# yukiteruono/pbsim3

Measured on AMD Instinct MI355X. Metric: simulated bases/sec, higher is better.
Workload: dtype u8

## Files before the change

### include/pbsim3_amd.h

```cpp
#ifndef PBSIM3_AMD_H
#define PBSIM3_AMD_H

#include <stdint.h>

#ifdef __cplusplus
extern "C" {
#endif

#define PBSIM_SUCCEEDED 1
#define PBSIM_FAILED 0

#define PBSIM_STRATEGY_WGS 1
#define PBSIM_STRATEGY_TRANS 2
#define PBSIM_STRATEGY_TEMPL 3
#define PBSIM_METHOD_QS 1
#define PBSIM_METHOD_ERR 2
#define PBSIM_METHOD_SAMPLE 3

typedef struct pbsim_params {
  int32_t strategy;
  int32_t method;
  uint32_t seed;
  int32_t pass_num;
  double depth;
  double accuracy_mean;
  double len_mean;
  double len_sd;
  double hp_del_bias;
  int64_t len_min;
  int64_t len_max;
  int64_t sub_ratio;
  int64_t ins_ratio;
  int64_t del_ratio;
  char id_prefix[64];
} pbsim_params;

typedef struct pbsim_stats {
  int64_t res_num;
  int64_t res_pass_num;
  int64_t res_len_total;
  int64_t res_len_min, res_len_max;
  int64_t res_sub_num, res_ins_num, res_del_num;
  double res_depth;
  double res_len_mean, res_len_sd;
  double res_accuracy_mean, res_accuracy_sd;
  double res_sub_rate, res_ins_rate, res_del_rate;
} pbsim_stats;

typedef struct pbsim_batch_info {
  int64_t first_read;
  int64_t n_reads;
  int64_t n_final;
  int32_t quota_reached;
  int32_t need_truncated_read;
  int64_t len_total_after;
  int64_t bases;
  int64_t read_text_bytes;
  int64_t maf_text_bytes;
  int64_t ref_bases;
  int64_t maf_columns;
} pbsim_batch_info;

typedef struct pbsim_sink {
  void *user;
  int (*on_read_text)(void *user, const char *text, int64_t bytes);
  int (*on_maf_text)(void *user, const char *text, int64_t bytes);
} pbsim_sink;

typedef struct pbsim_ctx pbsim_ctx;

void pbsim_params_default(pbsim_params *p);
pbsim_ctx *pbsim_create(const pbsim_params *p, int device);
void pbsim_destroy(pbsim_ctx *ctx);
const char *pbsim_last_error(void);
const char *pbsim_version(void);

int pbsim_load_errhmm(pbsim_ctx *ctx, const char *path);
int pbsim_load_qshmm(pbsim_ctx *ctx, const char *path);

int pbsim_set_reference(pbsim_ctx *ctx, const uint8_t *seq, int64_t len, int64_t record_index);
int pbsim_set_reference_device(pbsim_ctx *ctx, const void *seq_device, int64_t len, int64_t record_index);
int pbsim_prefetch_reference(pbsim_ctx *ctx, const uint8_t *seq, int64_t len);
int pbsim_prefetch_reference_device(pbsim_ctx *ctx, const void *seq_device, int64_t len);
int pbsim_add_hp_census(pbsim_ctx *ctx, const uint8_t *seq, int64_t len);
int pbsim_finish_hp_census(pbsim_ctx *ctx);

int pbsim_set_transcripts(pbsim_ctx *ctx, int64_t n, const char *const *ids, const int64_t *plus_exp,
                          const int64_t *minus_exp, const uint8_t *const *seqs, const int64_t *lens);

int pbsim_set_templates(pbsim_ctx *ctx, int64_t n, const char *const *ids, const uint8_t *const *seqs,
                        const int64_t *lens);

int pbsim_simulate_wgs(pbsim_ctx *ctx, const pbsim_sink *sink);
int pbsim_simulate_trans(pbsim_ctx *ctx, const pbsim_sink *sink);
int pbsim_simulate_templ(pbsim_ctx *ctx, const pbsim_sink *sink);
int pbsim_simulate_units_range(pbsim_ctx *ctx, int64_t first_read, int64_t n_reads, const pbsim_sink *sink);
int64_t pbsim_unit_reads(pbsim_ctx *ctx);

typedef struct pbsim_read_arrays {
  uint8_t *seq, *qual;
  int32_t *ref_pos;
  int64_t *offsets;
  int64_t *read_number;
  int32_t *pass_index, *unit;
  uint8_t *strand;
  int64_t *ref_start;
  int32_t *ref_span, *n_sub, *n_ins, *n_del;
} pbsim_read_arrays;
typedef struct pbsim_array_sink {
  void *user;
  int (*alloc)(void *user, int64_t tasks, int64_t bases, pbsim_read_arrays *out);
  int (*on_batch)(void *user, const pbsim_batch_info *info);
} pbsim_array_sink;
int pbsim_simulate_arrays(pbsim_ctx *ctx, const pbsim_array_sink *sink);
int pbsim_load_transcript_file(pbsim_ctx *ctx, const char *path, int64_t stats[2]);
int pbsim_load_template_file(pbsim_ctx *ctx, const char *path, int64_t stats[2]);
int pbsim_get_stats(pbsim_ctx *ctx, pbsim_stats *out);
int pbsim_set_sample_profile(pbsim_ctx *ctx, int64_t n, const uint8_t *const *quals, const int64_t *lens);
int pbsim_simulate_sample(pbsim_ctx *ctx, const pbsim_sink *sink);
typedef struct pbsim_sample_stats {
  int64_t num, len_min, len_max, len_total;
  int64_t num_filtered, len_min_filtered, len_max_filtered, len_total_filtered;
  double len_mean_filtered, len_sd_filtered, accuracy_mean_filtered, accuracy_sd_filtered;
} pbsim_sample_stats;
int pbsim_sample_profile_from_bytes(pbsim_ctx *ctx, const void *fastq, int64_t n, double accuracy_min, double accuracy_max,
                                    pbsim_sample_stats *out);
int pbsim_sample_profile_from_device(pbsim_ctx *ctx, const void *d_fastq, int64_t n, double accuracy_min, double accuracy_max,
                                     pbsim_sample_stats *out);
int pbsim_load_sample_fastq(pbsim_ctx *ctx, const char *path, double accuracy_min, double accuracy_max, pbsim_sample_stats *out);
int pbsim_sample_profile_text(pbsim_ctx *ctx, char *dst, int64_t cap, int64_t *bytes);
int pbsim_set_sample_chunk_bytes(pbsim_ctx *ctx, int64_t bytes);
int pbsim_load_sample(pbsim_ctx *ctx, const char *path, double accuracy_min, double accuracy_max, pbsim_sample_stats *out);
int pbsim_sample_profile_from_bam_bytes(pbsim_ctx *ctx, const void *bam, int64_t n, double accuracy_min, double accuracy_max,
                                        pbsim_sample_stats *out);
int pbsim_sample_profile_from_bam_device(pbsim_ctx *ctx, const void *d_bam, int64_t n, double accuracy_min, double accuracy_max,
                                         pbsim_sample_stats *out);
int64_t pbsim_sam_header(pbsim_ctx *ctx, char *buf, int64_t cap);
int pbsim_set_bam_output(pbsim_ctx *ctx, int on);
int64_t pbsim_bam_header(pbsim_ctx *ctx, char *buf, int64_t cap);
int pbsim_set_truth_bam(pbsim_ctx *ctx, int on);
int64_t pbsim_truth_bam_header(pbsim_ctx *ctx, char *buf, int64_t cap);
int64_t pbsim_job_truth_bam_header(pbsim_ctx *ctx, int64_t record, char *buf, int64_t cap);
int pbsim_set_deflate(pbsim_ctx *ctx, int mask);
int64_t pbsim_deflate_bound(int64_t text_bytes);
int pbsim_batch_fetch_deflated(pbsim_ctx *ctx, char *read_gz, int64_t read_cap, char *maf_gz, int64_t maf_cap,
                               int64_t *read_gz_bytes, int64_t *maf_gz_bytes);
int pbsim_deflate_buffer(pbsim_ctx *ctx, const void *src, int64_t n, void *dst, int64_t cap, int64_t *out_bytes);
int64_t pbsim_inflate_bound(const void *src, int64_t n);
int pbsim_inflate_buffer(pbsim_ctx *ctx, const void *src, int64_t n, void *dst, int64_t cap, int64_t *out_bytes);
typedef struct pbsim_sorted_bam_sink {
  void *user;
  int (*on_bam)(void *user, const char *bytes, int64_t n, int64_t offset);
  int (*on_index)(void *user, const char *bytes, int64_t n);
} pbsim_sorted_bam_sink;
int pbsim_truth_bam_sort(pbsim_ctx *ctx, const void *bam, int64_t n, const pbsim_sorted_bam_sink *sink, int64_t stats[4]);
typedef struct pbsim_eval_truth {
  const void *bytes;
  int64_t n;
  const char *ref_name;
} pbsim_eval_truth;
typedef struct pbsim_eval_opts {
  int32_t overlap_permille;
  int32_t hash_bits;
} pbsim_eval_opts;
typedef struct pbsim_eval_sink {
  void *user;
  int (*on_verdicts)(void *user, const unsigned char *bytes, int64_t n);
} pbsim_eval_sink;
int pbsim_truth_bam_eval(pbsim_ctx *ctx, const pbsim_eval_truth *truth, int n_truth, const void *query, int64_t n,
                         const pbsim_eval_opts *opts, const pbsim_eval_sink *sink, int64_t counts[12], int64_t hist[512]);
int64_t pbsim_eval_report(const int64_t counts[12], const int64_t hist[512], char *buf, int64_t cap);
typedef struct pbsim_depth_opts {
  int32_t exclude_flags, min_mapq, count_deletions;
  int32_t format;
  int64_t window;
  int64_t piece_bytes;
} pbsim_depth_opts;
typedef struct pbsim_depth_sink {
  void *user;
  int (*on_text)(void *user, const char *bytes, int64_t n, int64_t offset);
  int (*on_refs)(void *user, int32_t n_ref, const char *const *names,
                 const int64_t *rows );
  int (*on_depth)(void *user, int32_t ref, const int32_t *depth, int64_t l_ref);
} pbsim_depth_sink;
int pbsim_bam_depth(pbsim_ctx *ctx, const void *bam, int64_t n, const pbsim_depth_opts *opts,
                    const pbsim_depth_sink *sink, int64_t counts[6], int64_t hist[256]);
int64_t pbsim_depth_report(const int64_t counts[6], int32_t n_ref, const char *const *names, const int64_t *rows,
                           const int64_t hist[256], char *buf, int64_t cap);
typedef struct pbsim_stats_file {
  const void *bam;
  int64_t n;
} pbsim_stats_file;
typedef struct pbsim_stats_opts {
  int32_t exclude_flags, min_mapq;
  int64_t piece_bytes;
} pbsim_stats_opts;
typedef struct pbsim_stats_sink {
  void *user;
  int (*on_text)(void *user, const char *bytes, int64_t n, int64_t offset);
} pbsim_stats_sink;
int pbsim_bam_stats(pbsim_ctx *ctx, const pbsim_stats_file *files, int n_files, const pbsim_stats_opts *opts,
                    const pbsim_stats_sink *sink, int64_t counts[10], int64_t len_row[16], int64_t totals[12],
                    int64_t hist_q[128], int64_t hist_identity[1001], int64_t hist_qacc[1001]);
int64_t pbsim_stats_report(const int64_t counts[10], const int64_t len_row[16], const int64_t totals[12],
                           const int64_t hist_q[128], const int64_t hist_identity[1001], const int64_t hist_qacc[1001],
                           char *buf, int64_t cap);
typedef struct pbsim_errors_ref {
  const char *name;
  const void *lines;
  int64_t bytes;
} pbsim_errors_ref;
typedef struct pbsim_errors_file {
  const void *bam;
  int64_t n;
  const char *ref_name;
} pbsim_errors_file;
typedef struct pbsim_errors_opts {
  int32_t exclude_flags, min_mapq;
  int64_t piece_bytes;
} pbsim_errors_opts;
typedef struct pbsim_errors_sink {
  void *user;
  int (*on_text)(void *user, const char *bytes, int64_t n, int64_t offset);
} pbsim_errors_sink;
typedef struct pbsim_errors_result {
  int64_t counts[14];
  int64_t totals[11];
  int64_t pair[25];
  int64_t hp_cols[12], hp_sub[12], hp_del[12];
  int64_t ins_len[64], del_len[64];
  int64_t ins_base[5], del_base[5];
  int64_t qcal[128][3];
  int64_t hist_identity[1001];
  int64_t fit_ok, fit_bias_milli, fit_suggest_milli;
} pbsim_errors_result;
int pbsim_bam_errors(pbsim_ctx *ctx, const pbsim_errors_ref *refs, int n_refs, const pbsim_errors_file *files, int n_files,
                     const pbsim_errors_opts *opts, const pbsim_errors_sink *sink, pbsim_errors_result *result);
int64_t pbsim_errors_report(const pbsim_errors_result *result, char *buf, int64_t cap);
typedef struct pbsim_pileup_opts {
  int32_t exclude_flags, min_mapq, min_baseq;
  int32_t format;
  int64_t min_depth;
  int64_t piece_bytes;
} pbsim_pileup_opts;
typedef struct pbsim_pileup_sink {
  void *user;
  int (*on_text)(void *user, const char *bytes, int64_t n, int64_t offset);
  int (*on_cells)(void *user, int32_t ref, const uint32_t *cells, int64_t l_ref);
} pbsim_pileup_sink;
typedef struct pbsim_pileup_result {
  int64_t counts[9];
  int64_t sites[9];
  int64_t cell_sums[8];
  int64_t ins_unanchored, max_depth;
  int64_t hp_called[12], hp_sub[12], hp_del[12], hp_ins[12];
} pbsim_pileup_result;
int pbsim_bam_pileup(pbsim_ctx *ctx, const pbsim_errors_ref *refs, int n_refs, const pbsim_errors_file *files, int n_files,
                     const pbsim_pileup_opts *opts, const pbsim_pileup_sink *sink, pbsim_pileup_result *result);
int64_t pbsim_pileup_report(const pbsim_pileup_result *result, char *buf, int64_t cap);
typedef struct pbsim_consensus_opts {
  int32_t exclude_flags, min_mapq, min_baseq;
  int32_t fill;
  int64_t min_depth;
  int32_t max_ins;
  int32_t line_width;
  int64_t piece_bytes;
} pbsim_consensus_opts;
typedef struct pbsim_consensus_sink {
  void *user;
  int (*on_text)(void *user, const char *bytes, int64_t n, int64_t offset);
  int (*on_record)(void *user, int32_t ref, int64_t l_ref, int64_t l_cons);
} pbsim_consensus_sink;
typedef struct pbsim_consensus_result {
  int64_t counts[9];
  int64_t sites[9];
  int64_t ins_unanchored, max_depth;
  int64_t bases[6];
  int64_t ins_sites, ins_longest, ins_capped;
  int64_t ins_len[64];
  int64_t text_bytes;
} pbsim_consensus_result;
int pbsim_bam_consensus(pbsim_ctx *ctx, const pbsim_errors_ref *refs, int n_refs, const pbsim_errors_file *files, int n_files,
                        const pbsim_consensus_opts *opts, const pbsim_consensus_sink *sink, pbsim_consensus_result *result);
int64_t pbsim_consensus_report(const pbsim_consensus_result *result, char *buf, int64_t cap);
typedef struct pbsim_call_opts {
  int32_t exclude_flags, min_mapq, min_baseq;
  int32_t max_ins;
  int64_t min_depth;
  int64_t piece_bytes;
} pbsim_call_opts;
typedef struct pbsim_call_sink {
  void *user;
  int (*on_text)(void *user, const char *bytes, int64_t n, int64_t offset);
  int (*on_record)(void *user, int32_t ref, int64_t l_ref, int64_t n_variants);
} pbsim_call_sink;
typedef struct pbsim_call_result {
  int64_t counts[9];
  int64_t sites[9];
  int64_t ins_unanchored, max_depth;
  int64_t variants;
// ... 174 lines not shown
```

### pbsim3_amd/__init__.py

```python
import ctypes as C
import os
from typing import NamedTuple

from . import build as _build

STRATEGY_WGS, STRATEGY_TRANS, STRATEGY_TEMPL = 1, 2, 3
METHOD_QS, METHOD_ERR, METHOD_SAMPLE = 1, 2, 3


class Params(C.Structure):
    _fields_ = [
        ("strategy", C.c_int32), ("method", C.c_int32), ("seed", C.c_uint32), ("pass_num", C.c_int32),
        ("depth", C.c_double), ("accuracy_mean", C.c_double), ("len_mean", C.c_double), ("len_sd", C.c_double),
        ("hp_del_bias", C.c_double), ("len_min", C.c_int64), ("len_max", C.c_int64),
        ("sub_ratio", C.c_int64), ("ins_ratio", C.c_int64), ("del_ratio", C.c_int64),
        ("id_prefix", C.c_char * 64),
    ]


class Stats(C.Structure):
    _fields_ = [
        ("res_num", C.c_int64), ("res_pass_num", C.c_int64), ("res_len_total", C.c_int64),
        ("res_len_min", C.c_int64), ("res_len_max", C.c_int64),
        ("res_sub_num", C.c_int64), ("res_ins_num", C.c_int64), ("res_del_num", C.c_int64),
# ... 257 lines not shown



class MutateOpts(C.Structure):
    _fields_ = [("seed", C.c_uint32), ("snv_ppm", C.c_int32), ("ins_ppm", C.c_int32), ("del_ppm", C.c_int32), ("ext_ppm", C.c_int32),
                ("max_indel", C.c_int32), ("line_width", C.c_int32), ("piece_bytes", C.c_int64)]


MUTATE_TEXT_CB = C.CFUNCTYPE(C.c_int, C.c_void_p, C.c_void_p, C.c_int64, C.c_int64)
MUTATE_RECORD_CB = C.CFUNCTYPE(C.c_int, C.c_void_p, C.c_int32, C.c_int64, C.c_int64, C.c_int64)
MUTATE_ORIGIN_CB = C.CFUNCTYPE(C.c_int, C.c_void_p, C.c_int32, C.c_void_p, C.c_int64)


class MutateSink(C.Structure):
    _fields_ = [("user", C.c_void_p), ("on_fasta", MUTATE_TEXT_CB), ("on_vcf", MUTATE_TEXT_CB), ("on_record", MUTATE_RECORD_CB),
                ("on_origin", MUTATE_ORIGIN_CB)]


MUTATE_TYPES = ["snv", "ins", "del"]


class MutateResult(C.Structure):
    _fields_ = [("records", C.c_int64), ("bases_in", C.c_int64), ("eligible", C.c_int64), ("bases_out", C.c_int64), ("drawn", C.c_int64 * 3),
                ("void_del", C.c_int64), ("dropped", C.c_int64), ("merged", C.c_int64), ("substituted", C.c_int64), ("inserted", C.c_int64),
                ("deleted", C.c_int64), ("variants", C.c_int64), ("types", C.c_int64 * 3), ("ref_bases", C.c_int64), ("alt_bases", C.c_int64),
                ("longest_ref", C.c_int64), ("longest_alt", C.c_int64), ("header_bytes", C.c_int64), ("vcf_bytes", C.c_int64),
                ("fasta_bytes", C.c_int64)]


class CompareOpts(C.Structure):
    _fields_ = [("lines", C.c_int32), ("min_ms", C.c_int32), ("piece_bytes", C.c_int64)]


COMPARE_TEXT_CB = C.CFUNCTYPE(C.c_int, C.c_void_p, C.c_void_p, C.c_int64, C.c_int64)


class CompareSink(C.Structure):
    _fields_ = [("user", C.c_void_p), ("on_text", COMPARE_TEXT_CB)]


COMPARE_LINES = {"discordant": 0, "all": 1}


class CompareResult(C.Structure):
    _fields_ = [("files", C.c_int64 * 11 * 2), ("types", C.c_int64 * 6 * 4), ("lengths", C.c_int64 * 4 * 5 * 2), ("ms", C.c_int64 * 2 * 64),
                ("text_bytes", C.c_int64)]

class ApplyOpts(C.Structure):
    _fields_ = [("haplotype", C.c_int32), ("sample", C.c_int32), ("lines", C.c_int32), ("line_width", C.c_int32), ("piece_bytes", C.c_int64)]


APPLY_TEXT_CB = C.CFUNCTYPE(C.c_int, C.c_void_p, C.c_void_p, C.c_int64, C.c_int64)
APPLY_RECORD_CB = C.CFUNCTYPE(C.c_int, C.c_void_p, C.c_int32, C.c_int64, C.c_int64, C.c_int64)
APPLY_ORIGIN_CB = C.CFUNCTYPE(C.c_int, C.c_void_p, C.c_int32, C.c_void_p, C.c_int64)


class ApplySink(C.Structure):
    _fields_ = [("user", C.c_void_p), ("on_fasta", APPLY_TEXT_CB), ("on_text", APPLY_TEXT_CB), ("on_record", APPLY_RECORD_CB),
                ("on_origin", APPLY_ORIGIN_CB)]


APPLY_LINES = {"discordant": 0, "all": 1}
APPLY_TYPES = ["snv", "ins", "del", "complex"]
APPLY_SCALARS = ["lines", "malformed", "unknown_contig", "no_call", "ref_allele", "unsupported", "ref_mismatch", "filtered", "no_change", "overlap",
                 "applied", "bases_in", "bases_out", "inserted", "deleted", "substituted", "longest_cluster", "fasta_bytes", "text_bytes"]


class ApplyResult(C.Structure):
    _fields_ = [("lines", C.c_int64), ("malformed", C.c_int64), ("unknown_contig", C.c_int64), ("no_call", C.c_int64), ("ref_allele", C.c_int64),
                ("unsupported", C.c_int64), ("ref_mismatch", C.c_int64), ("filtered", C.c_int64), ("no_change", C.c_int64), ("overlap", C.c_int64),
                ("applied", C.c_int64), ("types", C.c_int64 * 4), ("bases_in", C.c_int64), ("bases_out", C.c_int64), ("inserted", C.c_int64),
                ("deleted", C.c_int64), ("substituted", C.c_int64), ("longest_cluster", C.c_int64), ("fasta_bytes", C.c_int64),
                ("text_bytes", C.c_int64)]

API = [
    ("pbsim_job_add_record", C.c_int, [C.c_void_p, C.c_void_p, C.c_int64]),
    ("pbsim_job_add_record_device", C.c_int, [C.c_void_p, C.c_void_p, C.c_int64]),
    ("pbsim_job_add_record_lines", C.c_int, [C.c_void_p, C.c_void_p, C.c_int64, C.c_int64]),
    ("pbsim_job_add_record_comm", C.c_int, [C.c_void_p, C.c_void_p, C.c_int64, C.POINTER(Comm), C.c_int32]),
    ("pbsim_job_records", C.c_int64, [C.c_void_p]),
    ("pbsim_job_begin", C.c_int, [C.c_void_p, C.c_int64]),
    ("pbsim_job_clear", C.c_int, [C.c_void_p]),
    ("pbsim_job_run", C.c_int, [C.c_void_p, C.POINTER(Comm), C.POINTER(RecordSink)]),
    ("pbsim_job_sam_header", C.c_int64, [C.c_void_p, C.c_int64, C.c_char_p, C.c_int64]),
    ("pbsim_job_bam_header", C.c_int64, [C.c_void_p, C.c_int64, C.c_char_p, C.c_int64]),
    ("pbsim_job_counters", C.c_int, [C.c_void_p, C.POINTER(C.c_int64)]),
    ("pbsim_job_progress", C.c_int, [C.c_void_p, C.POINTER(C.c_int64)]),
    ("pbsim_job_set_interleave", C.c_int, [C.c_void_p, C.c_int]),
    ("pbsim_job_expect", C.c_int, [C.c_void_p, C.c_int64, C.POINTER(C.c_int64)]),
    ("pbsim_job_feed_abort", C.c_int, [C.c_void_p, C.c_char_p]),
    ("pbsim_scratch_state", C.c_int, [C.c_void_p, C.POINTER(C.c_double)]),
    ("pbsim_batch_fetch_lengths", C.c_int, [C.c_void_p, C.c_void_p, C.c_void_p, C.c_void_p]),
    ("pbsim_job_breakdown", C.c_int, [C.c_void_p, C.POINTER(C.c_double)]),
    ("pbsim_bind_host_to_device", C.c_int, [C.c_int, C.c_char_p, C.c_int64]),
    ("pbsim_rccl_unique_id", C.c_int64, [C.c_void_p, C.c_int64]),
    ("pbsim_rccl_comm_create", C.POINTER(Comm), [C.c_void_p, C.c_int64, C.c_int32, C.c_int32, C.c_int32]),
    ("pbsim_rccl_comm_create_file", C.POINTER(Comm), [C.c_char_p, C.c_int32, C.c_int32, C.c_int32]),
    ("pbsim_rccl_comm_info", C.c_int, [C.POINTER(Comm), C.POINTER(C.c_int64)]),
    ("pbsim_rccl_comm_destroy", None, [C.POINTER(Comm)]),
    ("pbsim_stats_keep_values", C.c_int, [C.c_void_p, C.c_int]),
    ("pbsim_stats_merge", C.c_int, [C.c_void_p, C.POINTER(Comm)]),
    ("pbsim_stats_add_tasks", C.c_int, [C.c_void_p, C.c_int64, C.c_int64, C.POINTER(C.c_int32), C.POINTER(C.c_int32),
                                        C.POINTER(C.c_int32), C.POINTER(C.c_int32), C.POINTER(C.c_double)]),
    ("pbsim_format_stats", C.c_int64, [C.POINTER(Params), C.POINTER(Stats), C.c_int64, C.c_char_p, C.c_int64]),
    ("pbsim_cli_main", C.c_int, [C.c_int, C.POINTER(C.c_char_p), C.POINTER(Comm), C.c_int]),
    ("pbsim_params_default", None, [C.POINTER(Params)]),
    ("pbsim_create", C.c_void_p, [C.POINTER(Params), C.c_int]),
    ("pbsim_destroy", None, [C.c_void_p]),
    ("pbsim_last_error", C.c_char_p, []),
    ("pbsim_version", C.c_char_p, []),
    ("pbsim_load_errhmm", C.c_int, [C.c_void_p, C.c_char_p]),
    ("pbsim_load_qshmm", C.c_int, [C.c_void_p, C.c_char_p]),
    ("pbsim_set_reference", C.c_int, [C.c_void_p, C.c_void_p, C.c_int64, C.c_int64]),
    ("pbsim_set_reference_device", C.c_int, [C.c_void_p, C.c_void_p, C.c_int64, C.c_int64]),
    ("pbsim_add_hp_census", C.c_int, [C.c_void_p, C.c_void_p, C.c_int64]),
    ("pbsim_finish_hp_census", C.c_int, [C.c_void_p]),
    ("pbsim_set_transcripts", C.c_int, [C.c_void_p, C.c_int64, C.POINTER(C.c_char_p), C.POINTER(C.c_int64),
                                        C.POINTER(C.c_int64), C.POINTER(C.c_void_p), C.POINTER(C.c_int64)]),
    ("pbsim_set_templates", C.c_int, [C.c_void_p, C.c_int64, C.POINTER(C.c_char_p), C.POINTER(C.c_void_p),
                                      C.POINTER(C.c_int64)]),
    ("pbsim_simulate_templ", C.c_int, [C.c_void_p, C.POINTER(Sink)]),
    ("pbsim_prefetch_reference", C.c_int, [C.c_void_p, C.c_char_p, C.c_int64]),
    ("pbsim_prefetch_reference_device", C.c_int, [C.c_void_p, C.c_void_p, C.c_int64]),
    ("pbsim_simulate_units_range", C.c_int, [C.c_void_p, C.c_int64, C.c_int64, C.POINTER(Sink)]),
    ("pbsim_unit_reads", C.c_int64, [C.c_void_p]),
    ("pbsim_load_transcript_file", C.c_int, [C.c_void_p, C.c_char_p, C.POINTER(C.c_int64)]),
    ("pbsim_load_template_file", C.c_int, [C.c_void_p, C.c_char_p, C.POINTER(C.c_int64)]),
    ("pbsim_simulate_wgs", C.c_int, [C.c_void_p, C.POINTER(Sink)]),
    ("pbsim_simulate_trans", C.c_int, [C.c_void_p, C.POINTER(Sink)]),
    ("pbsim_simulate_arrays", C.c_int, [C.c_void_p, C.POINTER(ArraySink)]),
    ("pbsim_get_stats", C.c_int, [C.c_void_p, C.POINTER(Stats)]),
    ("pbsim_sam_header", C.c_int64, [C.c_void_p, C.c_char_p, C.c_int64]),
    ("pbsim_set_bam_output", C.c_int, [C.c_void_p, C.c_int]),
    ("pbsim_bam_header", C.c_int64, [C.c_void_p, C.c_char_p, C.c_int64]),
    ("pbsim_set_truth_bam", C.c_int, [C.c_void_p, C.c_int]),
    ("pbsim_truth_bam_header", C.c_int64, [C.c_void_p, C.c_char_p, C.c_int64]),
    ("pbsim_job_truth_bam_header", C.c_int64, [C.c_void_p, C.c_int64, C.c_char_p, C.c_int64]),
    ("pbsim_set_sample_profile", C.c_int, [C.c_void_p, C.c_int64, C.POINTER(C.c_void_p), C.POINTER(C.c_int64)]),
    ("pbsim_simulate_sample", C.c_int, [C.c_void_p, C.POINTER(Sink)]),
    ("pbsim_sample_profile_from_bytes", C.c_int, [C.c_void_p, C.c_void_p, C.c_int64, C.c_double, C.c_double, C.POINTER(SampleStats)]),
    ("pbsim_sample_profile_from_device", C.c_int, [C.c_void_p, C.c_void_p, C.c_int64, C.c_double, C.c_double, C.POINTER(SampleStats)]),
    ("pbsim_load_sample_fastq", C.c_int, [C.c_void_p, C.c_char_p, C.c_double, C.c_double, C.POINTER(SampleStats)]),
    ("pbsim_load_sample", C.c_int, [C.c_void_p, C.c_char_p, C.c_double, C.c_double, C.POINTER(SampleStats)]),
    ("pbsim_sample_profile_from_bam_bytes", C.c_int, [C.c_void_p, C.c_void_p, C.c_int64, C.c_double, C.c_double, C.POINTER(SampleStats)]),
    ("pbsim_sample_profile_from_bam_device", C.c_int, [C.c_void_p, C.c_void_p, C.c_int64, C.c_double, C.c_double, C.POINTER(SampleStats)]),
    ("pbsim_sample_profile_text", C.c_int, [C.c_void_p, C.c_void_p, C.c_int64, C.POINTER(C.c_int64)]),
    ("pbsim_set_sample_chunk_bytes", C.c_int, [C.c_void_p, C.c_int64]),
    ("pbsim_simulate_sample_comm", C.c_int, [C.c_void_p, C.POINTER(Comm), C.POINTER(RecordSink)]),
    ("pbsim_set_deflate", C.c_int, [C.c_void_p, C.c_int]),
    ("pbsim_deflate_bound", C.c_int64, [C.c_int64]),
    ("pbsim_batch_fetch_deflated", C.c_int, [C.c_void_p, C.c_void_p, C.c_int64, C.c_void_p, C.c_int64,
                                             C.POINTER(C.c_int64), C.POINTER(C.c_int64)]),
    ("pbsim_deflate_buffer", C.c_int, [C.c_void_p, C.c_void_p, C.c_int64, C.c_void_p, C.c_int64, C.POINTER(C.c_int64)]),
    ("pbsim_inflate_bound", C.c_int64, [C.c_void_p, C.c_int64]),
    ("pbsim_inflate_buffer", C.c_int, [C.c_void_p, C.c_void_p, C.c_int64, C.c_void_p, C.c_int64, C.POINTER(C.c_int64)]),
    ("pbsim_truth_bam_sort", C.c_int, [C.c_void_p, C.c_void_p, C.c_int64, C.POINTER(SortedBamSink), C.POINTER(C.c_int64)]),
    ("pbsim_truth_bam_eval", C.c_int, [C.c_void_p, C.POINTER(EvalTruth), C.c_int, C.c_char_p, C.c_int64, C.POINTER(EvalOpts),
                                       C.POINTER(EvalSink), C.POINTER(C.c_int64), C.POINTER(C.c_int64)]),
    ("pbsim_eval_report", C.c_int64, [C.POINTER(C.c_int64), C.POINTER(C.c_int64), C.c_char_p, C.c_int64]),
    ("pbsim_bam_depth", C.c_int, [C.c_void_p, C.c_char_p, C.c_int64, C.POINTER(DepthOpts), C.POINTER(DepthSink), C.POINTER(C.c_int64),
                                  C.POINTER(C.c_int64)]),
    ("pbsim_depth_report", C.c_int64, [C.POINTER(C.c_int64), C.c_int32, C.POINTER(C.c_char_p), C.POINTER(C.c_int64), C.POINTER(C.c_int64),
                                       C.c_char_p, C.c_int64]),
    ("pbsim_bam_stats", C.c_int, [C.c_void_p, C.POINTER(StatsFile), C.c_int, C.POINTER(StatsOpts), C.POINTER(StatsSink)] + [C.POINTER(C.c_int64)] * 6),
    ("pbsim_stats_report", C.c_int64, [C.POINTER(C.c_int64)] * 6 + [C.c_char_p, C.c_int64]),
    ("pbsim_bam_errors", C.c_int, [C.c_void_p, C.POINTER(ErrorsRef), C.c_int, C.POINTER(ErrorsFile), C.c_int, C.POINTER(ErrorsOpts),
                                   C.POINTER(ErrorsSink), C.POINTER(ErrorsResult)]),
    ("pbsim_errors_report", C.c_int64, [C.POINTER(ErrorsResult), C.c_char_p, C.c_int64]),
    ("pbsim_bam_pileup", C.c_int, [C.c_void_p, C.POINTER(ErrorsRef), C.c_int, C.POINTER(ErrorsFile), C.c_int, C.POINTER(PileupOpts),
                                   C.POINTER(PileupSink), C.POINTER(PileupResult)]),
    ("pbsim_pileup_report", C.c_int64, [C.POINTER(PileupResult), C.c_char_p, C.c_int64]),
    ("pbsim_bam_consensus", C.c_int, [C.c_void_p, C.POINTER(ErrorsRef), C.c_int, C.POINTER(ErrorsFile), C.c_int, C.POINTER(ConsensusOpts),
                                      C.POINTER(ConsensusSink), C.POINTER(ConsensusResult)]),
    ("pbsim_consensus_report", C.c_int64, [C.POINTER(ConsensusResult), C.c_char_p, C.c_int64]),
    ("pbsim_bam_call", C.c_int, [C.c_void_p, C.POINTER(ErrorsRef), C.c_int, C.POINTER(ErrorsFile), C.c_int, C.POINTER(CallOpts), C.POINTER(CallSink),
                                 C.POINTER(CallResult)]),
    ("pbsim_call_report", C.c_int64, [C.POINTER(CallResult), C.c_char_p, C.c_int64]),
    ("pbsim_genome_mutate", C.c_int, [C.c_void_p, C.POINTER(ErrorsRef), C.c_int, C.POINTER(MutateOpts), C.POINTER(MutateSink),
                                      C.POINTER(MutateResult)]),
    ("pbsim_mutate_report", C.c_int64, [C.POINTER(MutateResult), C.c_char_p, C.c_int64]),
    ("pbsim_vcf_compare", C.c_int, [C.c_void_p, C.POINTER(ErrorsRef), C.c_int, C.POINTER(C.c_char_p), C.c_char_p, C.c_int64, C.c_char_p, C.c_int64,
                                    C.POINTER(CompareOpts), C.POINTER(CompareSink), C.POINTER(CompareResult)]),
    ("pbsim_compare_report", C.c_int64, [C.POINTER(CompareResult), C.c_char_p, C.c_int64]),
    ("pbsim_vcf_apply", C.c_int, [C.c_void_p, C.POINTER(ErrorsRef), C.c_int, C.POINTER(C.c_char_p), C.c_char_p, C.c_int64, C.POINTER(ApplyOpts),
                                  C.POINTER(ApplySink), C.POINTER(ApplyResult)]),
    ("pbsim_apply_report", C.c_int64, [C.POINTER(ApplyResult), C.c_char_p, C.c_int64]),
    ("pbsim_apply_sample", C.c_int32, [C.c_char_p, C.c_int64, C.c_char_p]),
    ("pbsim_batch_walk", C.c_int, [C.c_void_p, C.c_int64, C.c_int64, C.c_int64, C.POINTER(C.c_int64)]),
    ("pbsim_slot_count", C.c_int, []),
    ("pbsim_select_slot", C.c_int, [C.c_void_p, C.c_int]),
    ("pbsim_batch_walk_begin", C.c_int, [C.c_void_p, C.c_int64, C.c_int64, C.c_int64]),
    ("pbsim_batch_walk_end", C.c_int, [C.c_void_p, C.POINTER(C.c_int64)]),
    ("pbsim_batch_finalize", C.c_int, [C.c_void_p, C.c_int64, C.POINTER(BatchInfo)]),
    ("pbsim_batch_fetch", C.c_int, [C.c_void_p, C.c_void_p, C.c_void_p]),
    ("pbsim_batch_account", C.c_int, [C.c_void_p]),
    ("pbsim_reset_stats", C.c_int, [C.c_void_p]),
    ("pbsim_unit_quota", C.c_int64, [C.c_void_p]),
    ("pbsim_batch_capacity", C.c_int64, [C.c_void_p]),
    ("pbsim_set_scratch_bytes", C.c_int, [C.c_void_p, C.c_int64]),
    ("pbsim_release_pools", C.c_int, [C.c_void_p]),
    ("pbsim_prof_reset", C.c_int, [C.c_void_p]),
    ("pbsim_prof_get", C.c_int, [C.c_void_p, C.POINTER(C.c_double), C.POINTER(C.c_int64), C.POINTER(C.c_double)]),
    ("pbsim_prof_walk_busy", C.c_int, [C.c_void_p, C.POINTER(C.c_double)]),
    ("pbsim_prof_tail", C.c_int, [C.c_void_p, C.POINTER(C.c_double), C.POINTER(C.c_int64)]),
    ("pbsim_prof_secondary", C.c_int, [C.c_void_p, C.POINTER(C.c_double)]),
    ("pbsim_prof_wave_launches", C.c_int64, [C.c_void_p]),
    ("pbsim_stream", C.c_void_p, [C.c_void_p]),
    ("pbsim_device_synchronize", C.c_int, [C.c_void_p]),
    ("pbsim_philox4x32_10", None, [C.POINTER(C.c_uint32), C.POINTER(C.c_uint32), C.POINTER(C.c_uint32)]),
    ("pbsim_dump_table", C.c_int64, [C.c_void_p, C.c_int, C.c_void_p, C.c_int64]),
]

_lib = None


def lib_path():
    return _build.LIB


def _torch_runtime_first():
    import sys
    if "torch" in sys.modules or os.environ.get("PBSIM_TORCH_COMPAT", "1") == "0":
        return
    try:
        import importlib.util
        spec = importlib.util.find_spec("torch")
        if not spec or not spec.origin:
            return
        libdir = os.path.join(os.path.dirname(spec.origin), "lib")
        for name in ("libhsa-runtime64.so", "libamdhip64.so"):
            path = os.path.join(libdir, name)
            if os.path.exists(path):
                C.CDLL(path, mode=C.RTLD_GLOBAL)
    except Exception:
        pass


def load(build_if_missing=True):
    global _lib
    if _lib is not None:
        return _lib
    _torch_runtime_first()
    if not os.path.exists(_build.LIB):
        if not build_if_missing:
            raise RuntimeError("libpbsim3_amd.so is not built (python -m pbsim3_amd.build)")
        _build.build()
    lib = C.CDLL(_build.LIB)
    for name, res, args in API:
        fn = getattr(lib, name)
        fn.restype = res
        fn.argtypes = args
    _lib = lib
    return lib


def eval_report(counts, hist) -> bytes:
    vals = [counts[k] for k in EVAL_COUNTS] if isinstance(counts, dict) else list(counts)
    c = (C.c_int64 * 12)(*[int(v) for v in vals])
    h = (C.c_int64 * 512)(*[int(v) for row in hist for v in row])
    n = load().pbsim_eval_report(c, h, None, 0)
    if n < 0:
        raise PbsimError("pbsim_eval_report: bad argument")
    buf = C.create_string_buffer(max(n, 1))
    load().pbsim_eval_report(c, h, buf, n)
    return buf.raw[:n]


def depth_report(counts, refs, hist) -> bytes:
    vals = [counts[k] for k in DEPTH_COUNTS] if isinstance(counts, dict) else list(counts)
    refs = list(refs)
    c = (C.c_int64 * 6)(*[int(v) for v in vals])
    h = (C.c_int64 * 256)(*[int(v) for v in hist])
    names = (C.c_char_p * max(len(refs), 1))(*[r[0].encode() if isinstance(r[0], str) else bytes(r[0]) for r in refs])
    rows = (C.c_int64 * max(4 * len(refs), 1))(*[int(v) for r in refs for v in r[1:5]])
    n = load().pbsim_depth_report(c, len(refs), names, rows, h, None, 0)
    if n < 0:
        raise PbsimError("pbsim_depth_report: bad argument")
    buf = C.create_string_buffer(max(n, 1))
    load().pbsim_depth_report(c, len(refs), names, rows, h, buf, n)
    return buf.raw[:n]


def stats_report(counts, len_row, totals, hist_q, hist_identity, hist_qacc) -> bytes:
    def vals(x, names):
        return [int(x[k]) for k in names] if isinstance(x, dict) else [int(v) for v in x]
    parts = [vals(counts, STATS_COUNTS), vals(len_row, STATS_LEN_ROW), vals(totals, STATS_TOTALS), [int(v) for v in hist_q],
             [int(v) for v in hist_identity], [int(v) for v in hist_qacc]]
    if [len(p) for p in parts] != [10, 16, 12, 128, 1001, 1001]:
        raise ValueError("stats_report: 10 counts, 16 length values, 12 totals and histograms of 128, 1001 and 1001 bins")
    arrs = [(C.c_int64 * len(p))(*p) for p in parts]
    n = load().pbsim_stats_report(*arrs, None, 0)
    if n < 0:
        raise PbsimError("pbsim_stats_report: bad argument")
    buf = C.create_string_buffer(max(n, 1))
    load().pbsim_stats_report(*arrs, buf, n)
    return buf.raw[:n]


def _errors_dict(res) -> dict:
    out = dict(counts=dict(zip(ERRORS_COUNTS, (int(v) for v in res.counts))), totals=dict(zip(ERRORS_TOTALS, (int(v) for v in res.totals))))
    for name, _ in ERRORS_ARRAYS:
        out[name] = [int(v) for v in getattr(res, name)]
    for name in ERRORS_FIT:
        out[name] = int(getattr(res, name))
    return out

# ... 450 lines not shown
        sink = Sink(None, SINK_CB(on_read), SINK_CB(on_maf))
        _check(self.lib.pbsim_simulate_wgs(self.h, C.byref(sink) if collect else None))
        return b"".join(reads), b"".join(mafs)

    def simulate_arrays(self, on_batch=None, labels=True):
        import collections

        import torch
        dev = torch.device("cuda", self.device)
        pending, batches, error = collections.deque(), [], []

        def alloc(user, tasks, bases, out):
            try:
                torch.cuda.current_stream(dev).synchronize()
                t = {}
                for name, dtype, per in ARRAY_FIELDS:
                    if name == "ref_pos" and not labels:
                        t[name] = None
                        continue
                    n = bases if per == "base" else tasks + 1 if per == "offset" else tasks
                    t[name] = torch.empty(n, dtype=getattr(torch, dtype), device=dev)
                    setattr(out.contents, name, t[name].data_ptr() or None)
                pending.append(t)
                return 1
            except BaseException as e:
                error.append(e)
                return 0

        def done(user, info):
            try:
                b = ReadBatch(first_read=info.contents.first_read, **pending.popleft())
                if on_batch is None:
                    batches.append(b)
                    return 1
                return 0 if on_batch(b) is False else 1
            except BaseException as e:
                error.append(e)
                return 0

        sink = ArraySink(None, ARRAY_ALLOC_CB(alloc), ARRAY_BATCH_CB(done))
        ok = self.lib.pbsim_simulate_arrays(self.h, C.byref(sink))
        if error:
            raise error[0]
        _check(ok)
        if on_batch is not None:
            return None
        if not batches:
            empty = {name: torch.zeros(1 if per == "offset" else 0, dtype=getattr(torch, dtype), device=dev)
                     for name, dtype, per in ARRAY_FIELDS}
            if not labels:
                empty["ref_pos"] = None
            return ReadBatch(first_read=1, **empty)
        cat = {}
        for name, _, per in ARRAY_FIELDS:
            if name == "ref_pos" and not labels:
                cat[name] = None
            elif per == "offset":
                base, parts = 0, []
                for b in batches:
                    parts.append(b.offsets[:-1] + base)
                    base += int(b.offsets[-1])
                parts.append(torch.tensor([base], dtype=torch.int64, device=dev))
                cat[name] = torch.cat(parts)
            else:
                cat[name] = torch.cat([getattr(b, name) for b in batches])
        return ReadBatch(first_read=batches[0].first_read, **cat)

    def sam_header(self):
        n = self.lib.pbsim_sam_header(self.h, None, 0)
        buf = C.create_string_buffer(n + 1)
        self.lib.pbsim_sam_header(self.h, buf, n + 1)
        return buf.raw[:n]

    def set_sample_profile(self, quals):
        n = len(quals)
        keep = [C.create_string_buffer(q, len(q)) for q in quals]
        ptrs = (C.c_void_p * n)(*[C.cast(b, C.c_void_p).value for b in keep])
        lens = (C.c_int64 * n)(*[len(q) for q in quals])
        _check(self.lib.pbsim_set_sample_profile(self.h, n, ptrs, lens))

    def load_sample_fastq(self, path, acc_min=0.75, acc_max=1.0):
        st = SampleStats()
        _check(self.lib.pbsim_load_sample_fastq(self.h, os.fsencode(path), acc_min, acc_max, C.byref(st)))
        return st

    def sample_profile_from_fastq(self, data, acc_min=0.75, acc_max=1.0):
        st = SampleStats()
        if isinstance(data, (bytes, bytearray, memoryview)):
            data = bytes(data)
            _check(self.lib.pbsim_sample_profile_from_bytes(self.h, data, len(data), acc_min, acc_max, C.byref(st)))
            return st
        import torch
        if not (isinstance(data, torch.Tensor) and data.dtype == torch.uint8 and data.is_cuda and data.is_contiguous()):
            raise TypeError("sample_profile_from_fastq: bytes or a contiguous uint8 tensor on the context's device")
        if data.device.index != self.device:
            raise ValueError("sample_profile_from_fastq: the tensor is on another device than the context")
        torch.cuda.current_stream(data.device).synchronize()
        _check(self.lib.pbsim_sample_profile_from_device(self.h, C.c_void_p(data.data_ptr()), data.numel(), acc_min, acc_max,
                                                         C.byref(st)))
        return st

    def load_sample(self, path, acc_min=0.75, acc_max=1.0):
        st = SampleStats()
        _check(self.lib.pbsim_load_sample(self.h, os.fsencode(path), acc_min, acc_max, C.byref(st)))
        return st

    def sample_profile_from_bam(self, data, acc_min=0.75, acc_max=1.0):
        st = SampleStats()
        if isinstance(data, (bytes, bytearray, memoryview)):
            data = bytes(data)
            _check(self.lib.pbsim_sample_profile_from_bam_bytes(self.h, data, len(data), acc_min, acc_max, C.byref(st)))
            return st
        import torch
        if not (isinstance(data, torch.Tensor) and data.dtype == torch.uint8 and data.is_cuda and data.is_contiguous()):
            raise TypeError("sample_profile_from_bam: bytes or a contiguous uint8 tensor on the context's device")
        if data.device.index != self.device:
            raise ValueError("sample_profile_from_bam: the tensor is on another device than the context")
        torch.cuda.current_stream(data.device).synchronize()
        _check(self.lib.pbsim_sample_profile_from_bam_device(self.h, C.c_void_p(data.data_ptr()), data.numel(), acc_min, acc_max,
                                                             C.byref(st)))
        return st

    def sample_profile(self):
        n = C.c_int64(0)
        _check(self.lib.pbsim_sample_profile_text(self.h, None, 0, C.byref(n)))
        buf = C.create_string_buffer(max(n.value, 1))
        _check(self.lib.pbsim_sample_profile_text(self.h, buf, n.value, C.byref(n)))
        return buf.raw[:n.value].split(b"\n")[:-1]

    def set_sample_chunk_bytes(self, n):
        _check(self.lib.pbsim_set_sample_chunk_bytes(self.h, n))

    def simulate_sample(self, collect=True):
        return self._simulate(self.lib.pbsim_simulate_sample, collect)

    def _simulate(self, fn, collect):
        reads, mafs = [], []

        def on_read(user, text, n):
            reads.append(C.string_at(text, n))
            return 1

        def on_maf(user, text, n):
            mafs.append(C.string_at(text, n))
            return 1

        sink = Sink(None, SINK_CB(on_read), SINK_CB(on_maf))
        _check(fn(self.h, C.byref(sink) if collect else None))
        return b"".join(reads), b"".join(mafs)

    def set_deflate(self, mask=3):
        _check(self.lib.pbsim_set_deflate(self.h, 3 if mask is True else int(mask)))

    def deflate_buffer(self, data: bytes) -> bytes:
        cap = self.lib.pbsim_deflate_bound(len(data)) + 64
        dst = C.create_string_buffer(cap)
        n = C.c_int64(0)
        src = C.create_string_buffer(data, len(data)) if data else None
        _check(self.lib.pbsim_deflate_buffer(self.h, src, len(data), dst, cap, C.byref(n)))
        return dst.raw[:n.value]

    def inflate_buffer(self, data: bytes) -> bytes:
        cap = inflate_bound(data)
        if cap < 0:
            _check(self.lib.pbsim_inflate_buffer(self.h, data, len(data), None, 0, C.byref(C.c_int64(0))))
        dst = C.create_string_buffer(max(cap, 1))
        n = C.c_int64(0)
        _check(self.lib.pbsim_inflate_buffer(self.h, data, len(data), dst, cap, C.byref(n)))
        return dst.raw[:n.value]

    def sort_truth_bam(self, data, on_index=None):
        parts, index, at = [], [], [0]

        def on_bam(user, ptr, n, offset):
            if offset != at[0]:
                return 0
            parts.append(C.string_at(ptr, n))
            at[0] += n
            return 1

        def on_idx(user, ptr, n):
            index.append(C.string_at(ptr, n))
            if on_index:
                on_index(index[-1])
            return 1
        sink = SortedBamSink(None, SORTED_BAM_CB(on_bam), SORTED_INDEX_CB(on_idx))
        stats = (C.c_int64 * 4)()
        _check(self.lib.pbsim_truth_bam_sort(self.h, bytes(data), len(data), C.byref(sink), stats))
        return b"".join(parts), b"".join(index), tuple(stats)

    def eval_bam(self, truth, query, ref_names=None, overlap=0.1, verdicts=False, hash_bits=0):
        import numpy as np
        files = [truth] if isinstance(truth, (bytes, bytearray, memoryview)) else list(truth)
        names = list(ref_names) if ref_names is not None else [None] * len(files)
        if len(names) != len(files):
            raise ValueError("ref_names: one entry per truth file (%d given for %d files)" % (len(names), len(files)))
        if not 0 < overlap <= 1:
            raise ValueError("overlap must be in (0, 1]")
        keep = [bytes(f) for f in files]
        arr = (EvalTruth * max(len(keep), 1))()
        for k, (f, nm) in enumerate(zip(keep, names)):
            arr[k] = EvalTruth(f, len(f), None if nm is None else (nm.encode() if isinstance(nm, str) else bytes(nm)))
        opts = EvalOpts(max(1, int(round(overlap * 1000))), int(hash_bits))
        got = []

        def on_verdicts(user, ptr, n):
            got.append(np.frombuffer(C.string_at(ptr, n), dtype=np.uint8).copy() if n else np.zeros(0, np.uint8))
            return 1
        sink = EvalSink(None, EVAL_VERDICTS_CB(on_verdicts))
        counts = (C.c_int64 * 12)()
        hist = (C.c_int64 * 512)()
        query = bytes(query)
        _check(self.lib.pbsim_truth_bam_eval(self.h, arr, len(keep), query, len(query), C.byref(opts), C.byref(sink) if verdicts else None,
                                             counts, hist))
        cd = dict(zip(EVAL_COUNTS, (int(v) for v in counts)))
        hd = np.array(list(hist), dtype=np.int64).reshape(256, 2)
        out = (cd, hd, eval_report(cd, hd))
        return out + (got[0],) if verdicts else out

    def bam_depth(self, data, fmt="bedgraph", window=0, min_mapq=0, exclude_flags=0x704, deletions=True, arrays=False, piece_bytes=0):
        import numpy as np
        if fmt not in DEPTH_FORMATS:
            raise ValueError("fmt must be bedgraph or window")
        parts, at, refs, depth = [], [0], [], []

        def on_text(user, ptr, n, offset):
            if offset != at[0]:
                return 0
            parts.append(C.string_at(ptr, n))
            at[0] += n
            return 1

        def on_refs(user, n_ref, names, rows):
            refs.extend((names[r],) + tuple(int(rows[4 * r + k]) for k in range(4)) for r in range(n_ref))
            return 1

        def on_depth(user, ref, ptr, l_ref):
            depth.append(np.frombuffer(C.string_at(ptr, 4 * l_ref), dtype=np.int32).copy() if l_ref else np.zeros(0, np.int32))
            return 1
        sink = DepthSink(None, DEPTH_TEXT_CB(on_text), DEPTH_REFS_CB(on_refs), DEPTH_ARRAY_CB(on_depth) if arrays else DEPTH_ARRAY_CB())
        opts = DepthOpts(int(exclude_flags), int(min_mapq), 1 if deletions else 0, DEPTH_FORMATS[fmt], int(window), int(piece_bytes))
        counts = (C.c_int64 * 6)()
        hist = (C.c_int64 * 256)()
        data = bytes(data)
        _check(self.lib.pbsim_bam_depth(self.h, data, len(data), C.byref(opts), C.byref(sink), counts, hist))
        cd = dict(zip(DEPTH_COUNTS, (int(v) for v in counts)))
        hd = np.array(list(hist), dtype=np.int64)
        out = (b"".join(parts), cd, refs, hd, depth_report(cd, refs, hd))
        return out + (depth,) if arrays else out

    def bam_stats(self, files, min_mapq=0, exclude_flags=0x900, text=False, piece_bytes=0):
        import numpy as np
        if isinstance(files, (bytes, bytearray, memoryview)):
            files = [files]
        files = [bytes(f) for f in files]
        arr = (StatsFile * max(len(files), 1))(*[StatsFile(C.cast(C.c_char_p(f), C.c_void_p), len(f)) for f in files])
        parts, at = [], [0]

        def on_text(user, ptr, n, offset):
            if offset != at[0]:
                return 0
            parts.append(C.string_at(ptr, n))
            at[0] += n
            return 1
        sink = StatsSink(None, STATS_TEXT_CB(on_text) if text else STATS_TEXT_CB())
        opts = StatsOpts(int(exclude_flags), int(min_mapq), int(piece_bytes))
        out = [(C.c_int64 * k)() for k in (10, 16, 12, 128, 1001, 1001)]
        _check(self.lib.pbsim_bam_stats(self.h, arr, len(files), C.byref(opts), C.byref(sink), *out))
        cd = dict(zip(STATS_COUNTS, (int(v) for v in out[0])))
        ld = dict(zip(STATS_LEN_ROW, (int(v) for v in out[1])))
        td = dict(zip(STATS_TOTALS, (int(v) for v in out[2])))
        hists = tuple(np.array(list(h), dtype=np.int64) for h in out[3:])
        res = (cd, ld, td) + hists + (stats_report(cd, ld, td, *hists),)
        return res + (b"".join(parts),) if text else res

    def bam_errors(self, files, genome, ref_names=None, text=False, min_mapq=0, exclude_flags=0x900, piece_bytes=0):
        if isinstance(files, (bytes, bytearray, memoryview)):
            files = [files]
        files = [bytes(f) for f in files]
        names = list(ref_names) if ref_names is not None else [None] * len(files)
        if len(names) != len(files):
            raise ValueError("ref_names: one entry per file (%d given for %d files)" % (len(names), len(files)))
        names = [None if nm is None else (nm.encode() if isinstance(nm, str) else bytes(nm)) for nm in names]
        genome = [((nm.encode() if isinstance(nm, str) else bytes(nm)), bytes(lines)) for nm, lines in genome]
        refs = (ErrorsRef * max(len(genome), 1))(*[ErrorsRef(nm, C.cast(C.c_char_p(lines), C.c_void_p), len(lines)) for nm, lines in genome])
        arr = (ErrorsFile * max(len(files), 1))(*[ErrorsFile(C.cast(C.c_char_p(f), C.c_void_p), len(f), nm) for f, nm in zip(files, names)])
        parts, at = [], [0]

        def on_text(user, ptr, n, offset):
            if offset != at[0]:
                return 0
            parts.append(C.string_at(ptr, n))
            at[0] += n
            return 1
        sink = ErrorsSink(None, ERRORS_TEXT_CB(on_text) if text else ERRORS_TEXT_CB())
        opts = ErrorsOpts(int(exclude_flags), int(min_mapq), int(piece_bytes))
        res = ErrorsResult()
        _check(self.lib.pbsim_bam_errors(self.h, refs, len(genome), arr, len(files), C.byref(opts), C.byref(sink), C.byref(res)))
        out = _errors_dict(res)
        got = (out, errors_report(out))
        return got + (b"".join(parts),) if text else got

    def bam_pileup(self, files, genome, ref_names=None, text=False, fmt="sites", min_mapq=0, exclude_flags=0x900, min_baseq=0, min_depth=1,
                   arrays=False, piece_bytes=0):
        import numpy as np
        if arrays:
            import torch
        if fmt not in PILEUP_FORMATS:
            raise ValueError("fmt must be sites or all")
        if isinstance(files, (bytes, bytearray, memoryview)):
            files = [files]
        files = [bytes(f) for f in files]
# ... 503 lines not shown
```

### pbsim3_amd/csrc/ctx.h

```cpp
#pragma once
#include <hip/hip_runtime.h>
#include <limits.h>
#include <stdio.h>
#include <stdlib.h>
#include <stdint.h>

#include <algorithm>
#include <condition_variable>
#include <functional>
#include <memory>
#include <mutex>
#include <string>
#include <vector>

#include "../../include/pbsim3_amd.h"
#include "host_tables.h"
#include "kernels.h"

namespace pbsim {
extern thread_local std::string g_err;
int fail(const std::string &m);
}


#define NEED_DEVICE(c)                                                                      \
  do {                                                                                      \
    if ((c)->device < 0 || !(c)->stream)                                                    \
      return fail("this context has no HIP device: the gfx950 product path has no CPU fallback"); \
  } while (0)

#define HIP_OK(expr)                                                                        \
  do {                                                                                      \
    hipError_t e_ = (expr);                                                                 \
    if (e_ != hipSuccess)                                                                   \
      return fail(std::string("HIP error: ") + hipGetErrorString(e_) + " at " #expr);       \
  } while (0)

struct DevBuf {
  void *p = nullptr;
  size_t bytes = 0;
  ~DevBuf() { release(); }
  void release() {
    if (p) (void)hipFree(p);
    p = nullptr;
    bytes = 0;
  }
  hipError_t ensure(size_t n, bool exact = false) {
    if (n <= bytes) return hipSuccess;
    release();
    size_t want = exact ? n : std::max<size_t>(n + n / 8 + 256, 64u << 10);
    hipError_t e = hipMalloc(&p, want);
    if (e != hipSuccess) {
      p = nullptr;
      return e;
    }
    bytes = want;
    return hipSuccess;
  }
  template <class T>
  T *as() const {
    return reinterpret_cast<T *>(p);
  }
};

struct HostBuf {
  void *p = nullptr;
  size_t bytes = 0;
  ~HostBuf() {
    if (p) (void)hipHostFree(p);
  }
  hipError_t ensure(size_t n) {
    if (n <= bytes) return hipSuccess;
    if (p) (void)hipHostFree(p);
    p = nullptr;
    bytes = 0;
    size_t want = std::max<size_t>(n + n / 8 + 4096, 1u << 20);
    hipError_t e = hipHostMalloc(&p, want, hipHostMallocDefault);
    if (e != hipSuccess) {
      p = nullptr;
      return e;
    }
    bytes = want;
    return hipSuccess;
  }
};

using namespace pbsim;

constexpr int kMaxSlots = 6;
constexpr int kPipelineDepth = 2;
static_assert(kPipelineDepth >= 1 && kPipelineDepth <= kMaxSlots, "the pipeline's slots are the first of kMaxSlots");

constexpr size_t kScratchSlack = 64u << 10;
constexpr double kSinkBatchBases = 5.0e9;

constexpr int kDfBuffers = 5;
struct DfLane {
  DevBuf d_df_status, d_df_ctl;
  uint32_t epoch = 0;
  DevBuf d_df_dense[kDfBuffers];
  DevBuf d_df_code;
  HostBuf h_df_total, h_df_out[kDfBuffers];
  hipStream_t stream = nullptr;
  hipStream_t copy_stream = nullptr;
  bool own_streams = false;
  hipStream_t own[2] = {nullptr, nullptr};
  bool pre_valid = false, pre_own_staging = false, pre_elsewhere = false;
  const uint8_t *pre_text = nullptr;
  int64_t pre_n = 0;
  int pre_count = 0;
  hipStream_t lane_stream = nullptr;
  hipEvent_t ev_pre = nullptr;
  hipEvent_t ev_hand = nullptr;
  bool hand_open = false;
  hipEvent_t ev_df[kDfBuffers] = {}, ev_cp[kDfBuffers] = {};
  hipEvent_t ev_k0[kDfBuffers] = {}, ev_k1[kDfBuffers] = {};
  std::vector<std::unique_ptr<HostBuf>> arena_blocks;
  std::vector<size_t> arena_fill;
  std::vector<char> arena_touched;
  std::vector<int> arena_idle;
  std::vector<std::pair<const char *, int64_t>> arena_segs;
  size_t arena_bytes() const {
    size_t n = 0;
    for (const auto &b : arena_blocks) n += b->bytes;
    return n;
  }
  void arena_reset() {
    std::fill(arena_fill.begin(), arena_fill.end(), 0);
    arena_segs.clear();
  }
  char *arena_reserve(int64_t n, size_t max_bytes) {
    static const size_t kBlock = getenv("PBSIM_PINNED_BLOCK_KB") && atoll(getenv("PBSIM_PINNED_BLOCK_KB")) > 0
                                     ? (size_t)atoll(getenv("PBSIM_PINNED_BLOCK_KB")) << 10 : (size_t)256u << 20;
    const size_t need = ((size_t)n + 63) & ~(size_t)63;
    for (size_t i = 0; i < arena_blocks.size(); i++) {
      HostBuf &b = *arena_blocks[i];
      if (arena_fill[i] + need <= b.bytes) {
        char *p = (char *)b.p + arena_fill[i];
        arena_fill[i] += need;
        arena_touched[i] = 1;
        arena_segs.emplace_back(p, n);
        return p;
      }
    }
    const size_t want = std::max(kBlock, need);
    if (max_bytes && arena_bytes() + want > max_bytes) return nullptr;
    if (getenv("PBSIM_TRACE")) fprintf(stderr, "[pbsim arena] new block of %zu MB (lane holds %zu MB in %zu blocks)\n", want >> 20, arena_bytes() >> 20, arena_blocks.size());
    arena_blocks.emplace_back(new HostBuf);
    arena_fill.push_back(0);
    arena_touched.push_back(1);
    arena_idle.push_back(0);
    if (arena_blocks.back()->ensure(want) != hipSuccess) {
      arena_blocks.pop_back();
      arena_fill.pop_back();
      arena_touched.pop_back();
      arena_idle.pop_back();
      return nullptr;
    }
    arena_fill.back() = need;
    arena_segs.emplace_back((char *)arena_blocks.back()->p, n);
    return (char *)arena_blocks.back()->p;
  }
  static constexpr int kArenaIdleJobs = 16;
  void arena_release() {
    arena_blocks.clear();
    arena_fill.clear();
    arena_touched.clear();
    arena_idle.clear();
    arena_segs.clear();
  }
  void arena_trim() {
    size_t k = 0;
    for (size_t i = 0; i < arena_blocks.size(); i++) arena_idle[i] = arena_touched[i] ? 0 : arena_idle[i] + 1;
    if (getenv("PBSIM_TRACE")) {
      size_t drop = 0;
      for (size_t i = 0; i < arena_blocks.size(); i++) drop += arena_idle[i] >= kArenaIdleJobs ? 1 : 0;
      if (drop) fprintf(stderr, "[pbsim arena] trim: %zu of %zu blocks go back\n", drop, arena_blocks.size());
    }
    for (size_t i = 0; i < arena_blocks.size(); i++)
      if (arena_idle[i] < kArenaIdleJobs) {
        if (k != i) {
          arena_blocks[k] = std::move(arena_blocks[i]);
          arena_idle[k] = arena_idle[i];
        }
        k++;
      }
    arena_blocks.resize(k);
    arena_idle.resize(k);
    arena_fill.assign(k, 0);
    arena_touched.assign(k, 0);
    arena_segs.clear();
  }
};

struct RefDesc {
  const uint8_t *seq = nullptr;
  const uint8_t *hp = nullptr;
  int64_t len = 0;
  int64_t unit = 0;
  bool hp_flag = false;
  bool hp11 = false;
};

struct StatsAcc {
  int64_t res_num = 0, res_len_total = 0, res_len_min = LONG_MAX, res_len_max = 0;
  int64_t res_sub = 0, res_ins = 0, res_del = 0;
  double accuracy_total = 0.0;
  std::vector<int64_t> freq_len, freq_acc;
  bool keep_values = false;
  struct Block {
    int64_t first_task;
    std::vector<double> values;
  };
  std::vector<Block> blocks;
  void reset() {
    res_num = res_len_total = res_len_max = 0;
    res_len_min = LONG_MAX;
    res_sub = res_ins = res_del = 0;
    accuracy_total = 0.0;
    std::fill(freq_len.begin(), freq_len.end(), 0);
    std::fill(freq_acc.begin(), freq_acc.end(), 0);
    blocks.clear();
  }
};

struct Slot {
  RefDesc ref;
  hipStream_t stream = nullptr;
  hipEvent_t ev0 = nullptr, ev1 = nullptr, ev2 = nullptr, ev3 = nullptr;
  DevBuf d_flags;
  DevBuf d_rawlen, d_len, d_off, d_acc;
  DevBuf d_hist, d_bin_start, d_bin_cursor, d_class_start;
  DevBuf d_task_of_slot, d_slot_of_task, d_wave_cap, d_wave_off, d_wg_tmp, d_wg_order;
  DevBuf d_out_len, d_maf_len, d_nsub, d_nins, d_ndel, d_qsum;
  DevBuf d_cum, d_scan_tmp, d_rt_len, d_mt_len, d_row_dst;
  DevBuf d_n_runs;
  hipEvent_t ev_c0 = nullptr, ev_c1 = nullptr;
  DevBuf d_chain, d_chain_mask;
  DevBuf d_scratch, d_read_text, d_maf_text;
  HostBuf h_read_text, h_maf_text, h_stats, h_flags;
  DfLane df[2];
  hipStream_t walk_stream = nullptr;
  hipEvent_t ev_sq_walk = nullptr, ev_sq_done = nullptr;
  bool sq_pending = false;
  hipEvent_t ev_prep = nullptr;
  hipStream_t coop_stream = nullptr;
  hipEvent_t ev_coop = nullptr;
  bool stats_fetched = false;
  hipEvent_t ev_t0 = nullptr, ev_t1 = nullptr;
  bool text_timed = false;
  int64_t text_in = 0, text_out = 0;
  hipEvent_t ev_text = nullptr;
  int64_t b_first = 0, b_n = 0, b_slots_max = 0;
  bool b_truncated = false, b_enqueued = false, b_walked = false, b_finalized = false;
  bool b_chain = false;
  bool b_exported = false;
  int64_t b_trunc = -1;
  double b_factor = 2.0;
  int64_t b_pass0 = 0;
  int64_t b_max_raw = 0;
  pbsim_batch_info b_info;
};

struct JobRecord {
  DevBuf seq, hp, tiles, flags;
  int64_t len = 0;
  RefDesc ref;
  hipEvent_t ready = nullptr;
  DeviceFlags *h_flags = nullptr;
  ~JobRecord() {
    if (ready) (void)hipEventDestroy(ready);
    if (h_flags) (void)hipHostFree(h_flags);
  }
};

struct pbsim_ctx {
  pbsim_params p;
  int device = 0;
  hipStream_t stream = nullptr;
  Slot slots[kMaxSlots];
  int cur = 0;
  Slot &s() { return slots[cur]; }

  std::unique_ptr<ErrModel> err;
  std::unique_ptr<QsModel> qs;
  HeaderTables hdr;
  HpBias bias;
  ErrClassTables ect;
  QsClassTables qct;
  bool class_tables_dirty = true;
  int coop_wg_errhmm[2] = {0, 0};
  bool header_uploaded = false;

  DevBuf d_prob2len, d_prob2acc, d_cls;
  DevBuf d_qs_tabs_v[2];
  bool qs_tabs_ready[2] = {false, false};
  DevBuf d_seq_own, d_hp, d_tiles, d_ref_flags;
  DevBuf d_seq_next, d_hp_next, d_tiles_next, d_ref_flags_next;
  hipStream_t prefetch_stream = nullptr;
  DevBuf d_lines, d_lines_tmp;
  hipStream_t sq_stream = nullptr;
  const void *pf_src = nullptr;
  int64_t pf_len = 0;
  bool seq_hp_flag = false;
  const uint8_t *d_seq = nullptr;
  int64_t ref_len = 0;
  int64_t unit = 0;
  int64_t census[kHpSlots] = {0};
  int64_t unit_census[kHpSlots] = {0};
  bool census_done = false;
  bool census_from_job = false;
  bool hp11_explicit = false;
  bool hp11_before_job = false;
  int64_t n_units = 0, trans_reads = 0;
  DevBuf d_read_unit, d_read_minus, d_read_base, d_unit_len, d_unit_rank, d_unit_names, d_off_table, d_ssp, d_ssp_rv;
  DevBuf d_sq, d_sq_line_len, d_sq_line_qoff, d_sq_vbase;
  std::vector<int32_t> sq_len;
  std::vector<int64_t> sq_off;
  int64_t sq_total = 0;
  int64_t sp_chunk_bytes = 0;
  int64_t scratch_budget = 0;
  double scratch_factor = 2.0, need_seen = 0.0;
  bool scratch_factor_fixed = false;
  int64_t rewalked_batches = 0;
  bool scratch_auto = true;
  hipStream_t df_streams[2][2] = {{nullptr, nullptr}, {nullptr, nullptr}};
  bool defer_text_sync = false;
  bool defer_account = false;
  int walk_lds_kb = 27;
  bool bam_output = false;
  bool truth_bam = false;
  std::vector<std::string> unit_sn;
  std::vector<int64_t> unit_ln;
  int deflate = 0;
  bool deflate_parallel = false;
  DevBuf d_df_tables;
  DevBuf d_df_prof;

  StatsAcc st;
  std::vector<std::unique_ptr<JobRecord>> job_records;
  std::mutex job_mu;
  std::condition_variable job_cv;
  std::vector<int64_t> job_expect_len;
  std::vector<std::unique_ptr<JobRecord>> job_spare;
  bool job_feed_failed = false;
  std::string job_feed_err;
  int64_t job_counters[8] = {0};
  int64_t job_progress[8] = {0};
  double job_breakdown[16] = {0};
  int job_interleave = 1;
  int64_t job_first_unit = 1;

  double prof_walk_ms = 0, prof_total_ms = 0, prof_tail_ms = 0;
  int64_t prof_walk_launches = 0, prof_tail_launches = 0;
  int64_t prof_wave_launches = 0;
  hipEvent_t ev_prof_base = nullptr;
  std::vector<std::pair<float, float>> prof_intervals;
  double prof_text_ms = 0, prof_deflate_ms = 0;
  int64_t prof_text_launches = 0, prof_text_in = 0, prof_text_out = 0;
  int64_t prof_deflate_launches = 0, prof_deflate_in = 0, prof_deflate_out = 0;
  std::mutex prof_mu;
};

namespace pbsim {
RefDesc current_ref(const pbsim_ctx *c);
int64_t quota_of(const pbsim_ctx *c, int64_t ref_len);
int walk_begin(pbsim_ctx *c, const RefDesc &ref, int64_t first_read, int64_t n_reads, int64_t truncate_remaining, bool chain = false,
               double factor = 0.0 );
double scratch_factor_of(const pbsim_ctx *c);
int chain_end_finalize(pbsim_ctx *c, int64_t len_total_before, pbsim_batch_info *out);
int chain_reads_for(const pbsim_ctx *c, int64_t ref_len, int64_t remaining);
constexpr int kChainReads = 6;
int64_t batch_capacity_for(const pbsim_ctx *c, int64_t ref_len);
int finalize_cut(pbsim_ctx *c, int64_t len_total_before, pbsim_batch_info *out);
int finalize_text(pbsim_ctx *c, pbsim_batch_info *info);
int finalize_uncut(pbsim_ctx *c, pbsim_batch_info *out);
std::string sam_header_text(const pbsim_ctx *c, int64_t unit);
std::string truth_bam_header_bytes(const pbsim_ctx *c, int64_t ref_len);
int truth_bam_check_names(const pbsim_ctx *c);
int account_slot(pbsim_ctx *c, StatsAcc *st);
int account_of(pbsim_ctx *c, Slot &sl, StatsAcc *st);
void stats_add_task(StatsAcc *st, int64_t len_max, bool quality, long len, long nsub, long nins, long ndel, double qsum,
                    std::vector<double> *values);
void stats_finish(const StatsAcc &st, const pbsim_params &p, int64_t ref_len, pbsim_stats *o);
int stats_merge(StatsAcc *st, const pbsim_params &p, const pbsim_comm *comm, int64_t *extra, int n_extra);
int deflate_prelaunch(pbsim_ctx *c, Slot &sl, bool want_read, bool want_maf);
int deflate_pieces(pbsim_ctx *c, DfLane &lane, const uint8_t *d_text, int64_t n,
                   const std::function<int(const char *, int64_t)> &consume,
                   const std::function<char *(int64_t)> *place = nullptr, const std::function<bool()> *tail_hook = nullptr);
int deflate_handoff(pbsim_ctx *c, DfLane &next, int lane_index, const uint8_t *d_text, int64_t n, bool own_staging,
                    hipEvent_t text_ready);
int deflate_settle(DfLane &lane);
int ensure_deflate_ready(pbsim_ctx *c);
int ensure_crc_tables(pbsim_ctx *c);
// ... 5 lines not shown
```

### pbsim3_amd/csrc/deflate.hip

```cpp
#include <hip/hip_runtime.h>
#include <stdint.h>
#include <stdlib.h>

#include "kernels.h"

namespace pbsim {

namespace {

constexpr int kChunk = DF_CHUNK;
constexpr int kThreads = 256;
constexpr int kSeg = kChunk / kThreads;
constexpr int kSegDw = kSeg / 4;
constexpr int kInDw = kChunk / 4 + kChunk / 128;
constexpr int kOutBytes = 33024;
constexpr int kOutDw = kOutBytes / 4;
constexpr int kSyms = 288;
constexpr uint32_t kPoly = 0xEDB88320u;
constexpr int kHeadBits = 18 * 8;
constexpr int kPrefixBits = 3 + 5 + 5 + 4 + 19 * 3;

constexpr int kClLenTab[19] = {3, 5, 4, 4, 4, 5, 5, 5, 5, 5, 5, 5, 4, 5, 5, 5, 5, 3, 3};
constexpr int kClOrderTab[19] = {16, 17, 18, 0, 8, 7, 9, 6, 10, 5, 11, 4, 12, 3, 13, 2, 14, 1, 15};
constexpr uint64_t pack_cl_len() {
  uint64_t v = 0;
  for (int s = 0; s < 19; ++s) v |= (uint64_t)kClLenTab[s] << (3 * s);
  return v;
}
constexpr uint64_t kClLenPacked = pack_cl_len();
__device__ __forceinline__ uint32_t cl_len(uint32_t s) { return (uint32_t)(kClLenPacked >> (3 * s)) & 7u; }
constexpr unsigned __int128 pack_prefix() {
  unsigned __int128 v = 1u | (2u << 1) | ((unsigned __int128)15 << 13);
  for (int i = 0; i < 19; ++i) v |= (unsigned __int128)kClLenTab[kClOrderTab[i]] << (17 + 3 * i);
  return v;
}
constexpr uint64_t kPrefixLo = (uint64_t)pack_prefix();
constexpr uint32_t kPrefixHi = (uint32_t)(pack_prefix() >> 64);

__device__ __forceinline__ uint32_t rev_bits(uint32_t code, uint32_t len) { return __brev(code) >> (32 - len); }

__device__ __forceinline__ uint32_t cl_code(uint32_t s) {
  uint32_t c, l = cl_len(s);
  if (l == 3) c = s == 0 ? 0 : s - 16;
  else if (l == 4) c = s == 12 ? 9 : 4 + s;
  else c = s == 1 ? 20 : s <= 11 ? 16 + s : 15 + s;
  return rev_bits(c, l);
}

__device__ __forceinline__ uint32_t gf2_mul(uint32_t a, uint32_t b) {
  uint32_t p = 0;
#pragma unroll
  for (int i = 0; i < 32; ++i) {
    p ^= b & (0u - ((a >> (31 - i)) & 1u));
    b = (b >> 1) ^ (kPoly & (0u - (b & 1u)));
  }
  return p;
}

struct BitWriter {
  uint32_t *out;
  uint32_t word, nb;
  uint64_t acc;
  __device__ __forceinline__ void init(uint32_t *o, uint32_t bitpos) {
    out = o;
    word = bitpos >> 5;
    nb = bitpos & 31;
    acc = 0;
  }
  __device__ __forceinline__ void put(uint32_t v, uint32_t k) {
    acc |= (uint64_t)v << nb;
    nb += k;
    if (nb >= 32) {
      atomicOr(&out[word++], (uint32_t)acc);
      acc >>= 32;
      nb -= 32;
    }
  }
  __device__ __forceinline__ void put64(uint64_t v, uint32_t k) {
    if (k > 32) {
      put((uint32_t)v, 32);
      put((uint32_t)(v >> 32), k - 32);
    } else {
      put((uint32_t)v, k);
    }
  }
  __device__ __forceinline__ void flush() {
    if (nb) atomicOr(&out[word], (uint32_t)acc);
  }
};

__device__ __forceinline__ void length_symbol(uint32_t L, uint32_t *sym, uint32_t *eb, uint32_t *ev) {
  const uint32_t v = L - 3;
  if (v < 8) {
    *sym = 257 + v;
    *eb = 0;
    *ev = 0;
  } else if (L == 258) {
    *sym = 285;
    *eb = 0;
    *ev = 0;
  } else {
    const uint32_t e = (31 - __clz(v)) - 2;
    *sym = 261 + 4 * e + ((v >> e) & 3);
    *eb = e;
    *ev = v & ((1u << e) - 1);
  }
}

__device__ __forceinline__ uint32_t block_scan_excl(uint32_t v, uint32_t *s_wave, uint32_t *total) {
  const int lane = threadIdx.x & 63, wave = threadIdx.x >> 6;
  uint32_t inc = v;
#pragma unroll
  for (int d = 1; d < 64; d <<= 1) {
    const uint32_t o = __shfl_up(inc, d, 64);
    if (lane >= d) inc += o;
  }
  __syncthreads();
  if (lane == 63) s_wave[wave] = inc;
  __syncthreads();
  uint32_t base = 0, tot = 0;
#pragma unroll
  for (int w = 0; w < kThreads / 64; ++w) {
    const uint32_t x = s_wave[w];
    if (w < wave) base += x;
    tot += x;
  }
  *total = tot;
  return base + inc - v;
}

struct Mask128 {
  uint64_t lo, hi;
};
__device__ __forceinline__ Mask128 m_and(Mask128 a, Mask128 b) { return {a.lo & b.lo, a.hi & b.hi}; }
__device__ __forceinline__ Mask128 m_or(Mask128 a, Mask128 b) { return {a.lo | b.lo, a.hi | b.hi}; }
__device__ __forceinline__ Mask128 m_not(Mask128 a) { return {~a.lo, ~a.hi}; }
template <int K>
__device__ __forceinline__ Mask128 m_shl(Mask128 a) { return {a.lo << K, (a.hi << K) | (a.lo >> (64 - K))}; }
template <int K>
__device__ __forceinline__ Mask128 m_shr(Mask128 a) { return {(a.lo >> K) | (a.hi << (64 - K)), a.hi >> K}; }
__device__ __forceinline__ uint32_t m_nibble(Mask128 a, int j) {
  return (uint32_t)((j < 16 ? a.lo >> (4 * j) : a.hi >> (4 * j - 64)) & 15u);
}
__device__ __forceinline__ int m_first(Mask128 a) { return a.lo ? __builtin_ctzll(a.lo) : 64 + __builtin_ctzll(a.hi); }
__device__ __forceinline__ Mask128 m_clear(Mask128 a, int pos) {
  if (pos < 64) a.lo &= ~(1ull << pos);
  else a.hi &= ~(1ull << (pos - 64));
  return a;
}
__device__ __forceinline__ int m_run(Mask128 m, int pos) {
  uint64_t lo, hi;
  if (pos == 0) {
    lo = m.lo;
    hi = m.hi;
  } else if (pos < 64) {
    lo = (m.lo >> pos) | (m.hi << (64 - pos));
    hi = m.hi >> pos;
  } else {
    lo = m.hi >> (pos - 64);
    hi = 0;
  }
  if (~lo) return __builtin_ctzll(~lo);
  return ~hi ? 64 + __builtin_ctzll(~hi) : 128;
}

struct SegTokens {
  Mask128 lit;
  Mask128 start;
  Mask128 cover;
};

__device__ __forceinline__ SegTokens seg_tokens(const uint32_t (&seg)[kSegDw], int seg_n, uint32_t prev_dword,
                                                bool chunk_start) {
  uint64_t e[2] = {0, 0};
  uint32_t pw = prev_dword;
#pragma unroll
  for (int j = 0; j < kSegDw; ++j) {
    const uint32_t w = seg[j];
    const uint32_t d = w ^ ((w << 8) | (pw >> 24));
    const uint32_t z = ~(((d & 0x7F7F7F7Fu) + 0x7F7F7F7Fu) | d | 0x7F7F7F7Fu);
    const uint32_t nib = (((z >> 7) * 0x00204081u) >> 21) & 15u;
    e[j >> 4] |= (uint64_t)nib << (4 * (j & 15));
    pw = w;
  }
  Mask128 valid;
  valid.lo = seg_n >= 64 ? ~0ull : (1ull << seg_n) - 1;
  valid.hi = seg_n >= 128 ? ~0ull : seg_n > 64 ? (1ull << (seg_n - 64)) - 1 : 0ull;
  Mask128 eq = {e[0] & valid.lo, e[1] & valid.hi};
  if (chunk_start) eq.lo &= ~1ull;
  const Mask128 r3 = m_and(eq, m_and(m_shr<1>(eq), m_shr<2>(eq)));
  SegTokens t;
  t.cover = m_or(r3, m_or(m_shl<1>(r3), m_shl<2>(r3)));
  t.start = m_and(t.cover, m_not(m_shl<1>(t.cover)));
  t.lit = m_and(valid, m_not(t.cover));
  return t;
}

constexpr int kSampleChunks = DF_SAMPLE_CHUNKS;
constexpr int kHdrDw = DF_TABLE_HDR_DW;

struct DfTable {
  uint32_t code[kSyms];
  uint32_t hdr_end_bits;
  uint32_t pad[3];
  uint32_t hdr[kHdrDw];
};
static_assert(sizeof(DfTable) <= DF_TABLE_BYTES, "DF_TABLE_BYTES too small");

__device__ __forceinline__ void load_chunk(const uint8_t *__restrict__ text, int64_t n_bytes, int64_t chunk, uint32_t *s_in,
                                           uint32_t (&seg)[kSegDw], int *n_out, int *seg_n_out, uint32_t *prev_dw) {
  const int tid = threadIdx.x;
  const int64_t base = chunk * (int64_t)kChunk;
  const int n = (int)((n_bytes - base) < (int64_t)kChunk ? (n_bytes - base) : (int64_t)kChunk);
  const uint4 *src4 = reinterpret_cast<const uint4 *>(text + base);
  for (int q = tid; q < kChunk / 16; q += kThreads) {
    uint4 v = make_uint4(0, 0, 0, 0);
    if (q * 16 < n) v = src4[q];
    const int d = q * 4;
    uint32_t *dst = &s_in[d + (d >> 5)];
    dst[0] = v.x;
    dst[1] = v.y;
    dst[2] = v.z;
    dst[3] = v.w;
  }
  __syncthreads();
  const int beg = tid * kSeg;
  *n_out = n;
  *seg_n_out = n - beg < 0 ? 0 : (n - beg < kSeg ? n - beg : kSeg);
#pragma unroll
  for (int j = 0; j < kSegDw; ++j) seg[j] = s_in[tid * (kSegDw + 1) + j];
  *prev_dw = tid ? s_in[tid * (kSegDw + 1) - 2] : 0u;
  __syncthreads();
}

__global__ __launch_bounds__(kThreads) void k_deflate_hist(const uint8_t *__restrict__ text, int64_t n_bytes,
                                                            uint32_t *__restrict__ hist) {
  __shared__ uint32_t s_in[kInDw];
  __shared__ uint32_t s_hist[3 * kSyms + 64];
  const int tid = threadIdx.x, lane = tid & 63;
  for (int i = tid; i < 3 * kSyms + 64; i += kThreads) s_hist[i] = 0;
  uint32_t seg[kSegDw], prev_dw;
  int n, seg_n;
  load_chunk(text, n_bytes, blockIdx.x, s_in, seg, &n, &seg_n, &prev_dw);
  const SegTokens tk = seg_tokens(seg, seg_n, prev_dw, tid == 0);
  const uint32_t copy = (uint32_t)(lane % 3) * kSyms, dummy = 3 * kSyms + lane;
#pragma unroll
  for (int j = 0; j < kSegDw; ++j) {
    const uint32_t nl = m_nibble(tk.lit, j);
    if (nl == 0) continue;
    const uint32_t w = seg[j];
#pragma unroll
    for (int k = 0; k < 4; ++k) atomicAdd(&s_hist[((nl >> k) & 1u) ? copy + ((w >> (8 * k)) & 255u) : dummy], 1u);
  }
  Mask128 st = tk.start;
  while (st.lo | st.hi) {
    const int pos = m_first(st);
    st = m_clear(st, pos);
    uint32_t sy, eb, ev;
    length_symbol((uint32_t)m_run(tk.cover, pos), &sy, &eb, &ev);
    atomicAdd(&s_hist[copy + sy], 1u);
  }
  __syncthreads();
  for (int i = tid; i < 286; i += kThreads) {
    const uint32_t f = s_hist[i] + s_hist[kSyms + i] + s_hist[2 * kSyms + i] + (i == 256 ? 1u : 0u);
    if (f) atomicAdd(&hist[i], f);
  }
}

__global__ __launch_bounds__(kThreads) void k_deflate_build(const uint32_t *__restrict__ hist, DfTable *__restrict__ tbl) {
  __shared__ uint32_t s_freq[kSyms], s_sfreq[kSyms], s_w[kSyms], s_code[kSyms];
  __shared__ uint16_t s_sorted[kSyms], s_par[kSyms], s_leafpar[kSyms], s_dep[kSyms];
  __shared__ uint8_t s_len[kSyms];
  __shared__ uint32_t s_cnt[16], s_first[16];
  __shared__ uint32_t s_img[4 + kHdrDw];
  const int tid = threadIdx.x;
  constexpr int m = 286;
  for (int i = tid; i < kSyms; i += kThreads) {
    s_freq[i] = i < m ? hist[i] + 1u : 0u;
    s_code[i] = 0;
    s_len[i] = 0;
  }
  for (int i = tid; i < 4 + kHdrDw; i += kThreads) s_img[i] = 0;
  if (tid < 16) s_cnt[tid] = 0;
  __syncthreads();
  for (int i = tid; i < m; i += kThreads) {
    const uint32_t fi = s_freq[i];
    uint32_t rank = 0;
    for (int u = 0; u < m; ++u) {
      const uint32_t g = s_freq[u];
      rank += (g < fi) | ((g == fi) & (u < i));
    }
    s_sorted[rank] = (uint16_t)i;
    s_sfreq[rank] = fi;
  }
  __syncthreads();
  if (tid == 0) {
    int leaf = 0, root = 0;
    for (int nxt = 0; nxt < m - 1; ++nxt) {
      uint32_t tot = 0;
      for (int k = 0; k < 2; ++k) {
        const bool take_leaf = leaf < m && (root >= nxt || s_sfreq[leaf] <= s_w[root]);
        if (take_leaf) {
          tot += s_sfreq[leaf];
          s_leafpar[leaf] = (uint16_t)nxt;
          ++leaf;
        } else {
          tot += s_w[root];
          s_par[root] = (uint16_t)nxt;
          ++root;
        }
      }
      s_w[nxt] = tot;
    }
    s_dep[m - 2] = 0;
    for (int i = m - 3; i >= 0; --i) s_dep[i] = s_dep[s_par[i]] + 1;
    for (int i = 0; i < m; ++i) {
      int d = s_dep[s_leafpar[i]] + 1;
      if (d > 15) d = 15;
      s_cnt[d] += 1;
    }
    uint32_t total = 0;
    for (int l = 1; l <= 15; ++l) total += s_cnt[l] << (15 - l);
    while (total > (1u << 15)) {
      s_cnt[15] -= 1;
      for (int l = 14; l >= 1; --l)
        if (s_cnt[l]) {
          s_cnt[l] -= 1;
          s_cnt[l + 1] += 2;
          break;
        }
      total -= 1;
    }
    int i = 0;
    for (int l = 15; l >= 1; --l)
      for (uint32_t k = 0; k < s_cnt[l]; ++k) s_len[s_sorted[i++]] = (uint8_t)l;
    uint32_t code = 0;
    s_cnt[0] = 0;
    for (int l = 1; l <= 15; ++l) {
      code = (code + s_cnt[l - 1]) << 1;
      s_first[l] = code;
    }
  }
  __syncthreads();
  for (int i = tid; i < m; i += kThreads) {
    const uint32_t l = s_len[i];
    uint32_t idx = 0;
    for (int u = 0; u < i; ++u) idx += s_len[u] == l;
    s_code[i] = rev_bits(s_first[l] + idx, l) | (l << 16);
  }
  __syncthreads();
  if (tid == 0) {
    BitWriter bw;
    bw.init(s_img, kHeadBits);
    bw.put64(kPrefixLo | ((uint64_t)(m - 257) << 3), 64);
    bw.put(kPrefixHi, kPrefixBits - 64);
    uint32_t bits = kHeadBits + kPrefixBits;
    int p = 0;
    const int npos = m + 1;
    while (p < npos) {
      const uint32_t v = p < m ? s_len[p] : 1u;
      bw.put(cl_code(v), cl_len(v));
      bits += cl_len(v);
      ++p;
      int r = 0;
      while (p + r < npos && (p + r < m ? s_len[p + r] : 1u) == v) ++r;
      while (r >= 3) {
        const int t = r < 6 ? r : 6;
        bw.put(cl_code(16) | ((uint32_t)(t - 3) << cl_len(16)), cl_len(16) + 2);
        bits += cl_len(16) + 2;
        r -= t;
        p += t;
      }
    }
    bw.flush();
    tbl->hdr_end_bits = bits;
  }
  __syncthreads();
  for (int i = tid; i < kSyms; i += kThreads) tbl->code[i] = s_code[i];
  for (int i = tid; i < kHdrDw; i += kThreads) tbl->hdr[i] = s_img[4 + i];
}

struct DfCtl {
  uint32_t ticket;
  uint32_t error;
  int64_t total;
};
static_assert(sizeof(DfCtl) == DF_CTL_BYTES, "DF_CTL_BYTES");

constexpr uint64_t kStSize = 1ull << 32, kStPrefix = 2ull << 32;
__device__ __forceinline__ uint64_t st_word(uint32_t epoch, uint64_t flag, uint32_t v) { return ((uint64_t)epoch << 34) | flag | v; }

__device__ __forceinline__ uint32_t look_back(const uint64_t *status, int64_t c, uint32_t epoch, int lane, uint32_t *error) {
  uint32_t sum = 0;
  int64_t hi = c - 1;
  for (uint32_t spins = 0;; spins++) {
    if (spins > (1u << 24)) {
      if (lane == 0) atomicOr(error, 1u);
      return sum;
    }
    const int64_t i = hi - lane;
    uint64_t w = 0;
    if (i >= 0) w = __hip_atomic_load(&status[i], __ATOMIC_RELAXED, __HIP_MEMORY_SCOPE_AGENT);
    const bool mine = i >= 0 && (uint32_t)(w >> 34) == epoch && ((w >> 32) & 3u) != 0;
    const uint64_t ready = __ballot(mine || i < 0);
    const uint64_t pref = __ballot(mine && ((w >> 32) & 3u) == 2u);
    const int k = ~ready ? __builtin_ctzll(~ready) : 64;
    const uint64_t usable = k >= 64 ? ~0ull : ((1ull << k) - 1);
    const uint64_t stop = pref & usable;
    if (stop) {
      const int e = __builtin_ctzll(stop);
      uint32_t v = (lane <= e && i >= 0) ? (uint32_t)w : 0u;
#pragma unroll
      for (int d = 32; d >= 1; d >>= 1) v += __shfl_xor(v, d, 64);
      return sum + v;
    }
    if (k == 0) {
      __builtin_amdgcn_s_sleep(2);
      continue;
    }
    uint32_t v = (lane < k && i >= 0) ? (uint32_t)w : 0u;
#pragma unroll
    for (int d = 32; d >= 1; d >>= 1) v += __shfl_xor(v, d, 64);
    sum += v;
    hi -= k;
    if (hi < 0) return sum;
  }
}

typedef uint32_t u32x4 __attribute__((ext_vector_type(4)));
__device__ __forceinline__ void store_member(uint8_t *dst, const uint32_t *s_img, uint32_t bytes, int tid) {
  const uint32_t head = min((uint32_t)((16u - ((uintptr_t)dst & 15u)) & 15u), bytes);
  const uint8_t *s8 = reinterpret_cast<const uint8_t *>(s_img);
  if ((uint32_t)tid < head) dst[tid] = s8[tid];
  const uint32_t nvec = (bytes - head) >> 4;
  const uint32_t sh = head & 3u, dw0 = head >> 2;
  u32x4 *d4 = reinterpret_cast<u32x4 *>(dst + head);
  for (uint32_t v = tid; v < nvec; v += kThreads) {
    const uint32_t *p = s_img + dw0 + 4u * v;
    const uint32_t a = p[0], b = p[1], c = p[2], d = p[3], e = p[4];
    u32x4 o;
    o.x = __builtin_amdgcn_alignbyte(b, a, sh);
    o.y = __builtin_amdgcn_alignbyte(c, b, sh);
    o.z = __builtin_amdgcn_alignbyte(d, c, sh);
    o.w = __builtin_amdgcn_alignbyte(e, d, sh);
    __builtin_nontemporal_store(o, &d4[v]);
  }
  const uint32_t done = head + 16u * nvec;
  if ((uint32_t)tid < bytes - done) dst[done + tid] = s8[done + tid];
}

__global__ __launch_bounds__(kThreads) void k_deflate_chunks(const uint8_t *__restrict__ text, int64_t n_bytes,
                                                              uint8_t *__restrict__ dense, uint64_t *__restrict__ status,
                                                              DfCtl *__restrict__ ctl, uint32_t epoch,
                                                              const uint32_t *__restrict__ crc_table,
                                                              const uint32_t *__restrict__ pow128, uint32_t x8rem,
                                                              const DfTable *__restrict__ tbl,
                                                              unsigned long long *__restrict__ prof) {
  __shared__ uint32_t s_in[kInDw];
  static_assert(kOutDw <= kInDw, "the output image must fit the input image");
  uint32_t *const s_out = s_in;
  __shared__ uint32_t s_code[kSyms];
  uint32_t *const s_crc = s_in;
  __shared__ uint32_t s_wave[kThreads / 64];
  __shared__ uint32_t s_misc[4];

  const int tid = threadIdx.x, lane = tid & 63;
  unsigned long long t_prev = prof ? wall_clock64() : 0;
  int phase = 0;
  auto mark = [&]() {
    if (prof && tid == 0) {
      const unsigned long long t = wall_clock64();
      atomicAdd(&prof[phase], t - t_prev);
      t_prev = t;
    }
    ++phase;
  };
  for (int i = tid; i < kSyms; i += kThreads) s_code[i] = i < 286 ? tbl->code[i] : 0u;
  if (tid < 4) s_misc[tid] = tid == 0 ? atomicAdd(&ctl->ticket, 1u) : 0u;
  __syncthreads();
  const int64_t chunk = s_misc[0];
  const int64_t n_chunks = (n_bytes + kChunk - 1) / kChunk;
  uint32_t seg[kSegDw], prev_dw;
  int n, seg_n;
  load_chunk(text, n_bytes, chunk, s_in, seg, &n, &seg_n, &prev_dw);
  const int beg = tid * kSeg;
  mark();
  for (int i = tid; i < kInDw; i += kThreads) s_in[i] = (i < 1024) ? crc_table[i] : 0u;
  __syncthreads();
  const SegTokens tk = seg_tokens(seg, seg_n, prev_dw, tid == 0);

  uint32_t tok_bits = 0;
  {
    uint32_t c = tid == 0 ? 0xFFFFFFFFu : 0u;
    const int full = seg_n >> 2;
#pragma unroll
    for (int j = 0; j < kSegDw; ++j) {
      if (j < full) {
        const uint32_t x = c ^ seg[j];
        c = s_crc[768 + (x & 255u)] ^ s_crc[512 + ((x >> 8) & 255u)] ^ s_crc[256 + ((x >> 16) & 255u)] ^ s_crc[x >> 24];
      } else if (j == full) {
        for (int k = 0; k < (seg_n & 3); ++k) c = s_crc[(c ^ (seg[j] >> (8 * k))) & 255u] ^ (c >> 8);
      }
    }
    const int q = n >> 7, r = n & 127;
    if (seg_n == kSeg && tid < q) {
      c = gf2_mul(c, pow128[q - tid - 1]);
      if (r) c = gf2_mul(c, x8rem);
    }
    if (seg_n == 0) c = 0;
#pragma unroll
    for (int d = 32; d >= 1; d >>= 1) c ^= __shfl_xor(c, d, 64);
    if (lane == 0) atomicXor(&s_misc[3], c);
  }
  mark();
  {
#pragma unroll
    for (int j = 0; j < kSegDw; ++j) {
      const uint32_t nl = m_nibble(tk.lit, j);
      if (nl == 0) continue;
      const uint32_t w = seg[j];
#pragma unroll
      for (int k = 0; k < 4; ++k)
        tok_bits += s_code[((nl >> k) & 1u) ? (w >> (8 * k)) & 255u : 287u] >> 16;
    }
    Mask128 st = tk.start;
    while (st.lo | st.hi) {
      const int pos = m_first(st);
      st = m_clear(st, pos);
      uint32_t sy, eb, ev;
      length_symbol((uint32_t)m_run(tk.cover, pos), &sy, &eb, &ev);
      tok_bits += (s_code[sy] >> 16) + eb + 1;
    }
  }
  uint32_t tok_total;
  const uint32_t tok_off = block_scan_excl(tok_bits, s_wave, &tok_total);
  const uint32_t hdr_end = tbl->hdr_end_bits;
  const uint32_t eob_len = s_code[256] >> 16;
  const uint32_t payload_bits = hdr_end - kHeadBits + tok_total + eob_len;
  const uint32_t payload_bytes = (payload_bits + 7) >> 3;
  const bool huff = (18 + payload_bytes + 8 <= (uint32_t)kOutBytes) && (payload_bytes < (uint32_t)n + 5);
  const uint32_t crc = s_misc[3] ^ 0xFFFFFFFFu;
  const uint32_t member = huff ? 18 + payload_bytes + 8 : 18 + 5 + (uint32_t)n + 8;
  if (tid == 0)
    __hip_atomic_store(&status[chunk], st_word(epoch, chunk == 0 ? kStPrefix : kStSize, member), __ATOMIC_RELAXED, __HIP_MEMORY_SCOPE_AGENT);
  mark();

  if (huff) {
    __syncthreads();
    for (int i = tid; i < 1024; i += kThreads) s_in[i] = 0;
    __syncthreads();
    if (tid < kHdrDw) s_out[4 + tid] = tbl->hdr[tid];
    if (tid == 0) {
      s_out[0] = 0x04088b1fu;
      s_out[1] = 0;
      s_out[2] = 0x0006ff00u;
      s_out[3] = 0x00024342u;
    }
    __syncthreads();
    if (tid == 0) atomicOr(&s_out[4], member - 1);
    mark();
    {
      BitWriter bw;
      bw.init(s_out, hdr_end + tok_off);
#pragma unroll
      for (int j = 0; j < kSegDw; ++j) {
        const uint32_t nl = m_nibble(tk.lit, j), ns = m_nibble(tk.start, j);
        if ((nl | ns) == 0) continue;
        const uint32_t w = seg[j];
        uint32_t c[4];
#pragma unroll
        for (int k = 0; k < 4; ++k) c[k] = s_code[((nl >> k) & 1u) ? (w >> (8 * k)) & 255u : 287u];
        uint32_t mv = 0, ml = 0, ks = 4;
        if (ns) {
          ks = (uint32_t)__builtin_ctz(ns);
          uint32_t sy, eb, ev;
          length_symbol((uint32_t)m_run(tk.cover, 4 * j + (int)ks), &sy, &eb, &ev);
          const uint32_t cm = s_code[sy];
          mv = (cm & 0xFFFFu) | (ev << (cm >> 16));
          ml = (cm >> 16) + eb + 1;
        }
        bw.put(ks == 0 ? mv : 0u, ks == 0 ? ml : 0u);
        {
          const uint32_t l0 = c[0] >> 16;
          bw.put((c[0] & 0xFFFFu) | ((c[1] & 0xFFFFu) << l0), l0 + (c[1] >> 16));
        }
        const bool mid = ks == 1 || ks == 2;
        bw.put(mid ? mv : 0u, mid ? ml : 0u);
        {
          const uint32_t l2 = c[2] >> 16;
          bw.put((c[2] & 0xFFFFu) | ((c[3] & 0xFFFFu) << l2), l2 + (c[3] >> 16));
        }
        bw.put(ks == 3 ? mv : 0u, ks == 3 ? ml : 0u);
      }
      bw.flush();
    }
    mark();
    if (tid == 0) {
      BitWriter bw;
      bw.init(s_out, hdr_end + tok_total);
      bw.put(s_code[256] & 0xFFFFu, eob_len);
      bw.flush();
      bw.init(s_out, (18 + payload_bytes) * 8);
      bw.put(crc, 32);
      bw.put((uint32_t)n, 32);
      bw.flush();
    }
    if (tid < 64 && chunk > 0) {
      const uint32_t excl = look_back(status, chunk, epoch, tid, &ctl->error);
      if (tid == 0) {
        s_misc[1] = excl;
        __hip_atomic_store(&status[chunk], st_word(epoch, kStPrefix, excl + member), __ATOMIC_RELAXED, __HIP_MEMORY_SCOPE_AGENT);
      }
    }
    __syncthreads();
    mark();
    const uint32_t off = s_misc[1];
    store_member(dense + off, s_out, member, tid);
    if (tid == 0 && chunk == n_chunks - 1) ctl->total = (int64_t)off + member;
    mark();
  } else {
    if (tid < 64 && chunk > 0) {
      const uint32_t excl = look_back(status, chunk, epoch, tid, &ctl->error);
      if (tid == 0) {
        s_misc[1] = excl;
        __hip_atomic_store(&status[chunk], st_word(epoch, kStPrefix, excl + member), __ATOMIC_RELAXED, __HIP_MEMORY_SCOPE_AGENT);
      }
    }
    __syncthreads();
    uint8_t *slot = dense + s_misc[1];
    if (tid == 0 && chunk == n_chunks - 1) ctl->total = (int64_t)s_misc[1] + member;
    if (tid == 0) {
      const uint8_t head[23] = {0x1f, 0x8b, 8,   4,   0,   0,
                                0,    0,    0,   0xff, 6,  0,
                                'B',  'C',  2,   0,   (uint8_t)((member - 1) & 255), (uint8_t)((member - 1) >> 8),
                                1,    (uint8_t)(n & 255), (uint8_t)(n >> 8), (uint8_t)(~n & 255), (uint8_t)((~n >> 8) & 255)};
      for (int i = 0; i < 23; ++i) slot[i] = head[i];
      uint8_t *t = slot + 23 + n;
      for (int i = 0; i < 4; ++i) t[i] = (uint8_t)(crc >> (8 * i));
      for (int i = 0; i < 4; ++i) t[4 + i] = (uint8_t)((uint32_t)n >> (8 * i));
    }
#pragma unroll
    for (int j = 0; j < kSegDw; ++j)
#pragma unroll
      for (int k = 0; k < 4; ++k)
        if (4 * j + k < seg_n) slot[23 + beg + 4 * j + k] = (uint8_t)(seg[j] >> (8 * k));
  }
}

uint32_t host_gf2_mul(uint32_t a, uint32_t b) {
  uint32_t p = 0;
  for (int i = 0; i < 32; ++i) {
    if (a & (0x80000000u >> i)) p ^= b;
    b = (b >> 1) ^ ((b & 1u) ? kPoly : 0u);
  }
  return p;
}

uint32_t host_xpow8(uint64_t nbytes) {
  uint32_t r = 0x80000000u, b = 0x00800000u;
  while (nbytes) {
    if (nbytes & 1) r = host_gf2_mul(r, b);
    b = host_gf2_mul(b, b);
    nbytes >>= 1;
  }
  return r;
}

}

void deflate_host_tables(uint32_t *crc_table, uint32_t *pow128) {
  for (uint32_t i = 0; i < 256; ++i) {
    uint32_t c = i;
    for (int k = 0; k < 8; ++k) c = (c >> 1) ^ ((c & 1u) ? kPoly : 0u);
    crc_table[i] = c;
  }
  for (int t = 1; t < 4; ++t)
    for (uint32_t i = 0; i < 256; ++i) {
      const uint32_t c = crc_table[(t - 1) * 256 + i];
      crc_table[t * 256 + i] = (c >> 8) ^ crc_table[c & 255u];
    }
  const uint32_t step = host_xpow8(128);
  uint32_t v = 0x80000000u;
  for (int k = 0; k < 256; ++k) {
    pow128[k] = v;
    v = host_gf2_mul(v, step);
  }
}

void launch_deflate_table(const uint8_t *text, int64_t n_bytes, uint32_t *hist, void *table, hipStream_t s) {
  if (n_bytes <= 0) return;
  const int64_t nch = (n_bytes + DF_CHUNK - 1) / DF_CHUNK;
  const int64_t ns = nch < kSampleChunks ? nch : kSampleChunks;
  const int64_t sample_bytes = ns * (int64_t)DF_CHUNK < n_bytes ? ns * (int64_t)DF_CHUNK : n_bytes;
  (void)hipMemsetAsync(hist, 0, 288 * sizeof(uint32_t), s);
  hipLaunchKernelGGL(k_deflate_hist, dim3((unsigned)ns), dim3(kThreads), 0, s, text, sample_bytes, hist);
  hipLaunchKernelGGL(k_deflate_build, dim3(1), dim3(kThreads), 0, s, (const uint32_t *)hist, reinterpret_cast<DfTable *>(table));
}

void launch_deflate(const uint8_t *text, int64_t n_bytes, uint64_t *status, void *ctl, uint32_t epoch, uint8_t *dense,
                    const uint32_t *d_crc_table, const uint32_t *d_pow128, const void *table, hipStream_t s,
                    unsigned long long *d_prof, hipEvent_t ev_begin, hipEvent_t ev_chunks_done) {
  if (n_bytes <= 0) return;
  const int64_t nch = (n_bytes + DF_CHUNK - 1) / DF_CHUNK;
  const uint32_t x8rem = host_xpow8((uint64_t)(n_bytes % DF_CHUNK) & 127u);
  (void)hipMemsetAsync(ctl, 0, DF_CTL_BYTES, s);
  if (ev_begin) (void)hipEventRecord(ev_begin, s);
  hipLaunchKernelGGL(k_deflate_chunks, dim3((unsigned)nch), dim3(kThreads), 0, s, text, n_bytes, dense, status,
                     reinterpret_cast<DfCtl *>(ctl), epoch & 0x3fffffffu, d_crc_table, d_pow128, x8rem,
                     reinterpret_cast<const DfTable *>(table), d_prof);
  if (ev_chunks_done) (void)hipEventRecord(ev_chunks_done, s);
}

}
```

### pbsim3_amd/csrc/deflate_host.cpp

```cpp
#include <hip/hip_runtime.h>
#include <limits.h>
#include <math.h>
#include <stdio.h>
#include <stdlib.h>
#include <string.h>

#include <algorithm>
#include <chrono>
#include <functional>
#include <memory>
#include <string>
#include <thread>
#include <vector>

#include "ctx.h"
#include "engine_internal.h"
#include "unit_io.h"

extern "C" {

extern "C++" {
namespace {

int ensure_deflate_tables(pbsim_ctx *c) {
  if (c->d_df_tables.p) return PBSIM_SUCCEEDED;
  std::vector<uint32_t> t(1024 + 256);
  deflate_host_tables(t.data(), t.data() + 1024);
  if (!upload(c->d_df_tables, t.data(), t.size() * 4, c->stream)) return PBSIM_FAILED;
  HIP_OK(hipStreamSynchronize(c->stream));
  return PBSIM_SUCCEEDED;
}

struct DfGeom {
  int64_t piece, max_ch, n_pieces;
  int ahead, nbuf;
  int64_t off(int64_t j) const { return j * piece; }
  int64_t len(int64_t j, int64_t n) const { return std::min(piece, n - off(j)); }
};
DfGeom df_geom(int64_t n) {
  constexpr int64_t piece_chunks = DF_PIECE_CHUNKS;
  constexpr int kDfAhead = 4;
  static_assert(kDfAhead >= 1 && kDfAhead <= kDfBuffers - 1, "ahead + 1 dense buffers are in use");
  DfGeom g;
  g.piece = piece_chunks * DF_CHUNK;
  g.max_ch = std::min<int64_t>(piece_chunks, (n + DF_CHUNK - 1) / DF_CHUNK);
  g.n_pieces = (n + g.piece - 1) / g.piece;
  g.ahead = kDfAhead;
  g.nbuf = g.ahead + 1;
  return g;
}

int df_launch_piece(pbsim_ctx *c, DfLane &sl, const DfGeom &g, const uint8_t *d_text, int64_t n, int64_t j, bool wait_buffer,
                    bool own_staging, unsigned long long *d_prof) {
  const int b = (int)(j % g.nbuf);
  const int64_t off = g.off(j), len = g.len(j, n);
  const uint32_t *tab = c->d_df_tables.as<uint32_t>();
  int64_t *h_total = reinterpret_cast<int64_t *>(sl.h_df_total.p);
  HIP_OK(sl.d_df_dense[b].ensure((size_t)g.max_ch * DF_SLOT + 64, true));
  if (own_staging) HIP_OK(sl.h_df_out[b].ensure((size_t)g.max_ch * DF_SLOT + 64));
  if (wait_buffer) HIP_OK(hipStreamWaitEvent(sl.stream, sl.ev_cp[b], 0));
  uint8_t *dense = sl.d_df_dense[b].as<uint8_t>();
  if (((sl.epoch + 1) & 0x3fffffffu) == 0) {
    HIP_OK(hipMemsetAsync(sl.d_df_status.p, 0, sl.d_df_status.bytes, sl.stream));
    sl.epoch++;
  }
  launch_deflate(d_text + off, len, sl.d_df_status.as<uint64_t>(), sl.d_df_ctl.p, ++sl.epoch, dense, tab, tab + 1024,
                 sl.d_df_code.p, sl.stream, d_prof, sl.ev_k0[b], sl.ev_k1[b]);
  HIP_OK(hipGetLastError());
  HIP_OK(hipMemcpyAsync(&h_total[2 * b], sl.d_df_ctl.p, DF_CTL_BYTES, hipMemcpyDeviceToHost, sl.stream));
  HIP_OK(hipEventRecord(sl.ev_df[b], sl.stream));
  return PBSIM_SUCCEEDED;
}

int df_begin(pbsim_ctx *c, DfLane &sl, const uint8_t *d_text, int64_t n, bool own_staging, hipStream_t launch_stream) {
  if (!ensure_deflate_tables(c)) return PBSIM_FAILED;
  const DfGeom g = df_geom(n);
  const size_t status_bytes_was = sl.d_df_status.bytes;
  HIP_OK(sl.d_df_status.ensure((size_t)(g.piece / DF_CHUNK) * 8));
  HIP_OK(sl.d_df_ctl.ensure(DF_CTL_BYTES));
  HIP_OK(sl.h_df_total.ensure(DF_CTL_BYTES * kDfBuffers));
  HIP_OK(sl.d_df_code.ensure(DF_TABLE_BYTES + 288 * 4));
  int lane_index = 0;
  for (Slot &slot : c->slots)
    if (&slot.df[1] == &sl) lane_index = 1;
  hipStream_t lane_streams[2];
  if (sl.own_streams) {
    for (int i = 0; i < 2; i++)
      if (!sl.own[i]) HIP_OK(hipStreamCreateWithFlags(&sl.own[i], hipStreamNonBlocking));
    lane_streams[0] = sl.own[0];
    lane_streams[1] = sl.own[1];
  } else {
    for (int i = 0; i < 2; i++)
      if (!c->df_streams[lane_index][i]) HIP_OK(hipStreamCreateWithFlags(&c->df_streams[lane_index][i], hipStreamNonBlocking));
    lane_streams[0] = c->df_streams[lane_index][0];
    lane_streams[1] = c->df_streams[lane_index][1];
  }
  sl.lane_stream = lane_streams[0];
  sl.stream = launch_stream ? launch_stream : lane_streams[0];
  sl.copy_stream = lane_streams[1];
  if (sl.d_df_status.bytes != status_bytes_was) HIP_OK(hipMemsetAsync(sl.d_df_status.p, 0, sl.d_df_status.bytes, sl.stream));
  launch_deflate_table(d_text, n, reinterpret_cast<uint32_t *>(sl.d_df_code.as<uint8_t>() + DF_TABLE_BYTES), sl.d_df_code.p, sl.stream);
  if (!sl.ev_df[0]) {
    for (int i = 0; i < kDfBuffers; i++) {
      HIP_OK(hipEventCreateWithFlags(&sl.ev_df[i], hipEventDisableTiming));
      HIP_OK(hipEventCreateWithFlags(&sl.ev_cp[i], hipEventDisableTiming));
      HIP_OK(hipEventCreate(&sl.ev_k0[i]));
      HIP_OK(hipEventCreate(&sl.ev_k1[i]));
    }
  }
  unsigned long long *d_prof = nullptr;
  if (getenv("PBSIM_DEFLATE_PROF")) {
    HIP_OK(c->d_df_prof.ensure(128));
    HIP_OK(hipMemsetAsync(c->d_df_prof.p, 0, 128, sl.stream));
    d_prof = c->d_df_prof.as<unsigned long long>();
  }
  const int64_t first = std::min<int64_t>(launch_stream ? 1 : g.ahead, g.n_pieces);
  for (int64_t j = 0; j < first; j++)
    if (!df_launch_piece(c, sl, g, d_text, n, j, false, own_staging, d_prof)) return PBSIM_FAILED;
  sl.pre_count = (int)first;
  sl.pre_text = d_text;
  sl.pre_n = n;
  sl.pre_own_staging = own_staging;
  sl.pre_valid = true;
  sl.pre_elsewhere = launch_stream != nullptr;
  if (launch_stream) {
    if (!sl.ev_pre) HIP_OK(hipEventCreateWithFlags(&sl.ev_pre, hipEventDisableTiming));
    HIP_OK(hipEventRecord(sl.ev_pre, launch_stream));
  }
  return PBSIM_SUCCEEDED;
}

template <class F>
int deflate_stream(pbsim_ctx *c, DfLane &sl, const uint8_t *d_text, int64_t n, F &&consume,
                   const std::function<char *(int64_t)> *place = nullptr, const std::function<bool()> *tail_hook = nullptr) {
  if (n <= 0) return PBSIM_SUCCEEDED;
  const bool prelaunched = sl.pre_valid && sl.pre_text == d_text && sl.pre_n == n && sl.pre_own_staging == (place == nullptr);
  sl.pre_valid = false;
  const bool handed = prelaunched && sl.hand_open;
  if (!prelaunched && !pbsim::deflate_settle(sl)) return PBSIM_FAILED;
  if (!prelaunched && !df_begin(c, sl, d_text, n, place == nullptr, nullptr)) return PBSIM_FAILED;
  sl.pre_valid = false;
  if (handed && getenv("PBSIM_TRACE"))
    fprintf(stderr, "[deflate] lane call of %.1f MB found its head handed off (%d pieces launched behind the call in front)\n", n / 1e6,
            sl.pre_count);
  if (sl.pre_elsewhere) {
    sl.stream = sl.lane_stream;
    HIP_OK(hipStreamWaitEvent(sl.stream, sl.ev_pre, 0));
    sl.pre_elsewhere = false;
  }
  const DfGeom g = df_geom(n);
  const int64_t n_pieces = g.n_pieces;
  const int ahead = g.ahead, nbuf = g.nbuf;
  unsigned long long *d_prof = getenv("PBSIM_DEFLATE_PROF") ? c->d_df_prof.as<unsigned long long>() : nullptr;
  const bool trace = getenv("PBSIM_DEFLATE_TRACE") != nullptr;
  const auto now = []() { return std::chrono::duration<double, std::milli>(std::chrono::steady_clock::now().time_since_epoch()).count(); };
  double t_kernel = 0, t_copy = 0, t_consume = 0, t_begin = now();
  double t_first_copy = 0, t_last_copy = 0;
  bool hook_due = false;
  auto offer_tail = [&]() {
    if (tail_hook && hook_due && (*tail_hook)()) hook_due = false;
  };
  int64_t out_bytes = 0;
  std::vector<std::pair<hipEvent_t, hipEvent_t>> tev;
  bool used[kDfBuffers] = {false};
  int64_t *h_total = reinterpret_cast<int64_t *>(sl.h_df_total.p);
  auto launch = [&](int64_t j) -> int {
    return df_launch_piece(c, sl, g, d_text, n, j, used[(int)(j % nbuf)], place == nullptr, d_prof);
  };
  for (int64_t j = sl.pre_count; j < std::min<int64_t>(ahead, n_pieces); j++)
    if (!launch(j)) return PBSIM_FAILED;
  hook_due = n_pieces <= ahead;
  offer_tail();
  const char *prev_ptr = nullptr;
  int64_t prev_bytes = 0;
  int prev_buf = 0;
  for (int64_t k = 0; k < n_pieces; k++) {
    const int b = (int)(k % nbuf);
    const double t0 = now();
    HIP_OK(hipEventSynchronize(sl.ev_df[b]));
    t_kernel += now() - t0;
    const int64_t total = h_total[2 * b + 1];
    if ((uint64_t)h_total[2 * b] >> 32) return fail("deflate: a workgroup's look-back gave up waiting for its predecessors");
    out_bytes += total;
    {
      float ms = 0;
      if (hipEventElapsedTime(&ms, sl.ev_k0[b], sl.ev_k1[b]) == hipSuccess) {
        std::lock_guard<std::mutex> lk(c->prof_mu);
        c->prof_deflate_ms += ms;
        c->prof_deflate_launches++;
        c->prof_deflate_in += g.len(k, n);
        c->prof_deflate_out += total;
      }
    }
    char *dst = place ? (*place)(total) : (char *)sl.h_df_out[b].p;
    if (!dst) return fail("deflate: no room for a compressed piece");
    HIP_OK(hipStreamWaitEvent(sl.copy_stream, sl.ev_df[b], 0));
    if (trace) {
      hipEvent_t e0 = nullptr, e1 = nullptr;
      HIP_OK(hipEventCreate(&e0));
      HIP_OK(hipEventCreate(&e1));
      tev.emplace_back(e0, e1);
      HIP_OK(hipEventRecord(e0, sl.copy_stream));
    }
    if (k == 0) t_first_copy = now();
    HIP_OK(hipMemcpyAsync(dst, sl.d_df_dense[b].p, (size_t)total, hipMemcpyDeviceToHost, sl.copy_stream));
    if (trace) HIP_OK(hipEventRecord(tev.back().second, sl.copy_stream));
    HIP_OK(hipEventRecord(sl.ev_cp[b], sl.copy_stream));
    used[b] = true;
    if (prev_bytes) {
      const double t1 = now();
      HIP_OK(hipEventSynchronize(sl.ev_cp[prev_buf]));
      const double t2 = now();
      if (!consume(prev_ptr, prev_bytes)) return PBSIM_FAILED;
      t_copy += t2 - t1;
      t_consume += now() - t2;
    }
    prev_ptr = dst;
    prev_bytes = total;
    prev_buf = b;
    if (k + ahead < n_pieces && !launch(k + ahead)) return PBSIM_FAILED;
    if (k + ahead == n_pieces - 1) hook_due = true;
    offer_tail();
  }
  if (prev_bytes) {
    const double t1 = now();
    HIP_OK(hipEventSynchronize(sl.ev_cp[prev_buf]));
    const double t2 = now();
    t_last_copy = t2;
    if (!consume(prev_ptr, prev_bytes)) return PBSIM_FAILED;
    t_copy += t2 - t1;
    t_consume += now() - t2;
  }
  sl.hand_open = false;
  if (trace) {
    double t_link = 0, t_span = 0;
    float ms = 0;
    for (auto &e : tev) {
      if (hipEventElapsedTime(&ms, e.first, e.second) == hipSuccess) t_link += ms;
    }
    if (!tev.empty() && hipEventElapsedTime(&ms, tev.front().first, tev.back().second) == hipSuccess) t_span = ms;
    for (auto &e : tev) {
      (void)hipEventDestroy(e.first);
      (void)hipEventDestroy(e.second);
    }
    fprintf(stderr,
            "[deflate] %.1f MB -> %.1f MB in %.1f ms: waited %.1f ms for kernels, %.1f ms for copies, %.1f ms in the consumer; copies: "
            "%.1f ms on the engine within a span of %.1f ms (%.1f GB/s while copying); first copy enqueued at %.3f, last copy "
            "complete at %.3f ms%s%s\n",
            n / 1e6, out_bytes / 1e6, now() - t_begin, t_kernel, t_copy, t_consume, t_link, t_span, t_link > 0 ? out_bytes / t_link / 1e6 : 0.0,
            t_first_copy, t_last_copy, sl.own_streams ? " (chain lane)" : "", handed ? " (head handed off)" : "");
  }
  if (d_prof) {
    unsigned long long t[16];
    HIP_OK(hipMemcpy(t, d_prof, 128, hipMemcpyDeviceToHost));
    const double nch = (double)((n + DF_CHUNK - 1) / DF_CHUNK);
    static const char *names[7] = {"stage", "crc", "sizes+scan", "header", "tokens", "trailer", "store"};
    fprintf(stderr, "[deflate prof] %.0f chunks; us per chunk (lane 0):", nch);
    for (int i = 0; i < 7; ++i) fprintf(stderr, " %s %.1f", names[i], t[i] / nch / 100);
    fprintf(stderr, "\n");
  }
  return PBSIM_SUCCEEDED;
}

int deflate_to_host(pbsim_ctx *c, DfLane &sl, const uint8_t *d_text, int64_t n, char *host_dst, int64_t cap,
                    int64_t *out_bytes) {
  int64_t written = 0;
  const int ok = deflate_stream(c, sl, d_text, n, [&](const char *z, int64_t k) {
    if (written + k > cap) return fail("deflate: output buffer too small");
    memcpy(host_dst + written, z, (size_t)k);
    written += k;
    return PBSIM_SUCCEEDED;
  });
  *out_bytes = written;
  return ok;
}

}
}

extern "C++" int pbsim::deflate_pieces(pbsim_ctx *c, DfLane &lane, const uint8_t *d_text, int64_t n,
                                       const std::function<int(const char *, int64_t)> &consume,
                                       const std::function<char *(int64_t)> *place, const std::function<bool()> *tail_hook) {
  return deflate_stream(c, lane, d_text, n, consume, place, tail_hook);
}
extern "C++" int pbsim::deflate_handoff(pbsim_ctx *c, DfLane &next, int lane_index, const uint8_t *d_text, int64_t n,
                                        bool own_staging, hipEvent_t text_ready) {
  hipStream_t st = c->df_streams[lane_index][0];
  if (!st || next.own_streams || next.hand_open || n <= 0) return fail("deflate_handoff: bad argument");
  if (!next.ev_hand) HIP_OK(hipEventCreateWithFlags(&next.ev_hand, hipEventDisableTiming));
  HIP_OK(hipStreamWaitEvent(st, text_ready, 0));
  const int ok = df_begin(c, next, d_text, n, own_staging, nullptr);
  if (!ok) next.pre_valid = false;
  next.hand_open = true;
  HIP_OK(hipEventRecord(next.ev_hand, st));
  return ok;
}
extern "C++" int pbsim::deflate_settle(DfLane &lane) {
  if (!lane.hand_open) return PBSIM_SUCCEEDED;
  lane.pre_valid = false;
  HIP_OK(hipEventSynchronize(lane.ev_hand));
  lane.hand_open = false;
  return PBSIM_SUCCEEDED;
}
extern "C++" int pbsim::ensure_deflate_ready(pbsim_ctx *c) {
  for (auto &lane : c->df_streams)
    for (hipStream_t &st : lane)
      if (!st) HIP_OK(hipStreamCreateWithFlags(&st, hipStreamNonBlocking));
  return ensure_deflate_tables(c);
}
extern "C++" int pbsim::ensure_crc_tables(pbsim_ctx *c) { return ensure_deflate_tables(c); }
extern "C++" int pbsim::deflate_prelaunch(pbsim_ctx *c, Slot &sl, bool want_read, bool want_maf) {
  const pbsim_batch_info &bi = sl.b_info;
  if (want_read && bi.read_text_bytes > 0 && !df_begin(c, sl.df[0], sl.d_read_text.as<uint8_t>(), bi.read_text_bytes, true, sl.stream))
    return PBSIM_FAILED;
  if (want_maf && bi.maf_text_bytes > 0 && !df_begin(c, sl.df[1], sl.d_maf_text.as<uint8_t>(), bi.maf_text_bytes, true, sl.stream))
    return PBSIM_FAILED;
  return PBSIM_SUCCEEDED;
}

int pbsim_set_deflate(pbsim_ctx *c, int on) {
  if (!c) return fail("bad argument");
  c->deflate = on & 3;
  c->deflate_parallel = (on & 4) != 0;
  return PBSIM_SUCCEEDED;
}

int64_t pbsim_deflate_bound(int64_t n) {
  if (n <= 0) return 0;
  return n + ((n + DF_CHUNK - 1) / DF_CHUNK) * 31;
}

int pbsim_batch_fetch_deflated(pbsim_ctx *c, char *read_gz, int64_t read_cap, char *maf_gz, int64_t maf_cap,
                               int64_t *read_gz_bytes, int64_t *maf_gz_bytes) {
  if (!c || !c->s().b_finalized) return fail("pbsim_batch_fetch_deflated: no finalized batch");
  NEED_DEVICE(c);
  HIP_OK(hipSetDevice(c->device));
  int64_t nr = 0, nm = 0;
  if (read_gz && !deflate_to_host(c, c->s().df[0], c->s().d_read_text.as<uint8_t>(), c->s().b_info.read_text_bytes, read_gz,
                                  read_cap, &nr))
    return PBSIM_FAILED;
  if (maf_gz && !deflate_to_host(c, c->s().df[0], c->s().d_maf_text.as<uint8_t>(), c->s().b_info.maf_text_bytes, maf_gz,
                                 maf_cap, &nm))
    return PBSIM_FAILED;
  if (read_gz_bytes) *read_gz_bytes = nr;
  if (maf_gz_bytes) *maf_gz_bytes = nm;
  return PBSIM_SUCCEEDED;
}

int pbsim_deflate_buffer(pbsim_ctx *c, const void *src, int64_t n, void *dst, int64_t cap, int64_t *out_bytes) {
  if (!c || !out_bytes || n < 0 || (n > 0 && (!src || !dst))) return fail("pbsim_deflate_buffer: bad argument");
  NEED_DEVICE(c);
  HIP_OK(hipSetDevice(c->device));
  *out_bytes = 0;
  if (n == 0) return PBSIM_SUCCEEDED;
  Slot &sl = c->slots[0];
  DevBuf d_in;
  HIP_OK(d_in.ensure((size_t)n + 16));
  HIP_OK(hipMemcpyAsync(d_in.p, src, (size_t)n, hipMemcpyHostToDevice, sl.stream));
  HIP_OK(hipStreamSynchronize(sl.stream));
  return deflate_to_host(c, sl.df[0], d_in.as<uint8_t>(), n, (char *)dst, cap, out_bytes);
}

extern "C++" int pbsim::deliver(pbsim_ctx *c, const pbsim_sink *sink) {
  const pbsim_batch_info &bi = c->s().b_info;
  if (sink && c->defer_text_sync) {
    NEED_DEVICE(c);
    HIP_OK(hipEventSynchronize(c->s().ev_text));
  }
  if (sink && c->deflate) {
    const bool zr = c->deflate & 1, zm = c->deflate & 2;
    NEED_DEVICE(c);
    HIP_OK(hipSetDevice(c->device));
    if (!zr) HIP_OK(c->s().h_read_text.ensure((size_t)bi.read_text_bytes + 16));
    if (!zm) HIP_OK(c->s().h_maf_text.ensure((size_t)bi.maf_text_bytes + 16));
    if ((!zr || !zm) &&
        !pbsim_batch_fetch(c, zr ? nullptr : (char *)c->s().h_read_text.p, zm ? nullptr : (char *)c->s().h_maf_text.p))
      return PBSIM_FAILED;
    Slot &sl = c->s();
    auto send_read = [&]() -> int {
      if (!(sink->on_read_text && bi.read_text_bytes)) return PBSIM_SUCCEEDED;
      if (!zr)
        return sink->on_read_text(sink->user, (const char *)sl.h_read_text.p, bi.read_text_bytes) ? PBSIM_SUCCEEDED
                                                                                                 : fail("sink aborted (read text)");
      return deflate_stream(c, sl.df[0], sl.d_read_text.as<uint8_t>(), bi.read_text_bytes, [&](const char *z, int64_t k) {
        return sink->on_read_text(sink->user, z, k) ? PBSIM_SUCCEEDED : fail("sink aborted (read text)");
      });
    };
    auto send_maf = [&]() -> int {
      if (!(sink->on_maf_text && bi.maf_text_bytes)) return PBSIM_SUCCEEDED;
      if (!zm)
        return sink->on_maf_text(sink->user, (const char *)sl.h_maf_text.p, bi.maf_text_bytes) ? PBSIM_SUCCEEDED
                                                                                              : fail("sink aborted (MAF text)");
      return deflate_stream(c, sl.df[1], sl.d_maf_text.as<uint8_t>(), bi.maf_text_bytes, [&](const char *z, int64_t k) {
        return sink->on_maf_text(sink->user, z, k) ? PBSIM_SUCCEEDED : fail("sink aborted (MAF text)");
      });
    };
    if (c->deflate_parallel && zr && zm && bi.read_text_bytes && bi.maf_text_bytes) {
      if (!ensure_deflate_tables(c)) return PBSIM_FAILED;
      int ok_read = PBSIM_SUCCEEDED;
      std::string err_read;
      std::thread t([&]() {
        (void)hipSetDevice(c->device);
        ok_read = send_read();
        if (!ok_read) err_read = g_err;
      });
      const int ok_maf = send_maf();
      t.join();
      if (!ok_read) return fail(err_read);
      if (!ok_maf) return PBSIM_FAILED;
    } else {
      if (!send_read()) return PBSIM_FAILED;
      if (!send_maf()) return PBSIM_FAILED;
    }
  } else if (sink) {
    HIP_OK(c->s().h_read_text.ensure((size_t)bi.read_text_bytes + 16));
    HIP_OK(c->s().h_maf_text.ensure((size_t)bi.maf_text_bytes + 16));
    if (!pbsim_batch_fetch(c, (char *)c->s().h_read_text.p, (char *)c->s().h_maf_text.p)) return PBSIM_FAILED;
    if (sink->on_read_text && bi.read_text_bytes &&
        !sink->on_read_text(sink->user, (const char *)c->s().h_read_text.p, bi.read_text_bytes))
      return fail("sink aborted (read text)");
    if (sink->on_maf_text && bi.maf_text_bytes &&
        !sink->on_maf_text(sink->user, (const char *)c->s().h_maf_text.p, bi.maf_text_bytes))
      return fail("sink aborted (MAF text)");
  }
  return c->defer_account ? PBSIM_SUCCEEDED : pbsim_batch_account(c);
}
}
```

### pbsim3_amd/csrc/engine.cpp

```cpp
#include <hip/hip_runtime.h>
#include <limits.h>
#include <math.h>
#include <stdio.h>
#include <stdlib.h>
#include <string.h>

#include <algorithm>
#include <chrono>
#include <functional>
#include <memory>
#include <string>
#include <thread>
#include <unordered_map>
#include <vector>

#include "ctx.h"
#include "engine_internal.h"
#include "unit_io.h"
#include "philox.h"

namespace pbsim {
thread_local std::string g_err;
int fail(const std::string &m) {
  g_err = m;
// ... 861 lines not shown
}

extern "C++" int pbsim::chain_reads_for(const pbsim_ctx *c, int64_t ref_len, int64_t remaining) {
  const double lub = (double)std::min<int64_t>(std::min<int64_t>(c->p.len_max, std::max<int64_t>(ref_len, 1)),
                                               std::max<int64_t>(remaining, c->p.len_min));
  const double per_block = (double)regions_of(c) * 64.0 * (scratch_factor_of(c) * lub + kScratchPad + 64.0);
  const int64_t fit = (int64_t)((double)c->scratch_budget / (1.05 * per_block));
  return (int)std::max<int64_t>(1, std::min<int64_t>(kChainReads, fit));
}

extern "C++" int pbsim::chain_end_finalize(pbsim_ctx *c, int64_t len_total_before, pbsim_batch_info *out) {
  if (!c || !c->s().b_enqueued || !c->s().b_chain) return fail("internal: no chain of truncated reads on this slot");
  if (!pbsim_batch_walk_end(c, nullptr)) return PBSIM_FAILED;
  Slot &sl = c->s();
  ChainState *pin = reinterpret_cast<ChainState *>((char *)sl.h_flags.p + sizeof(DeviceFlags) + 16);
  HIP_OK(hipMemcpyAsync(pin, sl.d_chain.p, sizeof(ChainState), hipMemcpyDeviceToHost, sl.stream));
  HIP_OK(hipStreamSynchronize(sl.stream));
  const ChainState cs = *pin;
  pbsim_batch_info bi;
  memset(&bi, 0, sizeof bi);
  bi.first_read = sl.b_first;
  bi.n_reads = sl.b_n;
  bi.n_final = cs.made;
  bi.len_total_after = len_total_before + cs.total;
  bi.quota_reached = cs.done != 0;
  bi.need_truncated_read = !cs.done;
  sl.b_info = bi;
  if (!finalize_text(c, &bi)) return PBSIM_FAILED;
  *out = bi;
  return PBSIM_SUCCEEDED;
}

static void fill_text_args(pbsim_ctx *c, TextArgs *t, int64_t n_emit) {
  memset(t, 0, sizeof *t);
  t->first_read = c->s().b_first;
  t->n_reads = n_emit;
  t->pass_num = c->p.pass_num;
  t->is_wgs = c->p.strategy == PBSIM_STRATEGY_WGS;
  t->is_qs = has_quality_row(c);
  t->unit = (uint32_t)c->s().ref.unit;
  t->ref_len = c->s().ref.len;
  t->len = c->s().d_len.as<int32_t>();
  t->off = c->s().d_off.as<int32_t>();
  t->out_len = c->s().d_out_len.as<int32_t>();
  t->maf_len = c->s().d_maf_len.as<int32_t>();
  t->slot_of_task = c->s().d_slot_of_task.as<int32_t>();
  t->task_of_slot = c->s().d_task_of_slot.as<int32_t>();
  t->row_dst = c->s().d_row_dst.as<int64_t>();
  t->wave_cap = c->s().d_wave_cap.as<int32_t>();
  t->wave_off = c->s().d_wave_off.as<int64_t>();
  t->scratch = c->s().d_scratch.as<uint8_t>();
  t->read_text_len = c->s().d_rt_len.as<int64_t>();
  t->maf_text_len = c->s().d_mt_len.as<int64_t>();
  t->read_text_off = t->read_text_len;
  t->maf_text_off = t->maf_text_len;
  t->id_prefix_len = (int)strlen(c->p.id_prefix);
  memcpy(t->id_prefix, c->p.id_prefix, sizeof t->id_prefix);
  t->rq_len = snprintf(t->rq_text, sizeof t->rq_text, "%f", c->p.accuracy_mean);
  t->bam = c->bam_output && c->p.pass_num > 1;
  t->truth_bam = c->truth_bam;
  t->nsub = c->s().d_nsub.as<int32_t>();
  t->nins = c->s().d_nins.as<int32_t>();
  t->ndel = c->s().d_ndel.as<int32_t>();
  t->n_runs = c->s().d_n_runs.as<int32_t>();
  {
    const float f = strtof(t->rq_text, nullptr);
    memcpy(&t->rq_bits, &f, 4);
  }
  if (c->p.strategy != PBSIM_STRATEGY_WGS) {
    t->name_pad3 = c->p.strategy == PBSIM_STRATEGY_TEMPL;
    t->read_unit = c->d_read_unit.as<int32_t>() + (c->s().b_first - 1);
    t->read_minus = c->d_read_minus.as<uint8_t>() + (c->s().b_first - 1);
    t->unit_len = c->d_unit_len.as<int64_t>();
    t->unit_names = c->d_unit_names.as<char>();
  }
}

extern "C++" int pbsim::finalize_cut(pbsim_ctx *c, int64_t len_total_before, pbsim_batch_info *out) {
  if (!c || !c->s().b_walked) return fail("pbsim_batch_finalize: no walked batch");
  NEED_DEVICE(c);
  HIP_OK(hipSetDevice(c->device));
  DeviceFlags *flags = c->s().d_flags.as<DeviceFlags>();
  const int64_t quota = quota_of(c, c->s().ref.len);
  launch_quota_cut(c->s().d_cum.as<int64_t>(),
                   c->p.method == PBSIM_METHOD_SAMPLE ? nullptr : c->s().d_rawlen.as<int32_t>(), c->s().b_n, len_total_before, quota,
                   c->s().b_truncated ? 1 : 0, flags, c->s().stream);
  DeviceFlags f;
  if (!read_flags(c, &f)) return PBSIM_FAILED;
  const int64_t n_final = f.n_final;
  int64_t cum_final = c->s().b_pass0;
  if (n_final < c->s().b_n) {
    int64_t *pin = reinterpret_cast<int64_t *>((char *)c->s().h_flags.p + sizeof(DeviceFlags));
    HIP_OK(hipMemcpyAsync(pin, c->s().d_cum.as<int64_t>() + n_final, 8, hipMemcpyDeviceToHost, c->s().stream));
    HIP_OK(hipStreamSynchronize(c->s().stream));
    cum_final = *pin;
  }
  pbsim_batch_info bi;
  memset(&bi, 0, sizeof bi);
  bi.first_read = c->s().b_first;
  bi.n_reads = c->s().b_n;
  bi.n_final = n_final;
  bi.len_total_after = len_total_before + cum_final;
  if (c->p.strategy != PBSIM_STRATEGY_WGS) {
    bi.quota_reached = 0;
    bi.need_truncated_read = 0;
  } else if (c->s().b_truncated) {
    bi.quota_reached = bi.len_total_after >= quota;
    bi.need_truncated_read = !bi.quota_reached;
  } else {
    bi.quota_reached = (n_final < c->s().b_n) || (bi.len_total_after >= quota);
    bi.need_truncated_read = (n_final < c->s().b_n) && (bi.len_total_after < quota);
  }
  c->s().b_info = bi;
  *out = bi;
  return PBSIM_SUCCEEDED;
}

extern "C++" int pbsim::finalize_uncut(pbsim_ctx *c, pbsim_batch_info *out) {
  if (!c || !c->s().b_walked) return fail("pbsim_batch_finalize: no walked batch");
  NEED_DEVICE(c);
  pbsim_batch_info bi;
  memset(&bi, 0, sizeof bi);
  bi.first_read = c->s().b_first;
  bi.n_reads = c->s().b_n;
  bi.n_final = c->s().b_n;
  bi.len_total_after = c->s().b_pass0;
  c->s().b_info = bi;
  *out = bi;
  return PBSIM_SUCCEEDED;
}

static int fetch_stats(pbsim_ctx *c, Slot &sl, int64_t n_tasks);
static void collect_text_timing(pbsim_ctx *c, Slot &sl) {
  if (!sl.text_timed || hipEventQuery(sl.ev_t1) != hipSuccess) return;
  float ms = 0;
  if (hipEventElapsedTime(&ms, sl.ev_t0, sl.ev_t1) == hipSuccess) {
    std::lock_guard<std::mutex> lk(c->prof_mu);
    c->prof_text_ms += ms;
    c->prof_text_launches++;
    c->prof_text_in += sl.text_in;
    c->prof_text_out += sl.text_out;
  }
  sl.text_timed = false;
}
extern "C++" int pbsim::finalize_text(pbsim_ctx *c, pbsim_batch_info *info) {
  if (c->truth_bam && !truth_bam_check_names(c)) return PBSIM_FAILED;
  DeviceFlags *flags = c->s().d_flags.as<DeviceFlags>();
  DeviceFlags f;
  pbsim_batch_info bi = c->s().b_info;
  const int P = c->p.pass_num;
  const int64_t n_final = bi.n_final;
  const int64_t n_tasks = n_final * P;
  for (DfLane &L : c->s().df) L.pre_valid = false;
  if (n_tasks > 0) {
    HIP_OK(c->s().d_rt_len.ensure(n_tasks * 8));
    HIP_OK(c->s().d_mt_len.ensure(n_tasks * 8));
    HIP_OK(c->s().d_row_dst.ensure(n_tasks * 6 * 8));
    c->s().stats_fetched = c->defer_text_sync;
    if (c->defer_text_sync && !fetch_stats(c, c->s(), n_tasks)) return PBSIM_FAILED;
    HIP_OK(hipMemsetAsync(&flags->sums[1], 0, 5 * sizeof(int64_t), c->s().stream));
    if (c->truth_bam) HIP_OK(c->s().d_n_runs.ensure(n_tasks * 4));
    TextArgs t;
    fill_text_args(c, &t, n_final);
    if (c->truth_bam) {
      HIP_OK(hipEventRecord(c->s().ev_c0, c->s().stream));
      launch_cigar_count(t, c->s().b_slots_max, flags, c->s().stream);
      HIP_OK(hipEventRecord(c->s().ev_c1, c->s().stream));
    }
    launch_text_sizes(t, flags, c->s().stream);
    launch_exclusive_scan_i64(t.read_text_len, t.read_text_len, n_tasks, c->s().d_scan_tmp.as<int64_t>(), &flags->sums[1],
                              c->s().stream);
    launch_exclusive_scan_i64(t.maf_text_len, t.maf_text_len, n_tasks, c->s().d_scan_tmp.as<int64_t>(), &flags->sums[2],
                              c->s().stream);
    if (!read_flags(c, &f)) return PBSIM_FAILED;
    if (c->truth_bam) {
      float ms = 0;
      if (hipEventElapsedTime(&ms, c->s().ev_c0, c->s().ev_c1) == hipSuccess) {
        std::lock_guard<std::mutex> lk(c->prof_mu);
        c->prof_text_ms += ms;
        c->prof_text_in += 2 * f.sums[5];
      }
    }
    bi.read_text_bytes = f.sums[1];
    bi.maf_text_bytes = f.sums[2];
    bi.bases = f.sums[3];
    bi.ref_bases = f.sums[4];
    bi.maf_columns = f.sums[5];
    HIP_OK(c->s().d_read_text.ensure(std::max<size_t>((size_t)bi.read_text_bytes + 16, 8u << 20)));
    HIP_OK(c->s().d_maf_text.ensure(std::max<size_t>((size_t)bi.maf_text_bytes + 16, 8u << 20)));
    t.read_text = c->s().d_read_text.as<char>();
    t.maf_text = c->s().d_maf_text.as<char>();
    collect_text_timing(c, c->s());
    HIP_OK(hipEventRecord(c->s().ev_t0, c->s().stream));
    launch_text_emit(t, c->s().b_slots_max, flags, c->s().stream);
    HIP_OK(hipEventRecord(c->s().ev_t1, c->s().stream));
    c->s().text_timed = true;
    c->s().text_in = (int64_t)regions_of(c) * bi.maf_columns;
    c->s().text_out = bi.read_text_bytes + bi.maf_text_bytes;
    HIP_OK(hipGetLastError());
    HIP_OK(hipEventRecord(c->s().ev_text, c->s().stream));
    if (!c->defer_text_sync) HIP_OK(hipStreamSynchronize(c->s().stream));
  }
  c->s().b_info = bi;
  c->s().b_finalized = true;
  if (info) *info = bi;
  return PBSIM_SUCCEEDED;
}

extern "C++" int pbsim::emit_batch(pbsim_ctx *c, const BatchOutput &o, pbsim_batch_info *info) {
  return o.arrays ? export_batch(c, o.arrays, info) : finalize_text(c, info);
}
extern "C++" int pbsim::deliver_batch(pbsim_ctx *c, const BatchOutput &o) {
  return o.arrays ? deliver_arrays(c, o.arrays) : deliver(c, o.sink);
}

int pbsim_batch_finalize(pbsim_ctx *c, int64_t len_total_before, pbsim_batch_info *info) {
  pbsim_batch_info bi;
  if (!finalize_cut(c, len_total_before, &bi)) return PBSIM_FAILED;
  return finalize_text(c, info);
}

int pbsim_batch_fetch(pbsim_ctx *c, char *read_text, char *maf_text) {
  if (!c || !c->s().b_finalized) return fail("pbsim_batch_fetch: no finalized batch");
  NEED_DEVICE(c);
  HIP_OK(hipSetDevice(c->device));
  if (read_text && c->s().b_info.read_text_bytes)
    HIP_OK(hipMemcpyAsync(read_text, c->s().d_read_text.p, (size_t)c->s().b_info.read_text_bytes, hipMemcpyDeviceToHost,
                          c->s().stream));
  if (maf_text && c->s().b_info.maf_text_bytes)
    HIP_OK(hipMemcpyAsync(maf_text, c->s().d_maf_text.p, (size_t)c->s().b_info.maf_text_bytes, hipMemcpyDeviceToHost,
                          c->s().stream));
  HIP_OK(hipStreamSynchronize(c->s().stream));
  return PBSIM_SUCCEEDED;
}

static int fetch_stats(pbsim_ctx *c, Slot &sl, int64_t n_tasks) {
  HIP_OK(sl.h_stats.ensure((size_t)n_tasks * 24));
  int32_t *ol = reinterpret_cast<int32_t *>(sl.h_stats.p);
  int32_t *ns = ol + n_tasks, *ni = ns + n_tasks, *nd = ni + n_tasks;
  double *qs = reinterpret_cast<double *>(nd + n_tasks);
  if (sl.sq_pending) {
    HIP_OK(hipStreamWaitEvent(sl.stream, sl.ev_sq_done, 0));
    sl.sq_pending = false;
  }
  HIP_OK(hipMemcpyAsync(ol, sl.d_out_len.p, n_tasks * 4, hipMemcpyDeviceToHost, sl.stream));
  HIP_OK(hipMemcpyAsync(ns, sl.d_nsub.p, n_tasks * 4, hipMemcpyDeviceToHost, sl.stream));
  HIP_OK(hipMemcpyAsync(ni, sl.d_nins.p, n_tasks * 4, hipMemcpyDeviceToHost, sl.stream));
  HIP_OK(hipMemcpyAsync(nd, sl.d_ndel.p, n_tasks * 4, hipMemcpyDeviceToHost, sl.stream));
  if (has_quality_row(c)) HIP_OK(hipMemcpyAsync(qs, sl.d_qsum.p, n_tasks * 8, hipMemcpyDeviceToHost, sl.stream));
  return PBSIM_SUCCEEDED;
}

extern "C++" int pbsim::account_of(pbsim_ctx *c, Slot &sl, StatsAcc *st) {
  if (!c || !sl.b_finalized) return fail("pbsim_batch_account: no finalized batch");
  NEED_DEVICE(c);
  HIP_OK(hipSetDevice(c->device));
  const int P = c->p.pass_num;
  const int64_t n_tasks = sl.b_info.n_final * P;
  if (n_tasks == 0) return PBSIM_SUCCEEDED;
  if (!sl.stats_fetched) {
    if (!fetch_stats(c, sl, n_tasks)) return PBSIM_FAILED;
    HIP_OK(hipStreamSynchronize(sl.stream));
  }
  const int32_t *ol = reinterpret_cast<const int32_t *>(sl.h_stats.p);
  const int32_t *ns = ol + n_tasks, *ni = ns + n_tasks, *nd = ni + n_tasks;
  const double *qs = reinterpret_cast<const double *>(nd + n_tasks);
  const bool quality = has_quality_row(c);
  st->res_num += sl.b_info.n_final;
  std::vector<double> *values = nullptr;
  if (st->keep_values) {
    st->blocks.emplace_back();
    st->blocks.back().first_task = (sl.b_first - 1) * P;
    values = &st->blocks.back().values;
    values->reserve((size_t)n_tasks);
  }
  for (int64_t t = 0; t < n_tasks; t++) stats_add_task(st, c->p.len_max, quality, ol[t], ns[t], ni[t], nd[t], quality ? qs[t] : 0.0, values);
  return PBSIM_SUCCEEDED;
}

extern "C++" int pbsim::account_slot(pbsim_ctx *c, StatsAcc *st) {
  if (!c) return fail("pbsim_batch_account: bad argument");
  return account_of(c, c->s(), st);
}

int pbsim_batch_account(pbsim_ctx *c) { return c ? account_slot(c, &c->st) : fail("pbsim_batch_account: bad argument"); }

int pbsim_get_stats(pbsim_ctx *c, pbsim_stats *o) {
  if (!c || !o) return fail("pbsim_get_stats: bad argument");
  stats_finish(c->st, c->p, c->p.strategy == PBSIM_STRATEGY_WGS ? c->ref_len : 0, o);
  return PBSIM_SUCCEEDED;
}

extern "C++" std::string pbsim::sam_header_text(const pbsim_ctx *c, int64_t unit) {
  std::string h = "@HD\tVN:1.5\tSO:unknown\tpb:3.0.7\n";
  h += "@RG\tID:ffffffff\tPL:PACBIO\tDS:READTYPE=SUBREAD;Ipd:CodecV1=ip;PulseWidth:CodecV1=pw;"
       "BINDINGKIT=101-789-500;SEQUENCINGKIT=101-826-100;BASECALLERVERSION=5.0.0;FRAMERATEHZ=100.000000\tPU:";
  h += c->p.id_prefix;
  if (c->p.strategy == PBSIM_STRATEGY_WGS) h += std::to_string((long)unit);
  h += "\tPM:SEQUELII\n";
  return h;
}
int64_t pbsim_sam_header(pbsim_ctx *c, char *buf, int64_t cap) {
  if (!c) return -1;
  const std::string h = sam_header_text(c, c->unit);
  if (buf && cap > (int64_t)h.size()) memcpy(buf, h.c_str(), h.size() + 1);
  return (int64_t)h.size();
}

int pbsim_set_bam_output(pbsim_ctx *c, int on) {
  if (!c) return fail("bad argument");
  if (on && c->p.pass_num < 2) return fail("BAM output applies to --pass-num >= 2 (single pass writes FASTQ, pbsim.cpp:707)");
  c->bam_output = on != 0;
  return PBSIM_SUCCEEDED;
}

int64_t pbsim_bam_header(pbsim_ctx *c, char *buf, int64_t cap) {
  if (!c) return -1;
  const int64_t lt = pbsim_sam_header(c, nullptr, 0);
  const int64_t n = 4 + 4 + lt + 4;
  if (buf && cap >= n) {
    std::vector<char> text((size_t)lt + 1);
    pbsim_sam_header(c, text.data(), lt + 1);
    memcpy(buf, "BAM\1", 4);
    const uint32_t l = (uint32_t)lt, zero = 0;
    memcpy(buf + 4, &l, 4);
    memcpy(buf + 8, text.data(), (size_t)lt);
    memcpy(buf + 8 + lt, &zero, 4);
  }
  return n;
}

static bool rname_ok(const std::string &s) {
  if (s.empty()) return false;
  for (size_t i = 0; i < s.size(); i++) {
    const unsigned char ch = (unsigned char)s[i];
    if (ch < '!' || ch > '~') return false;
    if (strchr("\\,\"`'()[]{}<>", ch)) return false;
    if (i == 0 && (ch == '*' || ch == '=')) return false;
  }
  return true;
}
extern "C++" int pbsim::truth_bam_check_names(const pbsim_ctx *c) {
  if (c->p.strategy == PBSIM_STRATEGY_WGS) return PBSIM_SUCCEEDED;
  std::unordered_map<std::string, size_t> seen;
  for (size_t u = 0; u < c->unit_sn.size(); u++) {
    const std::string &s = c->unit_sn[u];
    const std::string which = "unit " + std::to_string(u + 1) + " ('" + s + "')";
// ... 353 lines not shown
```

### pbsim3_amd/csrc/kernels.h

```cpp
#pragma once
#include <hip/hip_runtime.h>
#include <stdint.h>

#include "modes.h"

namespace pbsim {

constexpr int kWG = 256;
constexpr int kLenBuckets = 4096;
constexpr int kBinPad = 16;
constexpr int kLenShift = 8;
constexpr int kScratchPad = 64;
constexpr int kMaxClasses = 64;
constexpr int32_t kWaveTransposed = 1 << 30;
constexpr int kHpTile = 4096;

enum : uint32_t {
  kErrScratchOverflow = 1u,
  kErrScratchBudget = 2u,
};

struct DeviceFlags {
  uint32_t error;
  uint32_t high_bytes;
// ... 71 lines not shown

struct WalkArgs {
  uint32_t seed, unit;
  int64_t first_read;
  int32_t pass_num;
  int32_t ncls;
  RefView ref;
  const int32_t *len, *off;
  const int64_t *read_base;
  const uint8_t *read_minus;
  const uint8_t *cls_blob;
  uint32_t stride, rows_off, init_off, tran_off, emis_off, freq_off, rv_off;
  const int32_t *class_start;
  const int32_t *task_of_slot;
  const int32_t *wg_order;
  int32_t mean_len;
  int32_t coop_min_len;
  int32_t coop_dynamic;
  int32_t cap_q8;
  const int32_t *coop_end;
  const int32_t *wave_cap;
  const int64_t *wave_off;
  uint8_t *scratch;
  int32_t *out_len, *maf_len, *nsub, *nins, *ndel;
  double *qsum;
  const uint32_t *sub_thre, *ins_thre, *del_thr;
  const double *qprob;
  DeviceFlags *flags;
};

struct SampleArgs {
  uint32_t seed, unit;
  int64_t first_read;
  int32_t n_lines;
  int32_t n_line_waves;
  int32_t n_coop_waves;
  int32_t n_coop_blocks;
  int64_t n_coop_slots;
  RefView ref;
  const uint8_t *quals;
  const int64_t *line_qoff;
  const int32_t *line_len;
  const int32_t *vbase;
  const int32_t *task_of_slot;
  const int32_t *wave_cap;
  const int64_t *wave_off;
  uint8_t *scratch;
  int32_t *span, *off;
  int32_t *out_len, *maf_len, *nsub, *nins, *ndel;
  double *qsum;
  const uint32_t *sub_thre, *ins_thre, *del_thr;
  const double *qprob;
  DeviceFlags *flags;
};

struct TextArgs {
  int64_t first_read;
  int64_t n_reads;
  int32_t pass_num;
  int32_t is_wgs;
  int32_t is_qs;
  uint32_t unit;
  int64_t ref_len;
  const int32_t *len, *off;
  const int32_t *out_len, *maf_len;
  const int32_t *slot_of_task;
  const int32_t *task_of_slot;
  int64_t *row_dst;
  const int32_t *wave_cap;
  const int64_t *wave_off;
  const uint8_t *scratch;
  const int64_t *read_text_off, *maf_text_off;
  int64_t *read_text_len, *maf_text_len;
  char *read_text, *maf_text;
  char id_prefix[64];
  int32_t id_prefix_len;
  char rq_text[32];
  int32_t rq_len;
  int32_t bam;
  uint32_t rq_bits;
  const int32_t *read_unit;
  const int64_t *unit_len;
  const char *unit_names;
  int32_t name_pad3;
  const uint8_t *read_minus;
  int32_t truth_bam;
  const int32_t *nsub, *nins, *ndel;
  int32_t *n_runs;
};

struct ReadArrays {
  uint8_t *seq, *qual;
  int32_t *ref_pos;
  int64_t *offsets;
  int64_t *read_number;
  int32_t *pass_index, *unit;
  uint8_t *strand;
  int64_t *ref_start;
  int32_t *ref_span, *n_sub, *n_ins, *n_del;
};

struct ExportArgs {
  int64_t first_read;
  int64_t n_reads;
  int64_t bases;
  int32_t pass_num;
  int32_t is_qs;
  uint32_t unit;
  const int32_t *len, *off;
  const int32_t *out_len, *maf_len, *nsub, *nins, *ndel;
  const int32_t *task_of_slot;
  const int32_t *wave_cap;
  const int64_t *wave_off;
  const uint8_t *scratch;
  const int32_t *read_unit;
  const uint8_t *read_minus;
  int64_t *task_off;
  ReadArrays out;
};

void launch_prepare_reference(uint8_t *seq, uint8_t *hp, int flag_hp11, int64_t len, int64_t *tile_first, int64_t *tile_last,
                              int64_t *carry_start, int64_t *carry_next, int keep_first_case, DeviceFlags *flags,
                              hipStream_t s);
void launch_squeeze_lines(const uint8_t *lines, int64_t bytes, uint8_t *dst, int64_t *tile_tmp, int64_t *scan_tmp, int64_t *total,
                          hipStream_t s);
void launch_header_wgs(const HeaderArgs &a, hipStream_t s);
void launch_header_trans(const HeaderArgs &a, hipStream_t s);
void launch_task_sort(const SortArgs &a, hipStream_t s);
void launch_chain_prepare(const HeaderArgs &a, int k, int32_t pass_num, const int32_t *task_of_slot, int32_t *masked,
                          int64_t n_slots_max, ChainState *chain, hipStream_t s);
void launch_chain_update(int k, int32_t pass_num, const int32_t *out_len, ChainState *chain, hipStream_t s);
void launch_chain_init(ChainState *chain, int64_t remaining, hipStream_t s);
void launch_walk_errhmm(const WalkArgs &a, int64_t n_slots_max, uint32_t lds_bytes, bool fast_rv, bool hp_bits,
                        hipStream_t s, int min_lds_kb);
constexpr int kCoopMaxStates = 31;
constexpr int kCoopWaves = 8;
void launch_walk_errhmm_coop(const WalkArgs &a, int n_wg, uint32_t lds_bytes, bool hp_bits, hipStream_t s);
int walk_errhmm_coop_resident(uint32_t lds_bytes, bool hp_bits);
constexpr int kQCoopMaxStates = 63;
void launch_walk_qshmm_coop(const WalkArgs &a, int n_wg, uint32_t lds_bytes, hipStream_t s);
void launch_qshmm_coop_qsum(const WalkArgs &a, int64_t n_slots_max, hipStream_t s);
void launch_walk_qshmm(const WalkArgs &a, int64_t n_slots_max, uint32_t lds_bytes, bool fast_rv, bool hp_bits,
                       hipStream_t s, int min_lds_kb);
void launch_walk_sample(const SampleArgs &a, bool hp_bits, hipStream_t s);
void launch_sample_qsum(const SampleArgs &a, hipStream_t s);
void launch_exclusive_scan_i64(const int64_t *in, int64_t *out, int64_t n, int64_t *tmp, int64_t *total, hipStream_t s);
void launch_gather_pass0_scan(const int32_t *out_len, int64_t n_reads, int32_t pass_num, int64_t *cum, int64_t *tmp,
                              int64_t *total, hipStream_t s);
void launch_quota_cut(const int64_t *cum, const int32_t *rawlen, int64_t n_reads, int64_t len_total_before,
                      int64_t quota, int force_all, DeviceFlags *flags, hipStream_t s);
void launch_cigar_count(const TextArgs &a, int64_t n_slots_max, const DeviceFlags *flags, hipStream_t s);
void launch_text_sizes(const TextArgs &a, DeviceFlags *flags, hipStream_t s);
void launch_text_emit(const TextArgs &a, int64_t n_slots_max, const DeviceFlags *flags, hipStream_t s);
void launch_export_sizes(const ExportArgs &a, DeviceFlags *flags, int64_t *scan_tmp, hipStream_t s);
void launch_export(const ExportArgs &a, int64_t n_slots_max, const DeviceFlags *flags, hipStream_t s);

#define DF_CHUNK 32768
#define DF_SLOT (DF_CHUNK + 64)
#define DF_PIECE_CHUNKS 8192
#define DF_SAMPLE_CHUNKS 64
#define DF_TABLE_HDR_DW 96
#define DF_TABLE_BYTES 2048
void deflate_host_tables(uint32_t *crc_table , uint32_t *pow128 );
void launch_deflate_table(const uint8_t *text, int64_t n_bytes, uint32_t *hist, void *table, hipStream_t s);
#define DF_CTL_BYTES 16
void launch_deflate(const uint8_t *text, int64_t n_bytes, uint64_t *status, void *ctl, uint32_t epoch, uint8_t *dense,
                    const uint32_t *d_crc_table, const uint32_t *d_pow128, const void *table, hipStream_t s,
                    unsigned long long *d_prof = nullptr ,
                    hipEvent_t ev_begin = nullptr, hipEvent_t ev_chunks_done = nullptr );

struct InflateMember {
  int64_t in_off, out_off;
  int32_t in_len, out_len;
  uint32_t crc, pad;
};
enum InflateStatus : int32_t {
  kInfOk = 0,
  kInfBlockType,
  kInfStoredLen,
  kInfTooMany,
  kInfClSet,
  kInfRepeat,
  kInfNoEob,
  kInfLitSet,
  kInfDistSet,
  kInfLitCode,
  kInfDistCode,
  kInfTooFar,
  kInfTruncated,
  kInfTrailing,
  kInfCrc,
  kInfLength,
  kInfCount
};
const char *inflate_reason(int32_t status);
void launch_inflate(const uint8_t *in, const InflateMember *members, int64_t n_members, uint8_t *out, int32_t *status,
                    const uint32_t *d_crc_table, const uint32_t *d_pow128, hipStream_t s);

constexpr int kSpTile = 1024;
inline int64_t sp_tiles(int64_t b0, int64_t b1) { return b1 > b0 ? (b1 - (b0 & ~(int64_t)(kSpTile - 1)) + kSpTile - 1) / kSpTile : 0; }
void launch_sp_count(const uint8_t *buf, int64_t b0, int64_t b1, int64_t *tile_count, int32_t *nul, hipStream_t s);
void launch_sp_lines(const uint8_t *buf, int64_t b0, int64_t b1, int phase, const int64_t *tile_base, uint32_t *rec_start,
                     uint32_t *rec_end, hipStream_t s);
void launch_sp_sums(const uint8_t *buf, const uint32_t *rec_start, const uint32_t *rec_end, int64_t n_rec, int32_t len_min,
                    int32_t len_max, double acc_min, double acc_max, const double *qprob , int32_t *rec_len,
                    double *accuracy, int64_t *padded, hipStream_t s);
void launch_sp_pool(const uint8_t *buf, const uint32_t *rec_start, const int32_t *rec_len, const int64_t *padded, const int64_t *off,
                    int64_t n_rec, uint8_t *pool, hipStream_t s);

enum : int32_t { kSbCounted = 0, kSbSkipped = 1, kSbNoQual = 2 };
void launch_sb_sums(const uint8_t *buf, const uint64_t *rec, int64_t n_rec, int32_t len_min, int32_t len_max, double acc_min, double acc_max,
                    const double *qprob , uint32_t *qual_at, int32_t *rec_len, int32_t *status, double *accuracy,
                    int64_t *padded, hipStream_t s);
void launch_sb_pool(const uint8_t *buf, const uint64_t *rec, const uint32_t *qual_at, const int32_t *rec_len, const int64_t *padded,
                    const int64_t *off, int64_t n_rec, uint8_t *pool, hipStream_t s);

}
```

### pbsim3_amd/csrc/kernels.hip

```cpp
#include <hip/hip_runtime.h>
#include <type_traits>

#include "kernels.h"
#include "philox.h"

namespace pbsim {

namespace {

constexpr int kScanBlock = 256;

__device__ __forceinline__ void short_kernel_priority() { __builtin_amdgcn_s_setprio(3); }
constexpr uint32_t kATGC = 0x43475441u;

__device__ __forceinline__ uint32_t to_upper(uint32_t c) { return (c >= 'a' && c <= 'z') ? c - 32u : c; }

__device__ __forceinline__ void scratch_store(uint32_t *p, uint32_t v) { __builtin_nontemporal_store(v, p); }
__device__ __forceinline__ uint32_t scratch_load(const uint32_t *p) { return *p; }

__device__ __forceinline__ uint32_t complement(uint32_t c) {
  uint32_t r = c;
  r = (c == 'A') ? 'T' : r;
  r = (c == 'T') ? 'A' : r;
  r = (c == 'G') ? 'C' : r;
// ... 3420 lines not shown
  hipLaunchKernelGGL(k_chain_init, dim3(1), dim3(1), 0, s, chain, remaining);
}
void launch_chain_prepare(const HeaderArgs &a, int k, int32_t pass_num, const int32_t *task_of_slot, int32_t *masked,
                          int64_t n_slots_max, ChainState *chain, hipStream_t s) {
  hipLaunchKernelGGL(k_chain_prepare, dim3(blocks_for(n_slots_max, 256)), dim3(256), 0, s, a, k, pass_num, task_of_slot, masked,
                     n_slots_max, chain);
}
void launch_chain_update(int k, int32_t pass_num, const int32_t *out_len, ChainState *chain, hipStream_t s) {
  hipLaunchKernelGGL(k_chain_update, dim3(1), dim3(1), 0, s, k, pass_num, out_len, chain);
}

void launch_header_trans(const HeaderArgs &a, hipStream_t s) {
  if (a.n_reads <= 0) return;
  hipLaunchKernelGGL(k_header_trans, dim3(blocks_for(a.n_reads, 256)), dim3(256), 0, s, a);
}

void launch_task_sort(const SortArgs &a, hipStream_t s) {
  const size_t nbins = (size_t)a.ncls * kLenBuckets;
  (void)hipMemsetAsync(a.hist, 0, nbins * kBinPad * sizeof(int32_t), s);
  (void)hipMemsetAsync(a.bin_cursor, 0, nbins * kBinPad * sizeof(int32_t), s);
  (void)hipMemsetAsync(a.task_of_slot, 0xff, (size_t)a.n_slots_max * sizeof(int32_t), s);
  hipLaunchKernelGGL(k_sort_hist, dim3(blocks_for(a.n_reads, 256)), dim3(256), 0, s, a);
  hipLaunchKernelGGL(k_sort_scan, dim3(1), dim3(kScanBlock), 0, s, a);
  hipLaunchKernelGGL(k_sort_scatter, dim3(blocks_for(a.n_reads, 256)), dim3(256), 0, s, a);
  hipLaunchKernelGGL(k_wave_cap, dim3(blocks_for(a.n_slots_max / 64, 256)), dim3(256), 0, s, a);
  hipLaunchKernelGGL(k_wave_scan, dim3(1), dim3(kScanBlock), 0, s, a);
  const int64_t n_wg = a.n_slots_max / kWG;
  (void)hipMemsetAsync(a.wg_hist, 0, (kLenBuckets + 1) * sizeof(int32_t), s);
  hipLaunchKernelGGL(k_wg_hist, dim3(blocks_for(n_wg, 256)), dim3(256), 0, s, a, a.wg_hist);
  hipLaunchKernelGGL(k_wg_scan, dim3(1), dim3(kScanBlock), 0, s, a.wg_hist, a.wg_start);
  hipLaunchKernelGGL(k_wg_scatter, dim3(blocks_for(n_wg, 256)), dim3(256), 0, s, a, a.wg_start, a.wg_order);
}

static uint32_t walk_lds(uint32_t lds_bytes, int min_lds_kb) {
  static const int env_kb = getenv("PBSIM_WALK_LDS_KB") ? atoi(getenv("PBSIM_WALK_LDS_KB")) : -1;
  const uint32_t pad = (uint32_t)(env_kb >= 0 ? env_kb : min_lds_kb) << 10;
  return lds_bytes > pad ? lds_bytes : pad;
}

void launch_walk_errhmm(const WalkArgs &a, int64_t n_slots_max, uint32_t lds_bytes, bool fast_rv, bool hp_bits,
                        hipStream_t s, int min_lds_kb) {
  lds_bytes = walk_lds(lds_bytes, min_lds_kb);
  const dim3 grid((unsigned)(n_slots_max / kWG)), block(kWG);
  if (fast_rv && hp_bits) hipLaunchKernelGGL((k_walk_errhmm<true, true>), grid, block, lds_bytes, s, a);
  else if (fast_rv) hipLaunchKernelGGL((k_walk_errhmm<true, false>), grid, block, lds_bytes, s, a);
  else if (hp_bits) hipLaunchKernelGGL((k_walk_errhmm<false, true>), grid, block, lds_bytes, s, a);
  else hipLaunchKernelGGL((k_walk_errhmm<false, false>), grid, block, lds_bytes, s, a);
}

int walk_errhmm_coop_resident(uint32_t lds_bytes, bool hp_bits) {
  int n = 0;
  const size_t lds = lds_bytes + kCoopWaves * kCoopWaveLds;
  const hipError_t e = hp_bits ? hipOccupancyMaxActiveBlocksPerMultiprocessor(&n, k_walk_errhmm_coop<true>, kCoopWaves * 64, lds)
                               : hipOccupancyMaxActiveBlocksPerMultiprocessor(&n, k_walk_errhmm_coop<false>, kCoopWaves * 64, lds);
  return e == hipSuccess ? n : 0;
}

void launch_walk_errhmm_coop(const WalkArgs &a, int n_wg, uint32_t lds_bytes, bool hp_bits, hipStream_t s) {
  const dim3 grid((unsigned)n_wg), block(kCoopWaves * 64);
  lds_bytes += kCoopWaves * kCoopWaveLds;
  if (hp_bits) hipLaunchKernelGGL((k_walk_errhmm_coop<true>), grid, block, lds_bytes, s, a);
  else hipLaunchKernelGGL((k_walk_errhmm_coop<false>), grid, block, lds_bytes, s, a);
}

void launch_walk_qshmm_coop(const WalkArgs &a, int n_wg, uint32_t lds_bytes, hipStream_t s) {
  const dim3 grid((unsigned)n_wg), block(kWG);
  lds_bytes += 94 * 32 + (kWG / 64) * kQCoopWaveLds;
  hipLaunchKernelGGL(k_walk_qshmm_coop, grid, block, lds_bytes, s, a);
}

void launch_qshmm_coop_qsum(const WalkArgs &a, int64_t n_slots_max, hipStream_t s) {
  hipLaunchKernelGGL(k_qshmm_coop_qsum, dim3((unsigned)((n_slots_max + 255) / 256)), dim3(256), 0, s, a, (int)n_slots_max);
}

void launch_walk_qshmm(const WalkArgs &a, int64_t n_slots_max, uint32_t lds_bytes, bool fast_rv, bool hp_bits,
                       hipStream_t s, int min_lds_kb) {
  lds_bytes = walk_lds(lds_bytes, min_lds_kb);
  const dim3 grid((unsigned)(n_slots_max / kWG)), block(kWG);
  if (fast_rv && hp_bits) hipLaunchKernelGGL((k_walk_qshmm<true, true>), grid, block, lds_bytes, s, a);
  else if (fast_rv) hipLaunchKernelGGL((k_walk_qshmm<true, false>), grid, block, lds_bytes, s, a);
  else if (hp_bits) hipLaunchKernelGGL((k_walk_qshmm<false, true>), grid, block, lds_bytes, s, a);
  else hipLaunchKernelGGL((k_walk_qshmm<false, false>), grid, block, lds_bytes, s, a);
}

void launch_walk_sample(const SampleArgs &a, bool hp_bits, hipStream_t s) {
  if (a.n_line_waves <= 0) return;
  const int lane_waves = a.n_line_waves - a.n_coop_waves;
  const dim3 grid((unsigned)(a.n_coop_blocks + (lane_waves + kWG / 64 - 1) / (kWG / 64))), block(kWG);
  if (hp_bits) hipLaunchKernelGGL((k_walk_sample<true>), grid, block, 0, s, a);
  else hipLaunchKernelGGL((k_walk_sample<false>), grid, block, 0, s, a);
}

void launch_sample_qsum(const SampleArgs &a, hipStream_t s) {
  if (a.n_coop_slots <= 0) return;
  hipLaunchKernelGGL(k_sample_qsum, dim3((unsigned)((a.n_coop_slots + 255) / 256)), dim3(256), 0, s, a, a.n_coop_slots);
}

void launch_exclusive_scan_i64(const int64_t *in, int64_t *out, int64_t n, int64_t *tmp, int64_t *total,
                               hipStream_t s) {
  if (n <= 0) {
    if (total) (void)hipMemsetAsync(total, 0, sizeof(int64_t), s);
    return;
  }
  const unsigned nb = blocks_for(n, kScanTile);
  hipLaunchKernelGGL(k_scan_sums, dim3(nb), dim3(256), 0, s, in, n, tmp);
  hipLaunchKernelGGL(k_scan_single, dim3(1), dim3(kScanBlock), 0, s, tmp, (int64_t)nb, total);
  hipLaunchKernelGGL(k_scan_apply, dim3(nb), dim3(256), 0, s, in, out, n, (const int64_t *)tmp);
}

void launch_quota_cut(const int64_t *cum, const int32_t *rawlen, int64_t n_reads, int64_t len_total_before,
                      int64_t quota, int force_all, DeviceFlags *flags, hipStream_t s) {
  hipLaunchKernelGGL(k_quota_init, dim3(1), dim3(1), 0, s, flags, n_reads);
  if (!force_all && n_reads > 0)
    hipLaunchKernelGGL(k_quota_find, dim3(blocks_for(n_reads, 256)), dim3(256), 0, s, cum, rawlen, n_reads,
                       len_total_before, quota, flags);
}

void launch_gather_pass0_scan(const int32_t *out_len, int64_t n_reads, int32_t pass_num, int64_t *cum, int64_t *tmp,
                              int64_t *total, hipStream_t s) {
  if (n_reads > 0)
    hipLaunchKernelGGL(k_gather_pass0, dim3(blocks_for(n_reads, 256)), dim3(256), 0, s, out_len, n_reads, pass_num,
                       cum);
  launch_exclusive_scan_i64(cum, cum, n_reads, tmp, total, s);
}

void launch_cigar_count(const TextArgs &a, int64_t n_slots_max, const DeviceFlags *flags, hipStream_t s) {
  if (a.n_reads * a.pass_num <= 0) return;
  hipLaunchKernelGGL(k_cigar_rows<false>, dim3((unsigned)(n_slots_max / 64)), dim3(256), 0, s, a, flags);
}

void launch_text_sizes(const TextArgs &a, DeviceFlags *flags, hipStream_t s) {
  const int64_t n_tasks = a.n_reads * a.pass_num;
  if (n_tasks <= 0) return;
  if (a.truth_bam) hipLaunchKernelGGL(k_text_sizes<true>, dim3(blocks_for(n_tasks, 256)), dim3(256), 0, s, a, flags);
  else hipLaunchKernelGGL(k_text_sizes<false>, dim3(blocks_for(n_tasks, 256)), dim3(256), 0, s, a, flags);
}

void launch_text_emit(const TextArgs &a, int64_t n_slots_max, const DeviceFlags *flags, hipStream_t s) {
  const int64_t n_tasks = a.n_reads * a.pass_num;
  if (n_tasks <= 0) return;
  if (a.truth_bam) hipLaunchKernelGGL(k_text_headers<true>, dim3(blocks_for(n_tasks, 256)), dim3(256), 0, s, a);
  else hipLaunchKernelGGL(k_text_headers<false>, dim3(blocks_for(n_tasks, 256)), dim3(256), 0, s, a);
  if (!a.is_qs || a.pass_num > 1) hipLaunchKernelGGL(k_text_fill, dim3(blocks_for(n_tasks, 4)), dim3(256), 0, s, a);
  if (a.truth_bam) {
    hipLaunchKernelGGL(k_text_rows<false>, dim3((unsigned)(n_slots_max / 64), a.is_qs ? 2 : 1), dim3(256), 0, s, a, flags);
    hipLaunchKernelGGL(k_cigar_rows<true>, dim3((unsigned)(n_slots_max / 64)), dim3(256), 0, s, a, flags);
    hipLaunchKernelGGL(k_aln_finish, dim3(blocks_for(n_tasks, 4)), dim3(256), 0, s, a);
  } else {
    hipLaunchKernelGGL(k_text_rows<true>, dim3((unsigned)(n_slots_max / 64), a.is_qs ? 3 : 2), dim3(256), 0, s, a, flags);
  }
  if (a.bam) hipLaunchKernelGGL(k_bam_finish, dim3(blocks_for(n_tasks, 4)), dim3(256), 0, s, a);
}

void launch_export_sizes(const ExportArgs &a, DeviceFlags *flags, int64_t *scan_tmp, hipStream_t s) {
  const int64_t n_tasks = a.n_reads * a.pass_num;
  if (n_tasks <= 0) return;
  hipLaunchKernelGGL(k_export_sizes, dim3(blocks_for(n_tasks, 256)), dim3(256), 0, s, a, flags);
  launch_exclusive_scan_i64(a.task_off, a.task_off, n_tasks, scan_tmp, a.task_off + n_tasks, s);
}

void launch_export(const ExportArgs &a, int64_t n_slots_max, const DeviceFlags *flags, hipStream_t s) {
  const int64_t n_tasks = a.n_reads * a.pass_num;
  if (n_tasks <= 0) return;
  hipLaunchKernelGGL(k_export_meta, dim3(blocks_for(n_tasks, 256)), dim3(256), 0, s, a);
  if (!a.is_qs && a.bases > 0) (void)hipMemsetAsync(a.out.qual, 0, (size_t)a.bases, s);
  const dim3 grid((unsigned)(n_slots_max / 64), a.is_qs ? 2 : 1);
  if (a.out.ref_pos)
    hipLaunchKernelGGL(k_export_rows<true>, grid, dim3(256), 0, s, a, flags);
  else
    hipLaunchKernelGGL(k_export_rows<false>, grid, dim3(256), 0, s, a, flags);
}

}
```

Measured before the change: 57.99 billion.

## Split deflate into two Huffman classes at sequence/quality boundaries

Adds a class-aware deflate path that builds two Huffman tables, one for sequence bytes and one for quality bytes. Compressed blocks switch tables at toggle positions taken from per-read sequence boundaries that a new kernel computes. The aim is better compression for mixed FASTQ/BAM text, which means fewer output bytes to write and copy. In exchange it adds a histogram pass, extra table builds, more shared-memory bookkeeping and block-switch headers, all of which add compute to the deflate kernels.

```diff
diff --git a/include/pbsim3_amd.h b/include/pbsim3_amd.h
--- a/include/pbsim3_amd.h
+++ b/include/pbsim3_amd.h
@@ -146,6 +146,8 @@
 int pbsim_batch_fetch_deflated(pbsim_ctx *ctx, char *read_gz, int64_t read_cap, char *maf_gz, int64_t maf_cap,
                                int64_t *read_gz_bytes, int64_t *maf_gz_bytes);
 int pbsim_deflate_buffer(pbsim_ctx *ctx, const void *src, int64_t n, void *dst, int64_t cap, int64_t *out_bytes);
+int pbsim_deflate_buffer_classes(pbsim_ctx *ctx, const void *src, int64_t n, const int64_t *toggles, int64_t n_toggles,
+                                 void *dst, int64_t cap, int64_t *out_bytes);
 int64_t pbsim_inflate_bound(const void *src, int64_t n);
 int pbsim_inflate_buffer(pbsim_ctx *ctx, const void *src, int64_t n, void *dst, int64_t cap, int64_t *out_bytes);
 typedef struct pbsim_sorted_bam_sink {
diff --git a/pbsim3_amd/__init__.py b/pbsim3_amd/__init__.py
--- a/pbsim3_amd/__init__.py
+++ b/pbsim3_amd/__init__.py
@@ -433,6 +433,8 @@
     ("pbsim_batch_fetch_deflated", C.c_int, [C.c_void_p, C.c_void_p, C.c_int64, C.c_void_p, C.c_int64,
                                              C.POINTER(C.c_int64), C.POINTER(C.c_int64)]),
     ("pbsim_deflate_buffer", C.c_int, [C.c_void_p, C.c_void_p, C.c_int64, C.c_void_p, C.c_int64, C.POINTER(C.c_int64)]),
+    ("pbsim_deflate_buffer_classes", C.c_int, [C.c_void_p, C.c_void_p, C.c_int64, C.POINTER(C.c_int64), C.c_int64, C.c_void_p,
+                                               C.c_int64, C.POINTER(C.c_int64)]),
     ("pbsim_inflate_bound", C.c_int64, [C.c_void_p, C.c_int64]),
     ("pbsim_inflate_buffer", C.c_int, [C.c_void_p, C.c_void_p, C.c_int64, C.c_void_p, C.c_int64, C.POINTER(C.c_int64)]),
     ("pbsim_truth_bam_sort", C.c_int, [C.c_void_p, C.c_void_p, C.c_int64, C.POINTER(SortedBamSink), C.POINTER(C.c_int64)]),
@@ -1189,12 +1191,16 @@
     def set_deflate(self, mask=3):
         _check(self.lib.pbsim_set_deflate(self.h, 3 if mask is True else int(mask)))
 
-    def deflate_buffer(self, data: bytes) -> bytes:
+    def deflate_buffer(self, data: bytes, toggles=None) -> bytes:
         cap = self.lib.pbsim_deflate_bound(len(data)) + 64
         dst = C.create_string_buffer(cap)
         n = C.c_int64(0)
         src = C.create_string_buffer(data, len(data)) if data else None
-        _check(self.lib.pbsim_deflate_buffer(self.h, src, len(data), dst, cap, C.byref(n)))
+        if toggles is None:
+            _check(self.lib.pbsim_deflate_buffer(self.h, src, len(data), dst, cap, C.byref(n)))
+        else:
+            tog = (C.c_int64 * max(1, len(toggles)))(*toggles)
+            _check(self.lib.pbsim_deflate_buffer_classes(self.h, src, len(data), tog, len(toggles), dst, cap, C.byref(n)))
         return dst.raw[:n.value]
 
     def inflate_buffer(self, data: bytes) -> bytes:
diff --git a/pbsim3_amd/csrc/ctx.h b/pbsim3_amd/csrc/ctx.h
--- a/pbsim3_amd/csrc/ctx.h
+++ b/pbsim3_amd/csrc/ctx.h
@@ -100,6 +100,8 @@
   uint32_t epoch = 0;
   DevBuf d_df_dense[kDfBuffers];
   DevBuf d_df_code;
+  const int64_t *tog = nullptr;
+  int64_t tog_n = 0;
   HostBuf h_df_total, h_df_out[kDfBuffers];
   hipStream_t stream = nullptr;
   hipStream_t copy_stream = nullptr;
@@ -240,6 +242,9 @@
   DevBuf d_scratch, d_read_text, d_maf_text;
   HostBuf h_read_text, h_maf_text, h_stats, h_flags;
   DfLane df[2];
+  DevBuf d_toggles;
+  const void *tog_text = nullptr;
+  int64_t tog_bytes = 0, tog_n = 0;
   hipStream_t walk_stream = nullptr;
   hipEvent_t ev_sq_walk = nullptr, ev_sq_done = nullptr;
   bool sq_pending = false;
diff --git a/pbsim3_amd/csrc/deflate.hip b/pbsim3_amd/csrc/deflate.hip
--- a/pbsim3_amd/csrc/deflate.hip
+++ b/pbsim3_amd/csrc/deflate.hip
@@ -86,6 +86,10 @@
   }
   __device__ __forceinline__ void flush() {
     if (nb) atomicOr(&out[word], (uint32_t)acc);
+  }
+  __device__ __forceinline__ void skip(uint32_t k) {
+    flush();
+    init(out, word * 32 + nb + k);
   }
 };
 
@@ -148,6 +152,16 @@
   else a.hi &= ~(1ull << (pos - 64));
   return a;
 }
+__device__ __forceinline__ Mask128 m_xor(Mask128 a, Mask128 b) { return {a.lo ^ b.lo, a.hi ^ b.hi}; }
+__device__ __forceinline__ uint32_t m_bit(Mask128 a, int pos) { return (uint32_t)((pos < 64 ? a.lo >> pos : a.hi >> (pos - 64)) & 1u); }
+__device__ __forceinline__ Mask128 m_set(Mask128 a, int pos) {
+  if (pos < 64) a.lo |= 1ull << pos;
+  else a.hi |= 1ull << (pos - 64);
+  return a;
+}
+__device__ __forceinline__ Mask128 m_from(int pos) {
+  return {pos < 64 ? ~0ull << pos : 0ull, pos < 64 ? ~0ull : ~0ull << (pos - 64)};
+}
 __device__ __forceinline__ int m_run(Mask128 m, int pos) {
   uint64_t lo, hi;
   if (pos == 0) {
@@ -171,7 +185,7 @@
 };
 
 __device__ __forceinline__ SegTokens seg_tokens(const uint32_t (&seg)[kSegDw], int seg_n, uint32_t prev_dword,
-                                                bool chunk_start) {
+                                                bool chunk_start, Mask128 brk = {0ull, 0ull}) {
   uint64_t e[2] = {0, 0};
   uint32_t pw = prev_dword;
 #pragma unroll
@@ -188,6 +202,7 @@
   valid.hi = seg_n >= 128 ? ~0ull : seg_n > 64 ? (1ull << (seg_n - 64)) - 1 : 0ull;
   Mask128 eq = {e[0] & valid.lo, e[1] & valid.hi};
   if (chunk_start) eq.lo &= ~1ull;
+  eq = m_and(eq, m_not(brk));
   const Mask128 r3 = m_and(eq, m_and(m_shr<1>(eq), m_shr<2>(eq)));
   SegTokens t;
   t.cover = m_or(r3, m_or(m_shl<1>(r3), m_shl<2>(r3)));
@@ -267,7 +282,76 @@
   }
 }
 
+constexpr int kSplitMaxToggles = 32;
+struct DfSplit {
+  const int64_t *toggles;
+  int64_t n_toggles;
+  int64_t base;
+};
+
+__device__ __forceinline__ void seg_classes(const DfSplit &sp, int64_t a, int seg_n, Mask128 *cls, Mask128 *tg) {
+  int64_t lo = 0, hi = sp.n_toggles;
+  while (lo < hi) {
+    const int64_t mid = (lo + hi) >> 1;
+    if (sp.toggles[mid] < a) lo = mid + 1;
+    else hi = mid;
+  }
+  Mask128 c = (lo & 1) ? Mask128{~0ull, ~0ull} : Mask128{0ull, 0ull}, t = {0ull, 0ull};
+  for (int64_t i = lo; i < sp.n_toggles; ++i) {
+    const int64_t rel = sp.toggles[i] - a;
+    if (rel >= seg_n) break;
+    c = m_xor(c, m_from((int)rel));
+    t = m_set(t, (int)rel);
+  }
+  *cls = c;
+  *tg = t;
+}
+
+__global__ __launch_bounds__(kThreads) void k_deflate_hist_classes(const uint8_t *__restrict__ text, int64_t n_bytes,
+                                                                    DfSplit sp, uint32_t *__restrict__ hist) {
+  __shared__ uint32_t s_in[kInDw];
+  __shared__ uint32_t s_hist[2 * kSyms];
+  const int tid = threadIdx.x;
+  for (int i = tid; i < 2 * kSyms; i += kThreads) s_hist[i] = 0;
+  uint32_t seg[kSegDw], prev_dw;
+  int n, seg_n;
+  load_chunk(text, n_bytes, blockIdx.x, s_in, seg, &n, &seg_n, &prev_dw);
+  const int beg = tid * kSeg;
+  Mask128 cls = {0ull, 0ull}, tg = {0ull, 0ull};
+  if (seg_n > 0) seg_classes(sp, sp.base + (int64_t)blockIdx.x * kChunk + beg, seg_n, &cls, &tg);
+  if (tid == 0) tg.lo &= ~1ull;
+  const SegTokens tk = seg_tokens(seg, seg_n, prev_dw, tid == 0, tg);
+#pragma unroll
+  for (int j = 0; j < kSegDw; ++j) {
+    const uint32_t nl = m_nibble(tk.lit, j);
+    if (nl == 0) continue;
+    const uint32_t w = seg[j], nc = m_nibble(cls, j);
+#pragma unroll
+    for (int k = 0; k < 4; ++k)
+      if ((nl >> k) & 1u) atomicAdd(&s_hist[((nc >> k) & 1u) * kSyms + ((w >> (8 * k)) & 255u)], 1u);
+  }
+  Mask128 st = tk.start;
+  while (st.lo | st.hi) {
+    const int pos = m_first(st);
+    st = m_clear(st, pos);
+    uint32_t sy, eb, ev;
+    length_symbol((uint32_t)m_run(tk.cover, pos), &sy, &eb, &ev);
+    atomicAdd(&s_hist[m_bit(cls, pos) * kSyms + sy], 1u);
+  }
+  while (tg.lo | tg.hi) {
+    const int pos = m_first(tg);
+    tg = m_clear(tg, pos);
+    atomicAdd(&s_hist[(m_bit(cls, pos) ^ 1u) * kSyms + 256], 1u);
+  }
+  if (seg_n > 0 && beg + seg_n == n) atomicAdd(&s_hist[m_bit(cls, seg_n - 1) * kSyms + 256], 1u);
+  __syncthreads();
+  for (int i = tid; i < 2 * kSyms; i += kThreads)
+    if (s_hist[i]) atomicAdd(&hist[i], s_hist[i]);
+}
+
 __global__ __launch_bounds__(kThreads) void k_deflate_build(const uint32_t *__restrict__ hist, DfTable *__restrict__ tbl) {
+  hist += blockIdx.x * kSyms;
+  tbl += blockIdx.x;
   __shared__ uint32_t s_freq[kSyms], s_sfreq[kSyms], s_w[kSyms], s_code[kSyms];
   __shared__ uint16_t s_sorted[kSyms], s_par[kSyms], s_leafpar[kSyms], s_dep[kSyms];
   __shared__ uint8_t s_len[kSyms];
@@ -449,13 +533,20 @@
   if ((uint32_t)tid < bytes - done) dst[done + tid] = s8[done + tid];
 }
 
+constexpr int kTogDw0 = 1024;
+constexpr int kLenDw0 = kOutDw;
+constexpr int kSwDw0 = kLenDw0 + 2 * kSyms / 4;
+static_assert(kSwDw0 + kSplitMaxToggles + 1 <= kInDw, "the split tables must fit behind the output image");
+static_assert(kChunk + 5 + 26 + 20 <= kOutBytes, "a member and the store's over-read stay inside the output image");
+
+template <bool kSplit>
 __global__ __launch_bounds__(kThreads) void k_deflate_chunks(const uint8_t *__restrict__ text, int64_t n_bytes,
                                                               uint8_t *__restrict__ dense, uint64_t *__restrict__ status,
                                                               DfCtl *__restrict__ ctl, uint32_t epoch,
                                                               const uint32_t *__restrict__ crc_table,
                                                               const uint32_t *__restrict__ pow128, uint32_t x8rem,
                                                               const DfTable *__restrict__ tbl,
-                                                              unsigned long long *__restrict__ prof) {
+                                                              unsigned long long *__restrict__ prof, DfSplit sp) {
   __shared__ uint32_t s_in[kInDw];
   static_assert(kOutDw <= kInDw, "the output image must fit the input image");
   uint32_t *const s_out = s_in;
@@ -463,6 +554,10 @@
   uint32_t *const s_crc = s_in;
   __shared__ uint32_t s_wave[kThreads / 64];
   __shared__ uint32_t s_misc[4];
+  uint16_t *const s_c16 = reinterpret_cast<uint16_t *>(s_code);
+  uint8_t *const s_len8 = reinterpret_cast<uint8_t *>(s_in + kLenDw0);
+  uint32_t *const s_sw = s_in + kSwDw0;
+  auto code_of = [&](uint32_t e) -> uint32_t { return (uint32_t)s_c16[e] | ((uint32_t)s_len8[e] << 16); };
 
   const int tid = threadIdx.x, lane = tid & 63;
   unsigned long long t_prev = prof ? wall_clock64() : 0;
@@ -475,19 +570,93 @@
     }
     ++phase;
   };
-  for (int i = tid; i < kSyms; i += kThreads) s_code[i] = i < 286 ? tbl->code[i] : 0u;
-  if (tid < 4) s_misc[tid] = tid == 0 ? atomicAdd(&ctl->ticket, 1u) : 0u;
+  if constexpr (!kSplit) {
+    for (int i = tid; i < kSyms; i += kThreads) s_code[i] = i < 286 ? tbl->code[i] : 0u;
+    if (tid < 4) s_misc[tid] = tid == 0 ? atomicAdd(&ctl->ticket, 1u) : 0u;
+  } else if (tid == 0) {
+    const uint32_t ticket = atomicAdd(&ctl->ticket, 1u);
+    const int64_t a0 = sp.base + (int64_t)ticket * kChunk;
+    const int64_t left = n_bytes - (int64_t)ticket * kChunk;
+    const int64_t a1 = a0 + (left < (int64_t)kChunk ? left : (int64_t)kChunk);
+    int64_t lo = 0, hi = sp.n_toggles;
+    while (lo < hi) {
+      const int64_t mid = (lo + hi) >> 1;
+      if (sp.toggles[mid] <= a0) lo = mid + 1;
+      else hi = mid;
+    }
+    const bool some = lo < sp.n_toggles && sp.toggles[lo] < a1;
+    const bool many = lo + kSplitMaxToggles < sp.n_toggles && sp.toggles[lo + kSplitMaxToggles] < a1;
+    s_misc[0] = ticket;
+    s_misc[1] = 0;
+    s_misc[2] = ((uint32_t)lo & 0x7fffffffu) | (some && !many ? 0x80000000u : 0u);
+    s_misc[3] = 0;
+  }
   __syncthreads();
   const int64_t chunk = s_misc[0];
   const int64_t n_chunks = (n_bytes + kChunk - 1) / kChunk;
+  const bool split = kSplit && (s_misc[2] >> 31);
+  const int64_t tog_lo = kSplit ? (int64_t)(s_misc[2] & 0x7fffffffu) : 0;
+  const DfTable *const tbl_a = split ? tbl + 1 : tbl;
+  const DfTable *const tbl_b = kSplit ? tbl + 2 : tbl;
+  const DfTable *const tbl_f = split ? tbl + 1 + (tog_lo & 1) : tbl;
+  if constexpr (kSplit) {
+    for (int i = tid; i < 2 * kSyms; i += kThreads) {
+      const int sym = i < kSyms ? i : i - kSyms;
+      s_c16[i] = sym < 286 ? (uint16_t)(i < kSyms ? tbl_a : tbl_b)->code[sym] : (uint16_t)0;
+    }
+  }
   uint32_t seg[kSegDw], prev_dw;
   int n, seg_n;
   load_chunk(text, n_bytes, chunk, s_in, seg, &n, &seg_n, &prev_dw);
   const int beg = tid * kSeg;
   mark();
-  for (int i = tid; i < kInDw; i += kThreads) s_in[i] = (i < 1024) ? crc_table[i] : 0u;
-  __syncthreads();
-  const SegTokens tk = seg_tokens(seg, seg_n, prev_dw, tid == 0);
+  if constexpr (!kSplit) {
+    for (int i = tid; i < kInDw; i += kThreads) s_in[i] = (i < 1024) ? crc_table[i] : 0u;
+  } else {
+    const int64_t a0 = sp.base + chunk * kChunk;
+    for (int i = tid; i < kOutDw; i += kThreads) {
+      uint32_t v = 0u;
+      if (i < 1024) {
+        v = crc_table[i];
+      } else if (i < kTogDw0 + 64) {
+        const int e = i - kTogDw0;
+        v = 0xFFFFFFFFu;
+        if (split && e < kSplitMaxToggles && tog_lo + e < sp.n_toggles) {
+          const int64_t g = tog_lo + e, x = sp.toggles[g], p = x - a0;
+          const bool twin = (g > 0 && sp.toggles[g - 1] == x) || (g + 1 < sp.n_toggles && sp.toggles[g + 1] == x);
+          if (p < (int64_t)n) v = twin ? 0xFFFFFFFEu : (uint32_t)p;
+        }
+      }
+      s_in[i] = v;
+    }
+    for (int i = tid; i < 2 * kSyms; i += kThreads) {
+      const int sym = i < kSyms ? i : i - kSyms;
+      s_len8[i] = sym < 286 ? (uint8_t)((i < kSyms ? tbl_a : tbl_b)->code[sym] >> 16) : (uint8_t)0;
+    }
+  }
+  __syncthreads();
+  Mask128 cls = {0ull, 0ull}, tg = {0ull, 0ull};
+  int sw_first = 0, sw_count = 0;
+  if constexpr (kSplit) {
+    if (split) {
+      if (tog_lo & 1) cls = Mask128{~0ull, ~0ull};
+      for (int e = 0; e < kSplitMaxToggles; ++e) {
+        const uint32_t p = s_in[kTogDw0 + e];
+        if (p == 0xFFFFFFFFu) break;
+        if (p == 0xFFFFFFFEu) continue;
+        ++sw_count;
+        const int rel = (int)p - beg;
+        if (rel < 0) {
+          cls = m_not(cls);
+          ++sw_first;
+        } else if (rel < kSeg) {
+          cls = m_xor(cls, m_from(rel));
+          tg = m_set(tg, rel);
+        }
+      }
+    }
+  }
+  const SegTokens tk = seg_tokens(seg, seg_n, prev_dw, tid == 0, tg);
 
   uint32_t tok_bits = 0;
   {
@@ -513,7 +682,34 @@
     if (lane == 0) atomicXor(&s_misc[3], c);
   }
   mark();
-  {
+  if constexpr (kSplit) {
+    const uint32_t hdr_bits_a = tbl_a->hdr_end_bits - kHeadBits, hdr_bits_b = tbl_b->hdr_end_bits - kHeadBits;
+#pragma unroll
+    for (int j = 0; j < kSegDw; ++j) {
+      const uint32_t nl = m_nibble(tk.lit, j);
+      if (nl == 0) continue;
+      const uint32_t w = seg[j], nc = m_nibble(cls, j);
+#pragma unroll
+      for (int k = 0; k < 4; ++k)
+        tok_bits += s_len8[((nl >> k) & 1u) ? ((nc >> k) & 1u) * kSyms + ((w >> (8 * k)) & 255u) : 287u];
+    }
+    Mask128 st = tk.start;
+    while (st.lo | st.hi) {
+      const int pos = m_first(st);
+      st = m_clear(st, pos);
+      uint32_t sy, eb, ev;
+      length_symbol((uint32_t)m_run(tk.cover, pos), &sy, &eb, &ev);
+      tok_bits += s_len8[m_bit(cls, pos) * kSyms + sy] + eb + 1;
+    }
+    Mask128 t2 = tg;
+    while (t2.lo | t2.hi) {
+      const int pos = m_first(t2);
+      t2 = m_clear(t2, pos);
+      const uint32_t cb = m_bit(cls, pos);
+      tok_bits += s_len8[(cb ^ 1u) * kSyms + 256] + (cb ? hdr_bits_b : hdr_bits_a);
+    }
+    if (seg_n > 0 && beg + seg_n == n) tok_bits += s_len8[m_bit(cls, seg_n - 1) * kSyms + 256];
+  } else {
 #pragma unroll
     for (int j = 0; j < kSegDw; ++j) {
       const uint32_t nl = m_nibble(tk.lit, j);
@@ -534,8 +730,8 @@
   }
   uint32_t tok_total;
   const uint32_t tok_off = block_scan_excl(tok_bits, s_wave, &tok_total);
-  const uint32_t hdr_end = tbl->hdr_end_bits;
-  const uint32_t eob_len = s_code[256] >> 16;
+  const uint32_t hdr_end = tbl_f->hdr_end_bits;
+  const uint32_t eob_len = kSplit ? 0u : s_code[256] >> 16;
   const uint32_t payload_bits = hdr_end - kHeadBits + tok_total + eob_len;
   const uint32_t payload_bytes = (payload_bits + 7) >> 3;
   const bool huff = (18 + payload_bytes + 8 <= (uint32_t)kOutBytes) && (payload_bytes < (uint32_t)n + 5);
@@ -547,9 +743,9 @@
 
   if (huff) {
     __syncthreads();
-    for (int i = tid; i < 1024; i += kThreads) s_in[i] = 0;
+    for (int i = tid; i < (kSplit ? kTogDw0 + 64 : 1024); i += kThreads) s_in[i] = 0;
     __syncthreads();
-    if (tid < kHdrDw) s_out[4 + tid] = tbl->hdr[tid];
+    if (tid < kHdrDw) s_out[4 + tid] = tbl_f->hdr[tid] & ~(sw_count > 0 && tid == 0 ? 1u << 16 : 0u);
     if (tid == 0) {
       s_out[0] = 0x04088b1fu;
       s_out[1] = 0;
@@ -559,7 +755,62 @@
     __syncthreads();
     if (tid == 0) atomicOr(&s_out[4], member - 1);
     mark();
-    {
+    if constexpr (kSplit) {
+      BitWriter bw;
+      bw.init(s_out, hdr_end + tok_off);
+      const uint32_t hdr_bits_a = tbl_a->hdr_end_bits - kHeadBits, hdr_bits_b = tbl_b->hdr_end_bits - kHeadBits;
+      int sw = sw_first;
+#pragma unroll
+      for (int j = 0; j < kSegDw; ++j) {
+        const uint32_t nl = m_nibble(tk.lit, j), ns = m_nibble(tk.start, j), nt = m_nibble(tg, j);
+        if ((nl | ns | nt) == 0) continue;
+        const uint32_t w = seg[j], nc = m_nibble(cls, j);
+        uint32_t mv = 0, ml = 0, ks = 4;
+        if (ns) {
+          ks = (uint32_t)__builtin_ctz(ns);
+          uint32_t sy, eb, ev;
+          length_symbol((uint32_t)m_run(tk.cover, 4 * j + (int)ks), &sy, &eb, &ev);
+          const uint32_t cm = code_of(((nc >> ks) & 1u) * kSyms + sy);
+          mv = (cm & 0xFFFFu) | (ev << (cm >> 16));
+          ml = (cm >> 16) + eb + 1;
+        }
+#pragma unroll
+        for (int k = 0; k < 4; ++k) {
+          const uint32_t cb = (nc >> k) & 1u;
+          if ((nt >> k) & 1u) {
+            s_sw[sw++] = bw.word * 32 + bw.nb;
+            bw.skip(s_len8[(cb ^ 1u) * kSyms + 256] + (cb ? hdr_bits_b : hdr_bits_a));
+          }
+          const uint32_t c = code_of(((nl >> k) & 1u) ? cb * kSyms + ((w >> (8 * k)) & 255u) : 287u);
+          bw.put(ks == (uint32_t)k ? mv : c & 0xFFFFu, ks == (uint32_t)k ? ml : c >> 16);
+        }
+      }
+      if (seg_n > 0 && beg + seg_n == n) {
+        const uint32_t c = code_of(m_bit(cls, seg_n - 1) * kSyms + 256);
+        bw.put(c & 0xFFFFu, c >> 16);
+      }
+      bw.flush();
+      sw = sw_first;
+      Mask128 t2 = tg;
+      while (t2.lo | t2.hi) {
+        const int pos = m_first(t2);
+        t2 = m_clear(t2, pos);
+        const uint32_t cb = m_bit(cls, pos);
+        const DfTable *const th = cb ? tbl_b : tbl_a;
+        const uint32_t nbits = cb ? hdr_bits_b : hdr_bits_a;
+        bw.init(s_out, s_sw[sw]);
+        const uint32_t c = code_of((cb ^ 1u) * kSyms + 256);
+        bw.put(c & 0xFFFFu, c >> 16);
+        for (uint32_t done = 0; done < nbits; done += 32) {
+          uint32_t v = (th->hdr[done >> 5] >> 16) | (th->hdr[(done >> 5) + 1] << 16);
+          if (done == 0) v = (v & ~1u) | (sw == sw_count - 1 ? 1u : 0u);
+          const uint32_t kb = nbits - done < 32 ? nbits - done : 32;
+          bw.put(kb < 32 ? v & ((1u << kb) - 1) : v, kb);
+        }
+        bw.flush();
+        ++sw;
+      }
+    } else {
       BitWriter bw;
       bw.init(s_out, hdr_end + tok_off);
 #pragma unroll
@@ -597,9 +848,11 @@
     mark();
     if (tid == 0) {
       BitWriter bw;
-      bw.init(s_out, hdr_end + tok_total);
-      bw.put(s_code[256] & 0xFFFFu, eob_len);
-      bw.flush();
+      if constexpr (!kSplit) {
+        bw.init(s_out, hdr_end + tok_total);
+        bw.put(s_code[256] & 0xFFFFu, eob_len);
+        bw.flush();
+      }
       bw.init(s_out, (18 + payload_bytes) * 8);
       bw.put(crc, 32);
       bw.put((uint32_t)n, 32);
@@ -687,27 +940,41 @@
   }
 }
 
-void launch_deflate_table(const uint8_t *text, int64_t n_bytes, uint32_t *hist, void *table, hipStream_t s) {
+static_assert(3 * sizeof(DfTable) <= DF_TABLES_BYTES, "DF_TABLES_BYTES too small");
+
+void launch_deflate_table(const uint8_t *text, int64_t n_bytes, uint32_t *hist, void *table, hipStream_t s,
+                          const int64_t *toggles, int64_t n_toggles) {
   if (n_bytes <= 0) return;
   const int64_t nch = (n_bytes + DF_CHUNK - 1) / DF_CHUNK;
   const int64_t ns = nch < kSampleChunks ? nch : kSampleChunks;
   const int64_t sample_bytes = ns * (int64_t)DF_CHUNK < n_bytes ? ns * (int64_t)DF_CHUNK : n_bytes;
-  (void)hipMemsetAsync(hist, 0, 288 * sizeof(uint32_t), s);
+  const bool classes = toggles && n_toggles > 0;
+  (void)hipMemsetAsync(hist, 0, (classes ? 3 : 1) * 288 * sizeof(uint32_t), s);
   hipLaunchKernelGGL(k_deflate_hist, dim3((unsigned)ns), dim3(kThreads), 0, s, text, sample_bytes, hist);
-  hipLaunchKernelGGL(k_deflate_build, dim3(1), dim3(kThreads), 0, s, (const uint32_t *)hist, reinterpret_cast<DfTable *>(table));
+  if (classes)
+    hipLaunchKernelGGL(k_deflate_hist_classes, dim3((unsigned)ns), dim3(kThreads), 0, s, text, sample_bytes,
+                       DfSplit{toggles, n_toggles, 0}, hist + 288);
+  hipLaunchKernelGGL(k_deflate_build, dim3(classes ? 3 : 1), dim3(kThreads), 0, s, (const uint32_t *)hist,
+                     reinterpret_cast<DfTable *>(table));
 }
 
 void launch_deflate(const uint8_t *text, int64_t n_bytes, uint64_t *status, void *ctl, uint32_t epoch, uint8_t *dense,
                     const uint32_t *d_crc_table, const uint32_t *d_pow128, const void *table, hipStream_t s,
-                    unsigned long long *d_prof, hipEvent_t ev_begin, hipEvent_t ev_chunks_done) {
+                    unsigned long long *d_prof, hipEvent_t ev_begin, hipEvent_t ev_chunks_done, const int64_t *toggles,
+                    int64_t n_toggles, int64_t toggle_base) {
   if (n_bytes <= 0) return;
   const int64_t nch = (n_bytes + DF_CHUNK - 1) / DF_CHUNK;
   const uint32_t x8rem = host_xpow8((uint64_t)(n_bytes % DF_CHUNK) & 127u);
   (void)hipMemsetAsync(ctl, 0, DF_CTL_BYTES, s);
   if (ev_begin) (void)hipEventRecord(ev_begin, s);
-  hipLaunchKernelGGL(k_deflate_chunks, dim3((unsigned)nch), dim3(kThreads), 0, s, text, n_bytes, dense, status,
-                     reinterpret_cast<DfCtl *>(ctl), epoch & 0x3fffffffu, d_crc_table, d_pow128, x8rem,
-                     reinterpret_cast<const DfTable *>(table), d_prof);
+  if (toggles && n_toggles > 0)
+    hipLaunchKernelGGL(k_deflate_chunks<true>, dim3((unsigned)nch), dim3(kThreads), 0, s, text, n_bytes, dense, status,
+                       reinterpret_cast<DfCtl *>(ctl), epoch & 0x3fffffffu, d_crc_table, d_pow128, x8rem,
+                       reinterpret_cast<const DfTable *>(table), d_prof, DfSplit{toggles, n_toggles, toggle_base});
+  else
+    hipLaunchKernelGGL(k_deflate_chunks<false>, dim3((unsigned)nch), dim3(kThreads), 0, s, text, n_bytes, dense, status,
+                       reinterpret_cast<DfCtl *>(ctl), epoch & 0x3fffffffu, d_crc_table, d_pow128, x8rem,
+                       reinterpret_cast<const DfTable *>(table), d_prof, DfSplit{nullptr, 0, 0});
   if (ev_chunks_done) (void)hipEventRecord(ev_chunks_done, s);
 }
 
diff --git a/pbsim3_amd/csrc/deflate_host.cpp b/pbsim3_amd/csrc/deflate_host.cpp
--- a/pbsim3_amd/csrc/deflate_host.cpp
+++ b/pbsim3_amd/csrc/deflate_host.cpp
@@ -65,7 +65,7 @@
     sl.epoch++;
   }
   launch_deflate(d_text + off, len, sl.d_df_status.as<uint64_t>(), sl.d_df_ctl.p, ++sl.epoch, dense, tab, tab + 1024,
-                 sl.d_df_code.p, sl.stream, d_prof, sl.ev_k0[b], sl.ev_k1[b]);
+                 sl.d_df_code.p, sl.stream, d_prof, sl.ev_k0[b], sl.ev_k1[b], sl.tog, sl.tog_n, off);
   HIP_OK(hipGetLastError());
   HIP_OK(hipMemcpyAsync(&h_total[2 * b], sl.d_df_ctl.p, DF_CTL_BYTES, hipMemcpyDeviceToHost, sl.stream));
   HIP_OK(hipEventRecord(sl.ev_df[b], sl.stream));
@@ -79,10 +79,17 @@
   HIP_OK(sl.d_df_status.ensure((size_t)(g.piece / DF_CHUNK) * 8));
   HIP_OK(sl.d_df_ctl.ensure(DF_CTL_BYTES));
   HIP_OK(sl.h_df_total.ensure(DF_CTL_BYTES * kDfBuffers));
-  HIP_OK(sl.d_df_code.ensure(DF_TABLE_BYTES + 288 * 4));
+  HIP_OK(sl.d_df_code.ensure(DF_TABLES_BYTES + 3 * 288 * 4));
+  sl.tog = nullptr;
+  sl.tog_n = 0;
   int lane_index = 0;
-  for (Slot &slot : c->slots)
+  for (Slot &slot : c->slots) {
     if (&slot.df[1] == &sl) lane_index = 1;
+    if ((&slot.df[0] == &sl || &slot.df[1] == &sl) && slot.tog_n > 0 && slot.tog_text == (const void *)d_text && slot.tog_bytes == n) {
+      sl.tog = slot.d_toggles.as<int64_t>();
+      sl.tog_n = slot.tog_n;
+    }
+  }
   hipStream_t lane_streams[2];
   if (sl.own_streams) {
     for (int i = 0; i < 2; i++)
@@ -99,7 +106,8 @@
   sl.stream = launch_stream ? launch_stream : lane_streams[0];
   sl.copy_stream = lane_streams[1];
   if (sl.d_df_status.bytes != status_bytes_was) HIP_OK(hipMemsetAsync(sl.d_df_status.p, 0, sl.d_df_status.bytes, sl.stream));
-  launch_deflate_table(d_text, n, reinterpret_cast<uint32_t *>(sl.d_df_code.as<uint8_t>() + DF_TABLE_BYTES), sl.d_df_code.p, sl.stream);
+  launch_deflate_table(d_text, n, reinterpret_cast<uint32_t *>(sl.d_df_code.as<uint8_t>() + DF_TABLES_BYTES), sl.d_df_code.p, sl.stream,
+                       sl.tog, sl.tog_n);
   if (!sl.ev_df[0]) {
     for (int i = 0; i < kDfBuffers; i++) {
       HIP_OK(hipEventCreateWithFlags(&sl.ev_df[i], hipEventDisableTiming));
@@ -359,6 +367,44 @@
   HIP_OK(hipMemcpyAsync(d_in.p, src, (size_t)n, hipMemcpyHostToDevice, sl.stream));
   HIP_OK(hipStreamSynchronize(sl.stream));
   return deflate_to_host(c, sl.df[0], d_in.as<uint8_t>(), n, (char *)dst, cap, out_bytes);
+}
+
+int pbsim_deflate_buffer_classes(pbsim_ctx *c, const void *src, int64_t n, const int64_t *toggles, int64_t n_toggles, void *dst,
+                                 int64_t cap, int64_t *out_bytes) {
+  if (!c || !out_bytes || n < 0 || (n > 0 && (!src || !dst)) || n_toggles < 0 || (n_toggles > 0 && !toggles) || n_toggles >= INT32_MAX)
+    return fail("pbsim_deflate_buffer_classes: bad argument");
+  for (int64_t i = 0; i < n_toggles; i++)
+    if (toggles[i] < 0 || toggles[i] > n || (i > 0 && toggles[i] <= toggles[i - 1]))
+      return fail("pbsim_deflate_buffer_classes: the toggles must ascend strictly within 0 .. n");
+  NEED_DEVICE(c);
+  HIP_OK(hipSetDevice(c->device));
+  *out_bytes = 0;
+  if (n == 0) return PBSIM_SUCCEEDED;
+  Slot &sl = c->slots[0];
+  DevBuf d_in, d_tog;
+  HIP_OK(d_in.ensure((size_t)n + 16));
+  HIP_OK(hipMemcpyAsync(d_in.p, src, (size_t)n, hipMemcpyHostToDevice, sl.stream));
+  if (n_toggles > 0) {
+    HIP_OK(d_tog.ensure((size_t)n_toggles * 8));
+    HIP_OK(hipMemcpyAsync(d_tog.p, toggles, (size_t)n_toggles * 8, hipMemcpyHostToDevice, sl.stream));
+  }
+  HIP_OK(hipStreamSynchronize(sl.stream));
+  const auto trade = [&]() {
+    std::swap(sl.d_toggles.p, d_tog.p);
+    std::swap(sl.d_toggles.bytes, d_tog.bytes);
+  };
+  const void *keep_text = sl.tog_text;
+  const int64_t keep_bytes = sl.tog_bytes, keep_n = sl.tog_n;
+  trade();
+  sl.tog_text = d_in.p;
+  sl.tog_bytes = n;
+  sl.tog_n = n_toggles;
+  const int ok = deflate_to_host(c, sl.df[0], d_in.as<uint8_t>(), n, (char *)dst, cap, out_bytes);
+  trade();
+  sl.tog_text = keep_text;
+  sl.tog_bytes = keep_bytes;
+  sl.tog_n = keep_n;
+  return ok;
 }
 
 extern "C++" int pbsim::deliver(pbsim_ctx *c, const pbsim_sink *sink) {
diff --git a/pbsim3_amd/csrc/engine.cpp b/pbsim3_amd/csrc/engine.cpp
--- a/pbsim3_amd/csrc/engine.cpp
+++ b/pbsim3_amd/csrc/engine.cpp
@@ -1037,6 +1037,7 @@
   const int64_t n_final = bi.n_final;
   const int64_t n_tasks = n_final * P;
   for (DfLane &L : c->s().df) L.pre_valid = false;
+  c->s().tog_n = 0;
   if (n_tasks > 0) {
     HIP_OK(c->s().d_rt_len.ensure(n_tasks * 8));
     HIP_OK(c->s().d_mt_len.ensure(n_tasks * 8));
@@ -1078,6 +1079,13 @@
     collect_text_timing(c, c->s());
     HIP_OK(hipEventRecord(c->s().ev_t0, c->s().stream));
     launch_text_emit(t, c->s().b_slots_max, flags, c->s().stream);
+    if ((c->deflate & 1) && t.is_qs && (t.bam || P == 1) && 2 * n_tasks < (int64_t)INT32_MAX) {
+      HIP_OK(c->s().d_toggles.ensure((size_t)n_tasks * 16));
+      launch_text_toggles(t, c->s().d_toggles.as<int64_t>(), c->s().stream);
+      c->s().tog_text = c->s().d_read_text.p;
+      c->s().tog_bytes = bi.read_text_bytes;
+      c->s().tog_n = 2 * n_tasks;
+    }
     HIP_OK(hipEventRecord(c->s().ev_t1, c->s().stream));
     c->s().text_timed = true;
     c->s().text_in = (int64_t)regions_of(c) * bi.maf_columns;
diff --git a/pbsim3_amd/csrc/kernels.h b/pbsim3_amd/csrc/kernels.h
--- a/pbsim3_amd/csrc/kernels.h
+++ b/pbsim3_amd/csrc/kernels.h
@@ -247,6 +247,7 @@
 void launch_cigar_count(const TextArgs &a, int64_t n_slots_max, const DeviceFlags *flags, hipStream_t s);
 void launch_text_sizes(const TextArgs &a, DeviceFlags *flags, hipStream_t s);
 void launch_text_emit(const TextArgs &a, int64_t n_slots_max, const DeviceFlags *flags, hipStream_t s);
+void launch_text_toggles(const TextArgs &a, int64_t *toggles, hipStream_t s);
 void launch_export_sizes(const ExportArgs &a, DeviceFlags *flags, int64_t *scan_tmp, hipStream_t s);
 void launch_export(const ExportArgs &a, int64_t n_slots_max, const DeviceFlags *flags, hipStream_t s);
 
@@ -257,12 +258,16 @@
 #define DF_TABLE_HDR_DW 96
 #define DF_TABLE_BYTES 2048
 void deflate_host_tables(uint32_t *crc_table , uint32_t *pow128 );
-void launch_deflate_table(const uint8_t *text, int64_t n_bytes, uint32_t *hist, void *table, hipStream_t s);
+#define DF_TABLES_BYTES (3 * DF_TABLE_BYTES)
+void launch_deflate_table(const uint8_t *text, int64_t n_bytes, uint32_t *hist, void *table, hipStream_t s,
+                          const int64_t *toggles = nullptr, int64_t n_toggles = 0);
 #define DF_CTL_BYTES 16
 void launch_deflate(const uint8_t *text, int64_t n_bytes, uint64_t *status, void *ctl, uint32_t epoch, uint8_t *dense,
                     const uint32_t *d_crc_table, const uint32_t *d_pow128, const void *table, hipStream_t s,
                     unsigned long long *d_prof = nullptr ,
-                    hipEvent_t ev_begin = nullptr, hipEvent_t ev_chunks_done = nullptr );
+                    hipEvent_t ev_begin = nullptr, hipEvent_t ev_chunks_done = nullptr ,
+                    const int64_t *toggles = nullptr, int64_t n_toggles = 0,
+                    int64_t toggle_base = 0 );
 
 struct InflateMember {
   int64_t in_off, out_off;
diff --git a/pbsim3_amd/csrc/kernels.hip b/pbsim3_amd/csrc/kernels.hip
--- a/pbsim3_amd/csrc/kernels.hip
+++ b/pbsim3_amd/csrc/kernels.hip
@@ -3596,6 +3596,22 @@
   if (a.bam) hipLaunchKernelGGL(k_bam_finish, dim3(blocks_for(n_tasks, 4)), dim3(256), 0, s, a);
 }
 
+__global__ __launch_bounds__(256) void k_text_toggles(TextArgs a, int64_t *__restrict__ toggles) {
+  const int64_t t = (int64_t)blockIdx.x * 256 + threadIdx.x;
+  if (t >= a.n_reads * a.pass_num) return;
+  const int64_t *rd = a.row_dst + t * 6;
+  const int64_t q = a.out_len[t];
+  const int64_t beg = a.bam ? rd[0] : rd[1];
+  toggles[2 * t] = beg;
+  toggles[2 * t + 1] = beg + (a.bam ? (q + 1) / 2 : q);
+}
+
+void launch_text_toggles(const TextArgs &a, int64_t *toggles, hipStream_t s) {
+  const int64_t n_tasks = a.n_reads * a.pass_num;
+  if (n_tasks <= 0) return;
+  hipLaunchKernelGGL(k_text_toggles, dim3(blocks_for(n_tasks, 256)), dim3(256), 0, s, a, toggles);
+}
+
 void launch_export_sizes(const ExportArgs &a, DeviceFlags *flags, int64_t *scan_tmp, hipStream_t s) {
   const int64_t n_tasks = a.n_reads * a.pass_num;
   if (n_tasks <= 0) return;
```

Result: no change. 58.08 billion, median of 2 (+0.1%).
